# ZhicengShi/mclSTExp

Measured on AMD Instinct MI355X. Metric: training spots/sec (= steps/sec x global batch) at batch 128/GPU, 224px patches, 1000 genes, higher is better.
Workload: dtype bf16; 1 GPU; BASELINE configs[1]: train step, batch 128/GPU, 224x224 patches, 1000 genes, densenet121 image encoder; global_batch=128, parallelism=dp1, backbone_dtype=bf16, infonce=fused, infonce_effective=exact (fused from 1024 pairs), hip_graphs=True, optimizer=Adam(lr=1e-4, wd=1e-3) incl. 2x(65536,G) tables

## Files before the change

### include/mclstexp_hip.h

```cpp
#ifndef MCLSTEXP_HIP_H
#define MCLSTEXP_HIP_H

#include <stddef.h>
#include <stdint.h>

#ifdef __cplusplus
extern "C" {
#endif

#define MCL_ABI_VERSION 13

#define MCL_OK 0
#define MCL_EINVAL (-1)
#define MCL_EUNSUPPORTED (-2)
#define MCL_EWORKSPACE (-3)

typedef void* mcl_stream_t;

int mcl_abi_version(void);
const char* mcl_error_string(int code);

#define MCL_EPI_GELU 1
#define MCL_EPI_GELU_BWD 2
#define MCL_EPI_ACCUM 4
#define MCL_COMPUTE_F32 0
#define MCL_COMPUTE_BF16 1

typedef struct mcl_gemm_args {
  uint32_t struct_size;
  int32_t M, N, K, batch;
  const float* A; int64_t sAm, sAk, sAb;
  const float* B; int64_t sBk, sBn, sBb;
  float* C; int64_t ldc, sCb;
  float alpha;
  int32_t flags;
  const float* bias;
  const float* resid; int64_t ldr, sRb;
  float* pre_out; int64_t ldp;
  const float* aux; int64_t ldaux;
  int32_t compute;
  int32_t ksplit;
  float* workspace;
  const float* flt_thr; int32_t* flt_cnt; float* flt_val; int32_t* flt_idx; int32_t flt_cap;
  uint32_t* counters;
} mcl_gemm_args;

int mcl_gemm(const mcl_gemm_args* args, mcl_stream_t stream);
uint32_t mcl_gemm_args_size(void);
uint32_t mcl_gemm_args_min_size(void);
int32_t mcl_gemm_auto_ksplit(int32_t M, int32_t N, int32_t K, int32_t batch);
int64_t mcl_gemm_workspace_floats(int32_t M, int32_t N, int32_t batch, int32_t ksplit);
int mcl_gemm_group(const mcl_gemm_args* args, int32_t n, mcl_stream_t stream);

int32_t mcl_proj_head_ksplit(int32_t M, int32_t D);
int64_t mcl_proj_head_ws_floats(int32_t M, int32_t ksplit);
int mcl_proj_head_fwd(const float* x, int64_t ldx, int32_t M, int32_t D, const float* wp, int64_t ldwp, const float* bp,
                      const float* wf, int64_t ldwf, const float* bf, const float* gamma, const float* beta, float eps,
                      float* e, float* p, float* a, float* z, float* mean, float* rstd, float* ws, uint32_t* counters,
                      int32_t ksplit, mcl_stream_t stream);
int mcl_proj_head_bwd_rows(const float* de, int64_t ldde, int32_t M, const float* z, const float* mean, const float* rstd,
                           const float* gamma, const float* p, const float* wf, int64_t ldwf, float* dz, float* dp,
                           float* dgamma, float* dbeta, float* dbf, float* dbp, int32_t accumulate_mask, float* ws,
                           uint32_t* counter, mcl_stream_t stream);

int mcl_pos_embed_add_fwd(const float* expr, int64_t ld_expr, const float* pos ,
                          const float* x_table, const float* y_table, int64_t ld_table, int32_t n_rows,
                          float* out, int64_t ld_out, int32_t* ix, int32_t* iy, int32_t* err_flag,
                          int32_t B, int32_t G, mcl_stream_t stream);

int mcl_embed_rowgrad(const float* d_out, int64_t ld_dout, const int32_t* idx, int32_t* owner_idx,
                      float* row_grad, int64_t ld_rg, int32_t B, int32_t G, mcl_stream_t stream);

int mcl_embed_scatter_rows(const int32_t* owner_idx, const float* row_grad, int64_t ld_rg, float* table_grad,
                           int64_t ld_table, int32_t B, int32_t G, int32_t accumulate, mcl_stream_t stream);

int mcl_layernorm_fwd(const float* x, int64_t ldx, const float* gamma, const float* beta, float* y, int64_t ldy,
                      float* mean, float* rstd, int32_t rows, int32_t cols, float eps, mcl_stream_t stream);
int mcl_layernorm_bwd(const float* dy, int64_t lddy, const float* x, int64_t ldx, const float* gamma,
                      const float* mean, const float* rstd, const float* dx_add, int64_t ldadd, float* dx,
                      int64_t lddx, float* dgamma, float* dbeta, int32_t accumulate_params, int32_t rows, int32_t cols,
                      mcl_stream_t stream);

int mcl_attention_fwd(const float* qkv, int64_t ld, int32_t B, int32_t heads, int32_t dim_head, float scale, float* out,
                      int64_t ldo, float* lse, mcl_stream_t stream);
int mcl_attention_bwd(const float* qkv, int64_t ld, int32_t B, int32_t heads, int32_t dim_head, float scale, const float* out,
                      const float* dout, int64_t ldo, const float* lse, float* dvec, float* dqkv, int64_t ldq,
                      mcl_stream_t stream);
int mcl_attention_batched_fwd(const float* qkv, int64_t ld, int32_t B, int32_t nseq, int32_t heads, int32_t dim_head, float scale,
                              float* out, int64_t ldo, float* lse, mcl_stream_t stream);
int mcl_attention_batched_bwd(const float* qkv, int64_t ld, int32_t B, int32_t nseq, int32_t heads, int32_t dim_head, float scale,
                              const float* out, const float* dout, int64_t ldo, const float* lse, float* dvec, float* dqkv,
                              int64_t ldq, mcl_stream_t stream);
int mcl_softmax_rows_fwd(float* s, int64_t ld, int32_t n_rows, int32_t cols, float scale, mcl_stream_t stream);
int mcl_softmax_rows_bwd(const float* p, float* dp, int64_t ld, int32_t n_rows, int32_t cols, float scale,
                         mcl_stream_t stream);

int mcl_colsum(const float* x, int64_t ldx, float* out, int32_t rows, int32_t cols, int32_t accumulate, mcl_stream_t stream);
int mcl_colred_group(int32_t n, const float* const* a, const int64_t* lda, const float* const* x, const int64_t* ldx,
                     const float* const* mean, const float* const* rstd, float* const* out0, float* const* out1,
                     const int32_t* cols, const int32_t* accumulate, int32_t rows, mcl_stream_t stream);
int64_t mcl_rowred_workspace_floats(int32_t rows, int32_t cols);
int mcl_colsum_ws(const float* x, int64_t ldx, float* out, int32_t rows, int32_t cols, int32_t accumulate, float* workspace,
                  mcl_stream_t stream);
int mcl_layernorm_bwd_ws(const float* dy, int64_t lddy, const float* x, int64_t ldx, const float* gamma, const float* mean,
                         const float* rstd, const float* dx_add, int64_t ldadd, float* dx, int64_t lddx, float* dgamma,
                         float* dbeta, int32_t accumulate_params, int32_t rows, int32_t cols, float* workspace, mcl_stream_t stream);

int mcl_soft_clip_mid(const float* S, const float* Tg, const float* lse_row, const float* lse_col, const float* tcol, int32_t B,
                      float c, float* dS, float* dA, float* loss_rows, mcl_stream_t stream);
int mcl_symmetrize(const float* a, int32_t B, float* out, mcl_stream_t stream);

int mcl_infonce_lse(const float* S, int64_t ldS, int32_t R, int32_t C, float* row_lse, float* col_lse,
                    mcl_stream_t stream);
int mcl_infonce_loss(const float* S, int64_t ldS, const float* row_lse, const float* col_lse,
                     int32_t di0, int32_t dj0, int32_t n_diag, int32_t use_rows, int32_t use_cols,
                     float* loss_sum, mcl_stream_t stream);
int mcl_infonce_loss_mean(const float* S, int64_t ldS, const float* row_lse, const float* col_lse, int32_t n, float denom,
                          float* loss_out, mcl_stream_t stream);
int mcl_infonce_dlogits(const float* S, int64_t ldS, const float* row_lse, const float* col_lse, int32_t R,
                        int32_t C, int32_t row0, int32_t col0, float coef, float* dS, int64_t lddS,
                        mcl_stream_t stream);

int64_t mcl_infonce_fused_workspace_bytes(int32_t R, int32_t C, int32_t dim);
int mcl_infonce_fused_lse(const void* a, int64_t lda, const void* b, int64_t ldb, int32_t R, int32_t C, int32_t dim,
                          int32_t diag_off, float inv_temp, float* lse, float* diag, void* workspace, int64_t ws_bytes,
                          mcl_stream_t stream);
int mcl_infonce_fused_grad(const void* a, int64_t lda, const void* b, int64_t ldb, int32_t R, int32_t C, int32_t dim,
                           int32_t diag_off, float inv_temp, const float* lse_a, const float* lse_b, float coef, float* dA,
                           void* workspace, int64_t ws_bytes, mcl_stream_t stream);
int mcl_cast_f32_to_bf16(const float* x, int64_t ldx, void* y, int64_t ldy, int64_t rows, int32_t cols,
                         mcl_stream_t stream);

int64_t mcl_gemm_bf16_workspace_floats(int32_t M, int64_t ldc, int32_t ksplit);
int mcl_gemm_bf16(const void* A, int64_t lda, int64_t sAb, const void* B, int64_t ldb, int64_t sBb, void* C, int64_t ldc,
                  int64_t sCb, int32_t M, int32_t N, int32_t K, int32_t batch, int32_t batch2, int64_t sAb2, int64_t sBb2,
                  int64_t sCb2, float alpha, int32_t flags,
                  const float* bias, const void* resid, int64_t ldr, int64_t sRb, const void* aux, int64_t ldaux,
                  void* pre_out, int64_t ldp, int32_t ksplit, float* workspace, int32_t accumulate, mcl_stream_t stream);
int mcl_ln_bf16_fwd(const void* x, int64_t ldx, const float* gamma, const float* beta, void* y, int64_t ldy, float* mean,
                    float* rstd, int64_t rows, int32_t D, float eps, mcl_stream_t stream);
int64_t mcl_colred_workspace_floats(int64_t rows, int32_t D);
int mcl_ln_bf16_bwd(const void* dy, int64_t lddy, const void* x, int64_t ldx, const float* gamma, const float* mean,
                    const float* rstd, const void* dx_add, int64_t ldadd, void* dx, int64_t lddx, float* workspace,
                    float* dgamma, float* dbeta, int32_t accumulate, int64_t rows, int32_t D, mcl_stream_t stream);
int mcl_colsum_bf16(const void* x, int64_t ldx, int64_t rows, int32_t D, float* workspace, float* out, int32_t accumulate,
                    mcl_stream_t stream);
int mcl_softmax_bf16_fwd(void* s, int64_t ld, int64_t rows, int32_t n, mcl_stream_t stream);
int mcl_softmax_bf16_bwd(const void* P, void* dP, int64_t ld, int64_t rows, int32_t n, float scale, mcl_stream_t stream);
int mcl_vit_attn_fwd(const void* qkv, void* o, float* lse, int32_t B, int32_t T, int32_t heads, float scale, mcl_stream_t stream);
int mcl_vit_attn_bwd(const void* qkv, const void* o, const void* dout, const float* lse, float* dsum, void* dqkv, int32_t B,
                     int32_t T, int32_t heads, float scale, mcl_stream_t stream);
int mcl_vit_patchify_tokens(const float* img, int64_t sb, int64_t sc, int64_t sy, int64_t sx, int32_t B, int32_t H, int32_t W,
                            int32_t p, void* out, int32_t lead_zero_row, int32_t out_f32, mcl_stream_t stream);
int mcl_vit_cls_row(const float* cls, const float* pos, void* x, int32_t B, int32_t T, int32_t D, int32_t dtype,
                    mcl_stream_t stream);
int mcl_vit_assemble_f32(const float* tok, const float* cls, const float* pos, float* x, int32_t B, int32_t T, int32_t D,
                         mcl_stream_t stream);
int mcl_vit_tokens_extract(const void* dx, void* dtok, int32_t B, int32_t T, int32_t D, int32_t dtype, mcl_stream_t stream);
int mcl_vit_token_mean_fwd(const void* x, float* feat, int32_t B, int32_t T, int32_t D, int32_t dtype, mcl_stream_t stream);
int mcl_vit_token_mean_bwd(const float* dfeat, void* dx, int32_t B, int32_t T, int32_t D, int32_t dtype, mcl_stream_t stream);
int mcl_vit_pos_grad(const void* dx, float* dpos, float* dcls, int32_t B, int32_t T, int32_t D, int32_t dtype,
                     int32_t accumulate, mcl_stream_t stream);
int mcl_vit_zero_cls_rows(void* dx, int32_t B, int32_t T, int32_t D, int32_t dtype, mcl_stream_t stream);
int mcl_strided4_f32(const float* src, int32_t n0, int32_t n1, int32_t n2, int32_t n3, int64_t a0, int64_t a1, int64_t a2,
                     int64_t a3, void* dst, int64_t d0, int64_t d1, int64_t d2, int64_t d3, int32_t dst_dtype, int32_t accumulate,
                     mcl_stream_t stream);
int mcl_copy_rows(const void* src, int64_t ld_src_bytes, void* dst, int64_t ld_dst_bytes, int64_t rows, int64_t row_bytes,
                  mcl_stream_t stream);
int mcl_weight_rot180(const void* w, void* wf, int32_t Co, int32_t k, int32_t Ci, int32_t dtype, mcl_stream_t stream);
int mcl_vit_patchify(const float* img, int64_t sb, int64_t sc, int64_t sy, int64_t sx, int32_t B, int32_t H, int32_t W,
                     int32_t p, void* out_bf16, mcl_stream_t stream);

int mcl_quant_e4m3_rows(const float* x, int64_t ldx, int32_t rows, int32_t cols, void* q, int64_t ldq, void* scale,
                        int64_t ld_scale, void* deq_bf16, int64_t ldd, mcl_stream_t stream);
int mcl_dequant_e4m3_rows(const void* q, int64_t ldq, const void* scale, int64_t ld_scale, int32_t rows, int32_t cols,
                          void* deq_bf16, int64_t ldd, mcl_stream_t stream);
int64_t mcl_infonce_fp8_workspace_bytes(int32_t R, int32_t C);
int mcl_infonce_fp8_lse(const void* a8, int64_t lda, const void* scale_a, int64_t ld_sa, const void* b8, int64_t ldb,
                        const void* scale_b, int64_t ld_sb, int32_t R, int32_t C, int32_t dim, float inv_temp, float* lse,
                        void* workspace, int64_t ws_bytes, mcl_stream_t stream);
int mcl_infonce_rowdot_bf16(const void* a, int64_t lda, const void* b, int64_t ldb, int32_t R, int32_t C, int32_t dim,
                            int32_t diag_off, float inv_temp, float* diag, mcl_stream_t stream);

int64_t mcl_bn_workspace_floats(int64_t S, int32_t C, int32_t dtype);
int mcl_bn_stats(const void* x, int64_t ld, int64_t S, int32_t C, int32_t dtype, void* copy_out, int64_t ld_out,
                 float* workspace, float eps, float* mean, float* var, float* rstd, mcl_stream_t stream);
int mcl_bn_act_fwd(const void* x, int64_t ldx, int64_t S, int32_t C, int32_t dtype, const float* gamma,
                   const float* beta, const float* mean, const float* rstd, int32_t relu, void* y, int64_t ldy,
                   mcl_stream_t stream);
int mcl_bn_act_bwd(const void* dy, int64_t lddy, const void* x, int64_t ldx, int64_t S, int32_t C, int32_t dtype,
                   const float* gamma, const float* beta, const float* mean, const float* rstd, int32_t relu,
                   float* workspace, float* dgamma, float* dbeta, int32_t accumulate_params, void* dx, int64_t lddx,
                   int32_t accumulate, mcl_stream_t stream);

int64_t mcl_dense_conv1x1_workspace_floats(int64_t S);
int mcl_dense_conv1x1_fwd(const void* x, int64_t ldx, int64_t S, int32_t K, const float* gamma, const float* beta,
                          const float* mean, const float* rstd, const void* W, void* z, int64_t ldz, float* workspace,
                          float eps, float* zmean, float* zvar, float* zrstd, mcl_stream_t stream);

int64_t mcl_dense_conv3x3_workspace_floats(int64_t S);
int mcl_dense_conv3x3_fwd(const void* z, int64_t S, int32_t H, int32_t W, const float* gamma, const float* beta,
                          const float* mean, const float* rstd, const void* W2, void* out, int64_t ldo,
                          float* workspace, float eps, float* ymean, float* yvar, float* yrstd, mcl_stream_t stream);

int64_t mcl_dense_conv3x3_wrw_workspace_floats(int64_t S);
int mcl_dense_conv3x3_wrw_det(const void* dy, int64_t lddy, const void* z, int64_t S, int32_t H, int32_t W,
                              const float* gamma, const float* beta, const float* mean, const float* rstd,
                              float* workspace, float* dW, int32_t accumulate_w, mcl_stream_t stream);

int64_t mcl_dense_bn1_bwd_workspace_floats(int64_t S, int32_t C);
int mcl_dense_bn1_bwd(const void* dz, const void* W1, int32_t C, const void* x, int64_t ldx, int64_t S,
                      const float* gamma, const float* beta, const float* mean, const float* rstd, float* workspace,
                      float* dgamma, float* dbeta, int32_t accumulate_params, void* gbuf, int64_t ldg,
                      mcl_stream_t stream);

int mcl_dense_bn1_dx_window(const void* dz, const void* W1, int32_t C, int32_t c0, int32_t nc, const void* x, int64_t ldx,
                            int64_t S, const float* gamma, const float* beta, const float* mean, const float* rstd,
                            const float* coef, void* gbuf, int64_t ldg, mcl_stream_t stream);
int mcl_dense_bn1_dx_pair(const void* dzA, const void* W1A, int32_t ldwA, const float* gammaA, const float* betaA,
                          const float* coefA, const void* dzB, const void* W1B, const float* gammaB, const float* betaB,
                          const float* coefB, int32_t C, const void* x, int64_t ldx, int64_t S, const float* mean,
                          const float* rstd, void* gbuf, int64_t ldg, mcl_stream_t stream);

int64_t mcl_wrw_workspace_floats(int64_t S, int32_t M, int32_t N);
int mcl_dense_bn1_wrw(const void* dz, const void* W1, int32_t C, const void* x, int64_t ldx, int64_t S,
                      const float* gamma, const float* beta, const float* mean, const float* rstd, float* workspace,
                      float* dW, int32_t accumulate_w, float* dgamma, float* dbeta, int32_t accumulate_params,
                      float* coef_out, mcl_stream_t stream);
int mcl_dense_bn1_dx(const void* dz, const void* W1, int32_t C, const void* x, int64_t ldx, int64_t S,
                     const float* gamma, const float* beta, const float* mean, const float* rstd, const float* coef,
                     void* gbuf, int64_t ldg, mcl_stream_t stream);
int mcl_dense_bn1_dx_sums(const void* dz, const void* W1, int32_t C, const void* x, int64_t ldx, int64_t S,
                          const float* gamma, const float* beta, const float* mean, const float* rstd, float* workspace,
                          float* dgamma, float* dbeta, int32_t accumulate_params, float* kprev, int32_t have_prev, void* gbuf,
                          int64_t ldg, mcl_stream_t stream);
int mcl_dense_bn1_fix(const void* x, int64_t ldx, void* gbuf, int64_t ldg, int64_t S, int32_t c0, int32_t nc,
                      const float* mean, const float* rstd, const float* kacc, mcl_stream_t stream);
int mcl_conv1x1_wrw_det(const void* dz, int64_t ldz, const void* a, int64_t lda, const float* gamma, const float* beta,
                        const float* mean, const float* rstd, float* workspace, float* dW, int32_t accumulate_w,
                        int64_t S, int32_t M, int32_t N, mcl_stream_t stream);

int64_t mcl_dense_conv3x3_bwd_workspace_floats(int64_t S);
int mcl_dense_conv3x3_bwd(const void* dy, int64_t lddy, int64_t S, int32_t H, int32_t W, const void* W2, const void* z,
                          const float* gamma, const float* beta, const float* mean, const float* rstd, float* workspace,
                          float* dgamma, float* dbeta, int32_t accumulate_params, void* g2, void* dz, mcl_stream_t stream);
int mcl_dense_conv3x3_bwd_fix(const void* dy, int64_t lddy, int64_t S, int32_t H, int32_t W, const void* W2, const void* z,
                              const float* gamma, const float* beta, const float* mean, const float* rstd, float* workspace,
                              float* dgamma, float* dbeta, int32_t accumulate_params, void* g2, void* dz, const void* xfix,
                              int64_t ldxf, const float* fmean, const float* frstd, const float* fk, void* dyc,
                              mcl_stream_t stream);

int mcl_avgpool2_nhwc_bf16(const void* x, void* y, int32_t N, int32_t H, int32_t W, int32_t C, int32_t backward,
                           mcl_stream_t stream);
int mcl_maxpool3s2_nhwc_bf16_fwd(const void* x, void* y, void* idx, int32_t N, int32_t H, int32_t W, int32_t C,
                                 mcl_stream_t stream);
int mcl_maxpool3s2_nhwc_bf16_bwd(const void* idx, const void* dy, void* dx, int32_t N, int32_t H, int32_t W, int32_t C,
                                 mcl_stream_t stream);
int mcl_maxpool3s2_nhwc_bf16_bwd_ld(const void* idx, const void* dy, int64_t lddy, void* dx, int32_t N, int32_t H, int32_t W,
                                    int32_t C, mcl_stream_t stream);

int mcl_bn_act_avgpool_fwd(const void* x, int64_t ldx, int32_t N, int32_t H, int32_t W, int32_t C, const float* gamma,
                           const float* beta, const float* mean, const float* rstd, void* y, int64_t ldy,
                           mcl_stream_t stream);
int mcl_bn_act_avgpool_bwd(const void* dp, int64_t lddp, const void* x, int64_t ldx, int32_t N, int32_t H, int32_t W,
                           int32_t C, const float* gamma, const float* beta, const float* mean, const float* rstd,
                           float* workspace, float* dgamma, float* dbeta, int32_t accumulate_params, void* dx,
                           int64_t lddx, mcl_stream_t stream);
int64_t mcl_conv0_workspace_floats(int32_t N, int32_t H, int32_t W);
int mcl_conv0_fwd(const void* x, int32_t N, int32_t H, int32_t W, const void* Wt, void* y, float* workspace, float eps,
                  float* mean, float* var, float* rstd, mcl_stream_t stream);
int64_t mcl_conv0_wrw_workspace_floats(int32_t N, int32_t H, int32_t W);
int mcl_conv0_wrw(const void* x, int32_t N, int32_t H, int32_t W, const void* dy, float* workspace, float* dW,
                  int32_t accumulate_w, mcl_stream_t stream);

int mcl_bn_act_maxpool_fwd(const void* x, int32_t N, int32_t H, int32_t W, int32_t C, const float* gamma,
                           const float* beta, const float* mean, const float* rstd, void* y, void* idx,
                           mcl_stream_t stream);
int mcl_accum_into_f32(float* dst, const void* src, int64_t n, int32_t src_dtype, mcl_stream_t stream);

int mcl_bn_gap_fwd(const void* x, int64_t ldx, int32_t B, int32_t HW, int32_t C, const float* gamma, const float* beta,
                   const float* mean, const float* rstd, float* out, float* xmean, mcl_stream_t stream);
int mcl_bn_gap_bwd(const float* g, const float* xmean, const void* x, int64_t ldx, int32_t B, int32_t HW, int32_t C,
                   const float* gamma, const float* mean, const float* rstd, float* coef, float* dgamma, float* dbeta,
                   int32_t accumulate_params, void* dx, int64_t lddx, mcl_stream_t stream);
int mcl_bn_eval_rstd(int32_t n, const float* const* running_var, float* const* rstd_out, const int32_t* C, const float* eps,
                     mcl_stream_t stream);
int mcl_bn_running_update(int32_t n, float* const* running_mean, float* const* running_var, const float* const* mean,
                          const float* const* var, int64_t* const* num_batches_tracked, const int32_t* C,
                          const float* factor, const float* momentum, mcl_stream_t stream);
int mcl_image_to_bf16_nhwc(const float* x, int64_t sb, int64_t sc, int64_t sy, int64_t sx, int32_t B, int32_t C, int32_t H,
                           int32_t W, void* y, mcl_stream_t stream);
int mcl_fill_zero(void* p, int64_t bytes, mcl_stream_t stream);
int mcl_dropout_fwd(const float* x, float* y, void* mask, int64_t n, float p, uint64_t seed, mcl_stream_t stream);
int mcl_dropout_bwd(const float* dy, const void* mask, float* dx, int64_t n, float p, mcl_stream_t stream);
int mcl_gelu_f32(const float* x, const float* dy, float* out, int64_t n, mcl_stream_t stream);
int mcl_add_f32(const float* a, const float* b, float* y, int64_t n, mcl_stream_t stream);
int mcl_stamp(void* buf, int32_t idx, mcl_stream_t stream);
int mcl_scale2_f32(const float* a, int64_t na, const float* b, int64_t nb, const float* s, float* ya, float* yb,
                   mcl_stream_t stream);

int mcl_im2col_nhwc(const void* x, int64_t ldx, int32_t N, int32_t H, int32_t W, int32_t C, int32_t KH, int32_t KW,
                    int32_t stride, int32_t pad, int32_t dtype, void* cols, mcl_stream_t stream);
int mcl_col2im_nhwc(const void* dcols, int32_t N, int32_t H, int32_t W, int32_t C, int32_t KH, int32_t KW, int32_t stride,
                    int32_t pad, int32_t dtype, void* dx, int64_t lddx, int32_t accumulate, mcl_stream_t stream);
int mcl_maxpool3s2_nhwc_fwd_any(const void* x, void* y, void* idx, int32_t N, int32_t H, int32_t W, int32_t C, int32_t dtype,
                                mcl_stream_t stream);
int mcl_maxpool3s2_nhwc_bwd_any(const void* idx, const void* dy, void* dx, int32_t N, int32_t H, int32_t W, int32_t C,
                                int32_t dtype, mcl_stream_t stream);
int mcl_avgpool2_nhwc_any(const void* x, void* y, int32_t N, int32_t H, int32_t W, int32_t C, int32_t backward, int32_t dtype,
                          mcl_stream_t stream);
int mcl_gap_nhwc_fwd(const void* x, int64_t ldx, int32_t B, int32_t HW, int32_t C, int32_t dtype, float* out,
                     mcl_stream_t stream);
int mcl_gap_nhwc_bwd(const float* g, int32_t B, int32_t HW, int32_t C, int32_t dtype, void* dx, mcl_stream_t stream);
int mcl_add_relu(const void* a, const void* b, void* y, int64_t n, int32_t backward, int32_t dtype, mcl_stream_t stream);

int mcl_dense_block_pack_w1(const void* const* w1_ptrs, void* const* out_ptrs, int32_t L, int32_t C0, mcl_stream_t stream);
int64_t mcl_dense_block_fwd_workspace_bytes(int32_t B, int32_t L);
int mcl_dense_block_fwd(void* buf, int32_t B, int32_t H, int32_t W, int32_t Ct, int32_t C0, int32_t L,
                        const void* const* layer_ptrs, float eps1, float eps2, float* mean, float* var, float* rstd,
                        void* workspace, int32_t* err_flag, uint32_t max_spins, void* stamps, mcl_stream_t stream);

int mcl_dense_block_pack_bwd(const void* const* w1_ptrs, const void* const* w2_ptrs, void* const* w1t_ptrs,
                             void* const* w2t_ptrs, int32_t L, int32_t C0, mcl_stream_t stream);
int64_t mcl_dense_block_bwd_workspace_bytes(int32_t B, int32_t L);
int mcl_dense_block_bwd(const void* buf, void* gbuf, int32_t B, int32_t H, int32_t W, int32_t Ct, int32_t C0, int32_t L,
                        const void* const* layer_ptrs, const float* mean, const float* rstd, void* workspace,
                        int32_t* err_flag, uint32_t max_spins, void* stamps, mcl_stream_t stream);

int mcl_adam_step(float* p, const float* g, float* m, float* v, int64_t n, double lr, double beta1, double beta2,
                  double eps, double weight_decay, double bc1, double bc2, mcl_stream_t stream);
int mcl_adam_table_step(float* p, float* m, float* v, int32_t n_rows, int32_t cols, const int32_t* row_slot,
                        const float* row_grad, int64_t ld_rg, double lr, double beta1, double beta2, double eps,
                        double weight_decay, double bc1, double bc2, mcl_stream_t stream);

int mcl_adam_consts_update(int64_t* step, float* consts, const double* hyper, mcl_stream_t stream);
int mcl_adam_step_dev(float* p, const float* g, float* m, float* v, int64_t n, const float* consts, mcl_stream_t stream);
int mcl_adam_table_step_dev(float* p, float* m, float* v, int32_t n_rows, int32_t cols, const int32_t* row_slot,
                            const float* row_grad, int64_t ld_rg, const float* consts, mcl_stream_t stream);
int mcl_adam_step_dev_shadow(float* p, const float* g, float* m, float* v, int64_t n, const float* consts,
                             void* shadow_bf16, mcl_stream_t stream);
int mcl_adam_consts_update_hist(int64_t* step, float* consts, const double* hyper, float* hist, int32_t hist_len,
                                mcl_stream_t stream);
int mcl_adam_table_lazy(float* p0, float* m0, float* v0, int32_t* row_step0, float* p1, float* m1, float* v1,
                        int32_t* row_step1, int32_t n_rows, int32_t cols, const float* pos, const int32_t* owner0,
                        const int32_t* owner1, int32_t n_owner, const float* row_grad0, const float* row_grad1, int64_t ld_rg,
                        const int64_t* step, const float* hist, int32_t hist_len, mcl_stream_t stream);
int mcl_row_slot_update(int32_t* row_slot, const int32_t* owner_idx, int32_t B, int32_t fill, mcl_stream_t stream);

int mcl_l2_normalize_rows(const float* x, int64_t ldx, float* y, int64_t ldy, int32_t rows, int32_t dim,
                          mcl_stream_t stream);
int mcl_topk_rows_max_k(void);
int mcl_topk_rows(const float* sim, int64_t ld, int32_t rows, int32_t n, int32_t k, float* values, int64_t* indices,
                  mcl_stream_t stream);
int mcl_topk_rows_indexed(const float* cand_val, int64_t ld, const int32_t* cand_idx, int64_t ld_idx, int rows, int n, int k,
                          float* values, int64_t* indices, int32_t* tie_flag, mcl_stream_t stream);
int mcl_knn_weighted_average(const float* spot_key, int64_t ldk, const float* expression_key, int64_t lde,
                             const float* query, int64_t ldq, const int64_t* indices, int32_t n_query, int32_t k,
                             int32_t dim, int32_t genes, int32_t ord, float* emb_pred, float* expr_pred,
                             mcl_stream_t stream);

int mcl_expr_metrics(const void* pred, int64_t ld_pred, int32_t pred_dtype, const void* truth, int64_t ld_true,
                     int32_t true_dtype, const int64_t* offsets, int32_t S, int32_t G, int32_t n_heg, double* r,
                     double* true_mean, int64_t* heg, double* summary, double* work, mcl_stream_t stream);

int mcl_pearson_pvalue(const double* r, const int64_t* offsets, int32_t S, int32_t G, double* p, double* neglog10p,
                       mcl_stream_t stream);
int mcl_gene_rank(const double* neglog10p, const double* r, int32_t S, int32_t G, int32_t top_n, double* mean,
                  int32_t* n_defined, int64_t* order, int32_t* best_slide, double* best_value, double* best_r,
                  mcl_stream_t stream);

int mcl_knn_combine(const float* spot_key, int64_t ldk, const float* expression_key, int64_t lde, const float* query,
                    int64_t ldq, const int64_t* indices, int32_t n_query, int32_t k, int32_t dim, int32_t genes,
                    int32_t mode, float* emb_pred, float* expr_pred, mcl_stream_t stream);
int mcl_cell_pearson(const void* pred, int64_t ld_pred, int32_t pred_dtype, const void* truth, int64_t ld_true,
                     int32_t true_dtype, int64_t rows, int32_t G, double* r_cell, mcl_stream_t stream);
int mcl_bleep_summary(const void* truth, int64_t ld_true, int32_t true_dtype, const int64_t* offsets, int32_t S, int32_t G,
                      int32_t n_top, const double* r_gene, const double* r_cell, const int32_t* markers, int32_t n_markers,
                      double* gene_sum, double* gene_var, int64_t* top_sum, int64_t* top_var, double* summary,
                      mcl_stream_t stream);
int mcl_corr_from_gram(const double* gram, int32_t m, double* corr, mcl_stream_t stream);

int mcl_pca_gram(const void* x, int64_t ld, int32_t dtype, const int64_t* offsets, int32_t S, int32_t G, int32_t max_rows,
                 const int64_t* gram_offsets, double* mean, double* gram, mcl_stream_t stream);
int mcl_pca_project(const void* x, int64_t ld, int32_t dtype, const int64_t* offsets, int32_t S, int32_t G,
                    int32_t max_rows, int32_t n_comps, const double* mean, const double* evec, const int64_t* evec_offsets,
                    const double* eval, double* loadings, double* sign, double* z, mcl_stream_t stream);
int mcl_kmeans(const double* z, int64_t ld, const int64_t* offsets, int32_t S, int64_t rows, int32_t D, const int32_t* k,
               int32_t k_max, int32_t R, const int64_t* seeds, uint64_t seed, int32_t segment_base, double tol,
               int32_t max_iter, int64_t* seeds_out, int32_t* labels_all, double* centers_all, double* inertia_all,
               int32_t* n_iter_all, double* work, int32_t* labels, double* centers, double* inertia, int32_t* n_iter,
               int32_t* restart, mcl_stream_t stream);
int mcl_cluster_scores(const int32_t* labels_a, const int32_t* labels_b, const int64_t* offsets, int32_t S,
                       int32_t max_rows, double* scores, mcl_stream_t stream);

int mcl_hvg_stats(const void* const* slides, const int64_t* ld, const int32_t* rows, const int32_t* ncols,
                  const int64_t* row_offsets, int32_t dtype, const int32_t* colmaps, int32_t S, int32_t G,
                  int32_t max_rows, int32_t n_top_genes, double* work, double* means, double* dispersions,
                  double* dispersions_norm, int32_t* mean_bin, uint8_t* highly_variable, double* cutoff,
                  double* target_sum, int32_t* status, mcl_stream_t stream);
int mcl_hvg_pool(const uint8_t* highly_variable, int32_t S, int32_t G, const int32_t* extra, int32_t n_extra,
                 uint8_t* union_out, uint8_t* intersection_out, mcl_stream_t stream);
int mcl_expression_matrices(const void* const* slides, const int64_t* ld, const int32_t* rows, const int32_t* ncols,
                            const int64_t* row_offsets, int32_t dtype, const int32_t* sel, int32_t S, int32_t K,
                            int32_t max_rows, float rescale, float* out, mcl_stream_t stream);

int mcl_patch_gather(const void* image_u8, int32_t Hs, int32_t Ws, const int32_t* centers_rc, int32_t N, int32_t r,
                     const void* ops, float divisor, float* out_nchw_f32, void* out_nhwc_bf16, mcl_stream_t stream);
int mcl_log_library_size_normalize(const float* counts, int64_t ldx, float* out, int64_t ldy, int32_t rows,
                                   int32_t cols, float rescale, mcl_stream_t stream);

int mcl_her2st_train_patches(const void* image_u8, int32_t Hs, int32_t Ws, const int32_t* centers_rc, int32_t N, int32_t r,
                             const void* params, float divisor, float* out_nchw_f32, void* out_nhwc_bf16,
                             mcl_stream_t stream);

#ifdef __cplusplus
}
#endif
#endif
```

### mclstexp_amd/_lib.py

```python
from __future__ import annotations

import ctypes as C
import os
from typing import Optional

import torch

_HERE = os.path.dirname(os.path.abspath(__file__))
LIB_PATH = os.environ.get("MCL_LIB_PATH") or os.path.join(_HERE, "libmclstexp_hip.so")
ABI_VERSION = 13

_lib: Optional[C.CDLL] = None

c_f = C.c_float
c_d = C.c_double
c_i = C.c_int32
c_l = C.c_int64
c_p = C.c_void_p


class GemmArgs(C.Structure):
    _fields_ = [
        ("struct_size", C.c_uint32),
        ("M", c_i), ("N", c_i), ("K", c_i), ("batch", c_i),
        ("A", c_p), ("sAm", c_l), ("sAk", c_l), ("sAb", c_l),
        ("B", c_p), ("sBk", c_l), ("sBn", c_l), ("sBb", c_l),
        ("C", c_p), ("ldc", c_l), ("sCb", c_l),
        ("alpha", c_f), ("flags", c_i),
        ("bias", c_p),
        ("resid", c_p), ("ldr", c_l), ("sRb", c_l),
        ("pre_out", c_p), ("ldp", c_l),
        ("aux", c_p), ("ldaux", c_l),
        ("compute", c_i), ("ksplit", c_i),
        ("workspace", c_p),
        ("flt_thr", c_p), ("flt_cnt", c_p), ("flt_val", c_p), ("flt_idx", c_p), ("flt_cap", c_i),
        ("counters", c_p),
    ]




def gemm_args(**kw) -> GemmArgs:
    a = GemmArgs(**kw)
    a.struct_size = C.sizeof(GemmArgs)
    return a


EPI_GELU, EPI_GELU_BWD, EPI_ACCUM = 1, 2, 4
COMPUTE_F32, COMPUTE_BF16 = 0, 1

PROTOTYPES = {
    "mcl_abi_version": [],
    "mcl_error_string": [c_i],
    "mcl_gemm": [C.POINTER(GemmArgs), c_p],
    "mcl_gemm_args_size": [],
    "mcl_gemm_args_min_size": [],
    "mcl_gemm_auto_ksplit": [c_i, c_i, c_i, c_i],
    "mcl_gemm_workspace_floats": [c_i, c_i, c_i, c_i],
    "mcl_gemm_group": [C.POINTER(GemmArgs), c_i, c_p],
    "mcl_proj_head_ksplit": [c_i, c_i],
    "mcl_proj_head_ws_floats": [c_i, c_i],
    "mcl_proj_head_fwd": [c_p, c_l, c_i, c_i, c_p, c_l, c_p, c_p, c_l, c_p, c_p, c_p, c_f, c_p, c_p, c_p, c_p, c_p, c_p, c_p, c_p,
                          c_i, c_p],
    "mcl_proj_head_bwd_rows": [c_p, c_l, c_i, c_p, c_p, c_p, c_p, c_p, c_p, c_l, c_p, c_p, c_p, c_p, c_p, c_p, c_i, c_p, c_p, c_p],
    "mcl_pos_embed_add_fwd": [c_p, c_l, c_p, c_p, c_p, c_l, c_i, c_p, c_l, c_p, c_p, c_p, c_i, c_i, c_p],
    "mcl_embed_rowgrad": [c_p, c_l, c_p, c_p, c_p, c_l, c_i, c_i, c_p],
    "mcl_embed_scatter_rows": [c_p, c_p, c_l, c_p, c_l, c_i, c_i, c_i, c_p],
    "mcl_layernorm_fwd": [c_p, c_l, c_p, c_p, c_p, c_l, c_p, c_p, c_i, c_i, c_f, c_p],
    "mcl_layernorm_bwd": [c_p, c_l, c_p, c_l, c_p, c_p, c_p, c_p, c_l, c_p, c_l, c_p, c_p, c_i, c_i, c_i, c_p],
    "mcl_attention_fwd": [c_p, c_l, c_i, c_i, c_i, c_f, c_p, c_l, c_p, c_p],
    "mcl_attention_bwd": [c_p, c_l, c_i, c_i, c_i, c_f, c_p, c_p, c_l, c_p, c_p, c_p, c_l, c_p],
    "mcl_attention_batched_fwd": [c_p, c_l, c_i, c_i, c_i, c_i, c_f, c_p, c_l, c_p, c_p],
    "mcl_attention_batched_bwd": [c_p, c_l, c_i, c_i, c_i, c_i, c_f, c_p, c_p, c_l, c_p, c_p, c_p, c_l, c_p],
    "mcl_softmax_rows_fwd": [c_p, c_l, c_i, c_i, c_f, c_p],
    "mcl_softmax_rows_bwd": [c_p, c_p, c_l, c_i, c_i, c_f, c_p],
    "mcl_colsum": [c_p, c_l, c_p, c_i, c_i, c_i, c_p],
    "mcl_colred_group": [c_i, C.POINTER(c_p), C.POINTER(c_l), C.POINTER(c_p), C.POINTER(c_l), C.POINTER(c_p), C.POINTER(c_p),
                         C.POINTER(c_p), C.POINTER(c_p), C.POINTER(c_i), C.POINTER(c_i), c_i, c_p],
    "mcl_soft_clip_mid": [c_p, c_p, c_p, c_p, c_p, c_i, c_f, c_p, c_p, c_p, c_p],
    "mcl_symmetrize": [c_p, c_i, c_p, c_p],
    "mcl_colsum_ws": [c_p, c_l, c_p, c_i, c_i, c_i, c_p, c_p],
    "mcl_rowred_workspace_floats": [c_i, c_i],
    "mcl_layernorm_bwd_ws": [c_p, c_l, c_p, c_l, c_p, c_p, c_p, c_p, c_l, c_p, c_l, c_p, c_p, c_i, c_i, c_i, c_p, c_p],
    "mcl_infonce_lse": [c_p, c_l, c_i, c_i, c_p, c_p, c_p],
    "mcl_infonce_loss": [c_p, c_l, c_p, c_p, c_i, c_i, c_i, c_i, c_i, c_p, c_p],
    "mcl_infonce_dlogits": [c_p, c_l, c_p, c_p, c_i, c_i, c_i, c_i, c_f, c_p, c_l, c_p],
    "mcl_infonce_fused_workspace_bytes": [c_i, c_i, c_i],
    "mcl_infonce_fused_lse": [c_p, c_l, c_p, c_l, c_i, c_i, c_i, c_i, c_f, c_p, c_p, c_p, c_l, c_p],
    "mcl_infonce_fused_grad": [c_p, c_l, c_p, c_l, c_i, c_i, c_i, c_i, c_f, c_p, c_p, c_f, c_p, c_p, c_l, c_p],
    "mcl_cast_f32_to_bf16": [c_p, c_l, c_p, c_l, c_l, c_i, c_p],
    "mcl_infonce_loss_mean": [c_p, c_l, c_p, c_p, c_i, c_f, c_p, c_p],
    "mcl_adam_step_dev_shadow": [c_p, c_p, c_p, c_p, c_l, c_p, c_p, c_p],
    "mcl_bn_gap_fwd": [c_p, c_l, c_i, c_i, c_i, c_p, c_p, c_p, c_p, c_p, c_p, c_p],
    "mcl_bn_gap_bwd": [c_p, c_p, c_p, c_l, c_i, c_i, c_i, c_p, c_p, c_p, c_p, c_p, c_p, c_i, c_p, c_l, c_p],
    "mcl_bn_running_update": [c_i, c_p, c_p, c_p, c_p, c_p, c_p, c_p, c_p, c_p],
    "mcl_bn_eval_rstd": [c_i, c_p, c_p, c_p, c_p, c_p],
    "mcl_image_to_bf16_nhwc": [c_p, c_l, c_l, c_l, c_l, c_i, c_i, c_i, c_i, c_p, c_p],
    "mcl_fill_zero": [c_p, c_l, c_p],
    "mcl_stamp": [c_p, c_i, c_p],
    "mcl_dropout_fwd": [c_p, c_p, c_p, c_l, c_f, C.c_uint64, c_p],
    "mcl_dropout_bwd": [c_p, c_p, c_p, c_l, c_f, c_p],
    "mcl_gelu_f32": [c_p, c_p, c_p, c_l, c_p],
    "mcl_add_f32": [c_p, c_p, c_p, c_l, c_p],
    "mcl_im2col_nhwc": [c_p, c_l, c_i, c_i, c_i, c_i, c_i, c_i, c_i, c_i, c_i, c_p, c_p],
    "mcl_col2im_nhwc": [c_p, c_i, c_i, c_i, c_i, c_i, c_i, c_i, c_i, c_i, c_p, c_l, c_i, c_p],
    "mcl_maxpool3s2_nhwc_fwd_any": [c_p, c_p, c_p, c_i, c_i, c_i, c_i, c_i, c_p],
    "mcl_maxpool3s2_nhwc_bwd_any": [c_p, c_p, c_p, c_i, c_i, c_i, c_i, c_i, c_p],
    "mcl_avgpool2_nhwc_any": [c_p, c_p, c_i, c_i, c_i, c_i, c_i, c_i, c_p],
    "mcl_gap_nhwc_fwd": [c_p, c_l, c_i, c_i, c_i, c_i, c_p, c_p],
    "mcl_gap_nhwc_bwd": [c_p, c_i, c_i, c_i, c_i, c_p, c_p],
    "mcl_add_relu": [c_p, c_p, c_p, c_l, c_i, c_i, c_p],
    "mcl_scale2_f32": [c_p, c_l, c_p, c_l, c_p, c_p, c_p, c_p],
    "mcl_maxpool3s2_nhwc_bf16_bwd_ld": [c_p, c_p, c_l, c_p, c_i, c_i, c_i, c_i, c_p],
    "mcl_gemm_bf16_workspace_floats": [c_i, c_l, c_i],
    "mcl_gemm_bf16": [c_p, c_l, c_l, c_p, c_l, c_l, c_p, c_l, c_l, c_i, c_i, c_i, c_i, c_i, c_l, c_l, c_l, c_f, c_i, c_p,
                      c_p, c_l, c_l, c_p, c_l, c_p, c_l, c_i, c_p, c_i, c_p],
    "mcl_ln_bf16_fwd": [c_p, c_l, c_p, c_p, c_p, c_l, c_p, c_p, c_l, c_i, c_f, c_p],
    "mcl_colred_workspace_floats": [c_l, c_i],
    "mcl_ln_bf16_bwd": [c_p, c_l, c_p, c_l, c_p, c_p, c_p, c_p, c_l, c_p, c_l, c_p, c_p, c_p, c_i, c_l, c_i, c_p],
    "mcl_colsum_bf16": [c_p, c_l, c_l, c_i, c_p, c_p, c_i, c_p],
    "mcl_softmax_bf16_fwd": [c_p, c_l, c_l, c_i, c_p],
    "mcl_softmax_bf16_bwd": [c_p, c_p, c_l, c_l, c_i, c_f, c_p],
    "mcl_vit_patchify": [c_p, c_l, c_l, c_l, c_l, c_i, c_i, c_i, c_i, c_p, c_p],
    "mcl_vit_patchify_tokens": [c_p, c_l, c_l, c_l, c_l, c_i, c_i, c_i, c_i, c_p, c_i, c_i, c_p],
    "mcl_vit_cls_row": [c_p, c_p, c_p, c_i, c_i, c_i, c_i, c_p],
    "mcl_vit_assemble_f32": [c_p, c_p, c_p, c_p, c_i, c_i, c_i, c_p],
    "mcl_vit_tokens_extract": [c_p, c_p, c_i, c_i, c_i, c_i, c_p],
    "mcl_vit_token_mean_fwd": [c_p, c_p, c_i, c_i, c_i, c_i, c_p],
    "mcl_vit_token_mean_bwd": [c_p, c_p, c_i, c_i, c_i, c_i, c_p],
    "mcl_vit_pos_grad": [c_p, c_p, c_p, c_i, c_i, c_i, c_i, c_i, c_p],
    "mcl_vit_zero_cls_rows": [c_p, c_i, c_i, c_i, c_i, c_p],
    "mcl_strided4_f32": [c_p, c_i, c_i, c_i, c_i, c_l, c_l, c_l, c_l, c_p, c_l, c_l, c_l, c_l, c_i, c_i, c_p],
    "mcl_copy_rows": [c_p, c_l, c_p, c_l, c_l, c_l, c_p],
    "mcl_weight_rot180": [c_p, c_p, c_i, c_i, c_i, c_i, c_p],
    "mcl_vit_attn_fwd": [c_p, c_p, c_p, c_i, c_i, c_i, c_f, c_p],
    "mcl_vit_attn_bwd": [c_p, c_p, c_p, c_p, c_p, c_p, c_i, c_i, c_i, c_f, c_p],
    "mcl_quant_e4m3_rows": [c_p, c_l, c_i, c_i, c_p, c_l, c_p, c_l, c_p, c_l, c_p],
    "mcl_dequant_e4m3_rows": [c_p, c_l, c_p, c_l, c_i, c_i, c_p, c_l, c_p],
    "mcl_infonce_fp8_workspace_bytes": [c_i, c_i],
    "mcl_infonce_fp8_lse": [c_p, c_l, c_p, c_l, c_p, c_l, c_p, c_l, c_i, c_i, c_i, c_f, c_p, c_p, c_l, c_p],
    "mcl_infonce_rowdot_bf16": [c_p, c_l, c_p, c_l, c_i, c_i, c_i, c_i, c_f, c_p, c_p],
    "mcl_bn_workspace_floats": [c_l, c_i, c_i],
    "mcl_bn_stats": [c_p, c_l, c_l, c_i, c_i, c_p, c_l, c_p, c_f, c_p, c_p, c_p, c_p],
    "mcl_bn_act_fwd": [c_p, c_l, c_l, c_i, c_i, c_p, c_p, c_p, c_p, c_i, c_p, c_l, c_p],
    "mcl_bn_act_bwd": [c_p, c_l, c_p, c_l, c_l, c_i, c_i, c_p, c_p, c_p, c_p, c_i, c_p, c_p, c_p, c_i, c_p, c_l, c_i, c_p],
    "mcl_dense_conv1x1_workspace_floats": [c_l],
    "mcl_dense_conv1x1_fwd": [c_p, c_l, c_l, c_i, c_p, c_p, c_p, c_p, c_p, c_p, c_l, c_p, c_f, c_p, c_p, c_p, c_p],
    "mcl_dense_conv3x3_workspace_floats": [c_l],
    "mcl_dense_bn1_bwd_workspace_floats": [c_l, c_i],
    "mcl_dense_conv3x3_bwd_workspace_floats": [c_l],
    "mcl_avgpool2_nhwc_bf16": [c_p, c_p, c_i, c_i, c_i, c_i, c_i, c_p],
    "mcl_maxpool3s2_nhwc_bf16_fwd": [c_p, c_p, c_p, c_i, c_i, c_i, c_i, c_p],
    "mcl_maxpool3s2_nhwc_bf16_bwd": [c_p, c_p, c_p, c_i, c_i, c_i, c_i, c_p],
    "mcl_dense_conv3x3_bwd": [c_p, c_l, c_l, c_i, c_i, c_p, c_p, c_p, c_p, c_p, c_p, c_p, c_p, c_p, c_i, c_p, c_p, c_p],
    "mcl_dense_conv3x3_bwd_fix": [c_p, c_l, c_l, c_i, c_i, c_p, c_p, c_p, c_p, c_p, c_p, c_p, c_p, c_p, c_i, c_p, c_p, c_p,
                                  c_l, c_p, c_p, c_p, c_p, c_p],
    "mcl_dense_bn1_bwd": [c_p, c_p, c_i, c_p, c_l, c_l, c_p, c_p, c_p, c_p, c_p, c_p, c_p, c_i, c_p, c_l, c_p],
    "mcl_dense_conv3x3_wrw_workspace_floats": [c_l],
    "mcl_dense_conv3x3_wrw_det": [c_p, c_l, c_p, c_l, c_i, c_i, c_p, c_p, c_p, c_p, c_p, c_p, c_i, c_p],
    "mcl_wrw_workspace_floats": [c_l, c_i, c_i],
    "mcl_dense_bn1_wrw": [c_p, c_p, c_i, c_p, c_l, c_l, c_p, c_p, c_p, c_p, c_p, c_p, c_i, c_p, c_p, c_i, c_p, c_p],
    "mcl_dense_bn1_dx_window": [c_p, c_p, c_i, c_i, c_i, c_p, c_l, c_l, c_p, c_p, c_p, c_p, c_p, c_p, c_l, c_p],
    "mcl_dense_bn1_dx_pair": [c_p, c_p, c_i, c_p, c_p, c_p, c_p, c_p, c_p, c_p, c_p, c_i, c_p, c_l, c_l, c_p, c_p, c_p, c_l, c_p],
    "mcl_dense_bn1_dx": [c_p, c_p, c_i, c_p, c_l, c_l, c_p, c_p, c_p, c_p, c_p, c_p, c_l, c_p],
    "mcl_dense_bn1_dx_sums": [c_p, c_p, c_i, c_p, c_l, c_l, c_p, c_p, c_p, c_p, c_p, c_p, c_p, c_i, c_p, c_i, c_p, c_l, c_p],
    "mcl_dense_bn1_fix": [c_p, c_l, c_p, c_l, c_l, c_i, c_i, c_p, c_p, c_p, c_p],
    "mcl_conv1x1_wrw_det": [c_p, c_l, c_p, c_l, c_p, c_p, c_p, c_p, c_p, c_p, c_i, c_l, c_i, c_i, c_p],
    "mcl_dense_conv3x3_fwd": [c_p, c_l, c_i, c_i, c_p, c_p, c_p, c_p, c_p, c_p, c_l, c_p, c_f, c_p, c_p, c_p, c_p],
    "mcl_accum_into_f32": [c_p, c_p, c_l, c_i, c_p],
    "mcl_adam_step": [c_p, c_p, c_p, c_p, c_l, c_d, c_d, c_d, c_d, c_d, c_d, c_d, c_p],
    "mcl_adam_table_step": [c_p, c_p, c_p, c_i, c_i, c_p, c_p, c_l, c_d, c_d, c_d, c_d, c_d, c_d, c_d, c_p],
    "mcl_adam_consts_update": [c_p, c_p, c_p, c_p],
    "mcl_adam_step_dev": [c_p, c_p, c_p, c_p, c_l, c_p, c_p],
    "mcl_adam_table_step_dev": [c_p, c_p, c_p, c_i, c_i, c_p, c_p, c_l, c_p, c_p],
    "mcl_row_slot_update": [c_p, c_p, c_i, c_i, c_p],
    "mcl_dense_block_fwd_workspace_bytes": [c_i, c_i],
    "mcl_dense_block_pack_w1": [c_p, c_p, c_i, c_i, c_p],
    "mcl_dense_block_pack_bwd": [c_p, c_p, c_p, c_p, c_i, c_i, c_p],
    "mcl_dense_block_bwd_workspace_bytes": [c_i, c_i],
    "mcl_dense_block_bwd": [c_p, c_p, c_i, c_i, c_i, c_i, c_i, c_i, c_p, c_p, c_p, c_p, c_p, C.c_uint32, c_p, c_p],
    "mcl_dense_block_fwd": [c_p, c_i, c_i, c_i, c_i, c_i, c_i, c_p, c_f, c_f, c_p, c_p, c_p, c_p, c_p, C.c_uint32, c_p, c_p],
    "mcl_adam_consts_update_hist": [c_p, c_p, c_p, c_p, c_i, c_p],
    "mcl_adam_table_lazy": [c_p, c_p, c_p, c_p, c_p, c_p, c_p, c_p, c_i, c_i, c_p, c_p, c_p, c_i, c_p, c_p, c_l, c_p, c_p, c_i,
                            c_p],
    "mcl_bn_act_avgpool_fwd": [c_p, c_l, c_i, c_i, c_i, c_i, c_p, c_p, c_p, c_p, c_p, c_l, c_p],
    "mcl_bn_act_avgpool_bwd": [c_p, c_l, c_p, c_l, c_i, c_i, c_i, c_i, c_p, c_p, c_p, c_p, c_p, c_p, c_p, c_i, c_p, c_l,
                               c_p],
    "mcl_conv0_workspace_floats": [c_i, c_i, c_i],
    "mcl_conv0_fwd": [c_p, c_i, c_i, c_i, c_p, c_p, c_p, c_f, c_p, c_p, c_p, c_p],
    "mcl_conv0_wrw_workspace_floats": [c_i, c_i, c_i],
    "mcl_conv0_wrw": [c_p, c_i, c_i, c_i, c_p, c_p, c_p, c_i, c_p],
    "mcl_bn_act_maxpool_fwd": [c_p, c_i, c_i, c_i, c_i, c_p, c_p, c_p, c_p, c_p, c_p, c_p],
    "mcl_patch_gather": [c_p, c_i, c_i, c_p, c_i, c_i, c_p, c_f, c_p, c_p, c_p],
    "mcl_her2st_train_patches": [c_p, c_i, c_i, c_p, c_i, c_i, c_p, c_f, c_p, c_p, c_p],
    "mcl_log_library_size_normalize": [c_p, c_l, c_p, c_l, c_i, c_i, c_f, c_p],
    "mcl_l2_normalize_rows": [c_p, c_l, c_p, c_l, c_i, c_i, c_p],
    "mcl_topk_rows_max_k": [],
    "mcl_topk_rows": [c_p, c_l, c_i, c_i, c_i, c_p, c_p, c_p],
    "mcl_topk_rows_indexed": [c_p, c_l, c_p, c_l, c_i, c_i, c_i, c_p, c_p, c_p, c_p],
    "mcl_knn_weighted_average": [c_p, c_l, c_p, c_l, c_p, c_l, c_p, c_i, c_i, c_i, c_i, c_i, c_p, c_p, c_p],
    "mcl_expr_metrics": [c_p, c_l, c_i, c_p, c_l, c_i, c_p, c_i, c_i, c_i, c_p, c_p, c_p, c_p, c_p, c_p],
    "mcl_pearson_pvalue": [c_p, c_p, c_i, c_i, c_p, c_p, c_p],
    "mcl_gene_rank": [c_p, c_p, c_i, c_i, c_i, c_p, c_p, c_p, c_p, c_p, c_p, c_p],
    "mcl_knn_combine": [c_p, c_l, c_p, c_l, c_p, c_l, c_p, c_i, c_i, c_i, c_i, c_i, c_p, c_p, c_p],
    "mcl_cell_pearson": [c_p, c_l, c_i, c_p, c_l, c_i, c_l, c_i, c_p, c_p],
    "mcl_bleep_summary": [c_p, c_l, c_i, c_p, c_i, c_i, c_i, c_p, c_p, c_p, c_i, c_p, c_p, c_p, c_p, c_p, c_p],
    "mcl_corr_from_gram": [c_p, c_i, c_p, c_p],
    "mcl_pca_gram": [c_p, c_l, c_i, c_p, c_i, c_i, c_i, c_p, c_p, c_p, c_p],
    "mcl_pca_project": [c_p, c_l, c_i, c_p, c_i, c_i, c_i, c_i, c_p, c_p, c_p, c_p, c_p, c_p, c_p, c_p],
    "mcl_kmeans": [c_p, c_l, c_p, c_i, c_l, c_i, c_p, c_i, c_i, c_p, C.c_uint64, c_i, c_d, c_i, c_p, c_p, c_p, c_p, c_p, c_p,
                   c_p, c_p, c_p, c_p, c_p, c_p],
    "mcl_cluster_scores": [c_p, c_p, c_p, c_i, c_i, c_p, c_p],
    "mcl_hvg_stats": [c_p, c_p, c_p, c_p, c_p, c_i, c_p, c_i, c_i, c_i, c_i, c_p, c_p, c_p, c_p, c_p, c_p, c_p, c_p, c_p, c_p],
    "mcl_hvg_pool": [c_p, c_i, c_i, c_p, c_i, c_p, c_p, c_p],
    "mcl_expression_matrices": [c_p, c_p, c_p, c_p, c_p, c_i, c_p, c_i, c_i, c_i, c_f, c_p, c_p],
}
_RESTYPES = {"mcl_error_string": C.c_char_p, "mcl_gemm_args_size": C.c_uint32, "mcl_gemm_args_min_size": C.c_uint32, "mcl_dense_block_fwd_workspace_bytes": C.c_int64, "mcl_dense_block_bwd_workspace_bytes": C.c_int64, "mcl_bn_workspace_floats": C.c_int64,
             "mcl_infonce_fused_workspace_bytes": C.c_int64, "mcl_dense_conv1x1_workspace_floats": C.c_int64,
             "mcl_dense_conv3x3_workspace_floats": C.c_int64, "mcl_dense_bn1_bwd_workspace_floats": C.c_int64,
             "mcl_dense_conv3x3_bwd_workspace_floats": C.c_int64, "mcl_conv0_workspace_floats": C.c_int64,
             "mcl_wrw_workspace_floats": C.c_int64, "mcl_dense_conv3x3_wrw_workspace_floats": C.c_int64,
             "mcl_conv0_wrw_workspace_floats": C.c_int64, "mcl_infonce_fp8_workspace_bytes": C.c_int64,
             "mcl_gemm_bf16_workspace_floats": C.c_int64, "mcl_colred_workspace_floats": C.c_int64,
             "mcl_gemm_workspace_floats": C.c_int64, "mcl_rowred_workspace_floats": C.c_int64,
             "mcl_proj_head_ws_floats": C.c_int64}


def load(path: str = LIB_PATH) -> C.CDLL:
    if not os.path.exists(path):
        raise RuntimeError(
            f"{path} not found: the HIP extension is not built.  Run `python -m mclstexp_amd.build` "
            "(hipcc --offload-arch=gfx950).  mclstexp_amd has no CPU fallback.")
    lib = C.CDLL(path)
    for name, argtypes in PROTOTYPES.items():
        try:
            fn = getattr(lib, name)
        except AttributeError as e:
            raise RuntimeError(f"{path} does not export {name}; rebuild the library") from e
        fn.argtypes = argtypes
        fn.restype = _RESTYPES.get(name, C.c_int)
    v = lib.mcl_abi_version()
    if v != ABI_VERSION:
        raise RuntimeError(f"{path} has ABI version {v}, host expects {ABI_VERSION}; rebuild")
    if lib.mcl_gemm_args_size() != C.sizeof(GemmArgs):
        raise RuntimeError(f"{path}: sizeof(mcl_gemm_args) = {lib.mcl_gemm_args_size()}, the ctypes declaration in "
                           f"mclstexp_amd/_lib.py has {C.sizeof(GemmArgs)}; the binding and include/mclstexp_hip.h drifted")
    return lib


def lib() -> C.CDLL:
    global _lib
    if _lib is None:
        _lib = load()
    return _lib


def check(code: int, what: str = "") -> None:
    if code != 0:
        msg = lib().mcl_error_string(code)
        raise RuntimeError(f"mclstexp_hip {what} failed: [{code}] {msg.decode() if msg else '?'}")


class AbiTimer:

    def __init__(self, names):
        self.names = list(names)
        self.records = {n: [] for n in self.names}
        self._orig = {}

    def __enter__(self):
        L = lib()
        for n in self.names:
            orig = getattr(L, n)
            self._orig[n] = orig

            def wrapped(*args, _orig=orig, _n=n):
                st = torch.cuda.current_stream()
                e0 = torch.cuda.Event(enable_timing=True)
                e1 = torch.cuda.Event(enable_timing=True)
                e0.record(st)
                rc = _orig(*args)
                e1.record(st)
                self.records[_n].append((e0, e1, args))
                return rc
            setattr(L, n, wrapped)
        return self

    def __exit__(self, *exc):
        L = lib()
        for n, orig in self._orig.items():
            setattr(L, n, orig)
        self._orig = {}
        return False

    def summary(self):
        torch.cuda.synchronize()
        out = {}
        for n, recs in self.records.items():
            if not recs:
                continue
            ms = [a.elapsed_time(b) for a, b, _ in recs]
            out[n] = {"calls": len(ms), "avg_ms": sum(ms) / len(ms), "total_ms": sum(ms), "ms": ms,
                      "args": [r[2] for r in recs]}
        return out
```

### mclstexp_amd/csrc/bnrelu.hip

```cpp
#include "common.h"

namespace {

constexpr int NTH = 256;

template <typename T> struct Vec;
template <> struct Vec<float> {
  static constexpr int V = 4;
  __device__ static void load(const float* p, float (&f)[4]) {
    const float4 v = *reinterpret_cast<const float4*>(p);
    f[0] = v.x; f[1] = v.y; f[2] = v.z; f[3] = v.w;
  }
  __device__ static void store(float* p, const float (&f)[4]) {
    *reinterpret_cast<float4*>(p) = make_float4(f[0], f[1], f[2], f[3]);
  }
};
template <> struct Vec<bf16_t> {
  static constexpr int V = 8;
  __device__ static void load(const bf16_t* p, float (&f)[8]) {
    const uint4 v = *reinterpret_cast<const uint4*>(p);
    const unsigned w[4] = {v.x, v.y, v.z, v.w};
#pragma unroll
    for (int i = 0; i < 4; ++i) {
      f[2 * i] = __uint_as_float(w[i] << 16);
// ... 30 lines not shown
    const long long r1 = min(S, r0 + rows_per_block);
    for (long long r = r0 + rloc; r < r1; r += rpi) {
      float f[V];
      Vec<T>::load(x + r * ld + (long long)cv * V, f);
      if (copy_out) Vec<T>::store(copy_out + r * ld_out + (long long)cv * V, f);
#pragma unroll
      for (int i = 0; i < V; ++i) {
        const float d = f[i] - k[i];
        s1[i] += d;
        s2[i] = fmaf(d, d, s2[i]);
      }
    }
  }
#pragma unroll
  for (int i = 0; i < V; ++i) {
    smem[i * NTH + t] = s1[i];
    smem[(V + i) * NTH + t] = s2[i];
  }
  __syncthreads();
  if (active && rloc == 0) {
    const long long nblk = gridDim.x;
#pragma unroll
    for (int i = 0; i < V; ++i) {
      float a = 0.0f, b = 0.0f;
      for (int q = 0; q < rpi; ++q) {
        a += smem[i * NTH + t + q * cvn];
        b += smem[(V + i) * NTH + t + q * cvn];
      }
      *reinterpret_cast<float2*>(partial + (((long long)cv * V + i) * nblk + blockIdx.x) * 2) = make_float2(a, b);
    }
  }
}

__device__ __forceinline__ void reduce_partials(const float* __restrict__ partial, int nblk, int c, double& a,
                                                double& b) {
  const int lane = threadIdx.x & 63;
  const float2* p = reinterpret_cast<const float2*>(partial) + (long long)c * nblk;
  float fa = 0.0f, fb = 0.0f;
  double da = 0.0, db = 0.0;
  int cnt = 0;
  for (int i0 = lane; i0 < nblk; i0 += 8 * 64) {
    float2 v[8];
#pragma unroll
    for (int u = 0; u < 8; ++u) v[u] = p[min(i0 + 64 * u, nblk - 1)];
#pragma unroll
    for (int u = 0; u < 8; ++u) {
      if (i0 + 64 * u >= nblk) break;
      fa += v[u].x;
      fb += v[u].y;
      if (++cnt == 4) {
        da += (double)fa; db += (double)fb; fa = fb = 0.0f; cnt = 0;
      }
    }
  }
  da += (double)fa;
  db += (double)fb;
#pragma unroll
  for (int o = 32; o > 0; o >>= 1) {
    da += __shfl_xor(da, o, 64);
    db += __shfl_xor(db, o, 64);
  }
  a = da;
  b = db;
}

template <typename T>
__global__ __launch_bounds__(256) void stats_finalize_kernel(const T* __restrict__ x,
                                                             const float* __restrict__ partial, int nblk, int C,
                                                             long long S, float eps, float* __restrict__ mean,
                                                             float* __restrict__ var, float* __restrict__ rstd) {
  const int c = blockIdx.x * 4 + (threadIdx.x >> 6);
  if (c >= C) return;
  double a, b;
  reduce_partials(partial, nblk, c, a, b);
  if ((threadIdx.x & 63) != 0) return;
  float k;
  if (sizeof(T) == 2) k = bf2f(((const bf16_t*)x)[c]); else k = ((const float*)x)[c];
  const double n = (double)S;
  const double m = a / n;
  double v = b / n - m * m;
  if (v < 0.0) v = 0.0;
  mean[c] = (float)((double)k + m);
  var[c] = (float)v;
  rstd[c] = (float)(1.0 / sqrt(v + (double)eps));
}

template <typename T>
__global__ __launch_bounds__(NTH) void act_fwd_kernel(const T* __restrict__ x, long long ldx, long long S, int C,
                                                      const float* __restrict__ gamma, const float* __restrict__ beta,
                                                      const float* __restrict__ mean, const float* __restrict__ rstd,
                                                      int relu, T* __restrict__ y, long long ldy, int rows_per_block) {
  constexpr int V = Vec<T>::V;
  const int cvn_all = C / V;
  const int tile0 = blockIdx.y * NTH;
  const int cvn = min(cvn_all - tile0, NTH);
  const int rpi = NTH / cvn;
  const int t = threadIdx.x;
  if (t >= rpi * cvn) return;
  const int cv = tile0 + t % cvn, rloc = t / cvn;
  float sc[V], sh[V];
#pragma unroll
  for (int i = 0; i < V; ++i) {
    const int c = cv * V + i;
    sc[i] = gamma[c] * rstd[c];
    sh[i] = fmaf(-mean[c], sc[i], beta[c]);
  }
  const long long r0 = (long long)blockIdx.x * rows_per_block;
  const long long r1 = min(S, r0 + rows_per_block);
  for (long long r = r0 + rloc; r < r1; r += rpi) {
    float f[V];
    Vec<T>::load(x + r * ldx + (long long)cv * V, f);
#pragma unroll
    for (int i = 0; i < V; ++i) {
      float v = fmaf(f[i], sc[i], sh[i]);
      f[i] = relu ? fmaxf(v, 0.0f) : v;
    }
    Vec<T>::store(y + r * ldy + (long long)cv * V, f);
  }
}

template <typename T>
__global__ __launch_bounds__(NTH) void act_avgpool_fwd_kernel(const T* __restrict__ x, long long ldx, long long SP,
                                                              int H, int W, int C, const float* __restrict__ gamma,
                                                              const float* __restrict__ beta,
                                                              const float* __restrict__ mean,
                                                              const float* __restrict__ rstd, T* __restrict__ y,
                                                              long long ldy, int rows_per_block) {
  constexpr int V = Vec<T>::V;
  const int cvn_all = C / V;
  const int tile0 = blockIdx.y * NTH;
  const int cvn = min(cvn_all - tile0, NTH);
  const int rpi = NTH / cvn;
  const int t = threadIdx.x;
  if (t >= rpi * cvn) return;
  const int cv = tile0 + t % cvn, rloc = t / cvn;
  float sc[V], sh[V];
#pragma unroll
  for (int i = 0; i < V; ++i) {
    const int c = cv * V + i;
    sc[i] = gamma[c] * rstd[c];
    sh[i] = fmaf(-mean[c], sc[i], beta[c]);
  }
  const int OW = W >> 1, OH = H >> 1;
  const long long r0 = (long long)blockIdx.x * rows_per_block;
  const long long r1 = min(SP, r0 + rows_per_block);
  for (long long r = r0 + rloc; r < r1; r += rpi) {
    const int ox = (int)(r % OW);
    const long long tt = r / OW;
    const int oy = (int)(tt % OH);
    const long long n = tt / OH;
    const long long base = ((n * H + 2 * oy) * W + 2 * ox);
    float a[V], b[V], c[V], d[V];
    Vec<T>::load(x + base * ldx + (long long)cv * V, a);
    Vec<T>::load(x + (base + 1) * ldx + (long long)cv * V, b);
    Vec<T>::load(x + (base + W) * ldx + (long long)cv * V, c);
    Vec<T>::load(x + (base + W + 1) * ldx + (long long)cv * V, d);
#pragma unroll
    for (int i = 0; i < V; ++i) {
      const float va = fmaxf(fmaf(a[i], sc[i], sh[i]), 0.0f), vb = fmaxf(fmaf(b[i], sc[i], sh[i]), 0.0f);
      const float vc = fmaxf(fmaf(c[i], sc[i], sh[i]), 0.0f), vd = fmaxf(fmaf(d[i], sc[i], sh[i]), 0.0f);
      a[i] = 0.25f * ((va + vb) + (vc + vd));
    }
    Vec<T>::store(y + r * ldy + (long long)cv * V, a);
  }
}

__device__ __forceinline__ long long pooled_row(long long r, int H, int W) {
  const int xw = (int)(r % W);
  const long long t = r / W;
  const int yh = (int)(t % H);
  const long long n = t / H;
  if ((xw >> 1) >= (W >> 1) || (yh >> 1) >= (H >> 1)) return -1;
  return (n * (H >> 1) + (yh >> 1)) * (W >> 1) + (xw >> 1);
}

template <typename T, int MODE = 0>
__global__ __launch_bounds__(NTH) void act_bwd_reduce_kernel(const T* __restrict__ dy, long long lddy,
                                                             const T* __restrict__ x, long long ldx, long long S,
                                                             int C, const float* __restrict__ gamma,
                                                             const float* __restrict__ beta,
                                                             const float* __restrict__ mean,
                                                             const float* __restrict__ rstd, int relu,
                                                             float* __restrict__ partial, int rows_per_block,
                                                             int H = 0, int W = 0) {
  constexpr bool POOL = MODE == 1;
  constexpr int V = Vec<T>::V;
  __shared__ float smem[NTH * 2 * V];
  const int cvn_all = C / V;
  const int tile0 = blockIdx.y * NTH;
  const int cvn = min(cvn_all - tile0, NTH);
  const int rpi = NTH / cvn;
  const int t = threadIdx.x;
  const bool active = t < rpi * cvn;
  const int cv = tile0 + t % cvn, rloc = t / cvn;
  float s1[V], s2[V];
#pragma unroll
  for (int i = 0; i < V; ++i) s1[i] = s2[i] = 0.0f;
  if (active) {
    float sc[V], sh[V], mu[V], rs[V];
#pragma unroll
    for (int i = 0; i < V; ++i) {
      const int c = cv * V + i;
      mu[i] = mean[c];
      rs[i] = rstd[c];
      sc[i] = gamma[c] * rs[i];
      sh[i] = fmaf(-mu[i], sc[i], beta[c]);
    }
    const long long r0 = (long long)blockIdx.x * rows_per_block;
    const long long r1 = min(S, r0 + rows_per_block);
    for (long long r = r0 + rloc; r < r1; r += rpi) {
      float f[V], g[V];
      Vec<T>::load(x + r * ldx + (long long)cv * V, f);
      const long long pr = POOL ? pooled_row(r, H, W) : r;
      if (pr >= 0) Vec<T>::load(dy + pr * lddy + (long long)cv * V, g);
#pragma unroll
      for (int i = 0; i < V; ++i) {
        if (POOL) g[i] = pr >= 0 ? g[i] * 0.25f : 0.0f;
        const float gi = (relu && fmaf(f[i], sc[i], sh[i]) <= 0.0f) ? 0.0f : g[i];
        s1[i] += gi;
        s2[i] = fmaf(gi, (f[i] - mu[i]) * rs[i], s2[i]);
      }
    }
  }
#pragma unroll
  for (int i = 0; i < V; ++i) {
    smem[i * NTH + t] = s1[i];
    smem[(V + i) * NTH + t] = s2[i];
  }
  __syncthreads();
  if (active && rloc == 0) {
    const long long nblk = gridDim.x;
#pragma unroll
    for (int i = 0; i < V; ++i) {
      float a = 0.0f, b = 0.0f;
      for (int q = 0; q < rpi; ++q) {
        a += smem[i * NTH + t + q * cvn];
        b += smem[(V + i) * NTH + t + q * cvn];
      }
      *reinterpret_cast<float2*>(partial + (((long long)cv * V + i) * nblk + blockIdx.x) * 2) = make_float2(a, b);
    }
  }
}

__global__ __launch_bounds__(256) void act_bwd_finalize_kernel(const float* __restrict__ partial, int nblk, int C,
                                                               long long S, float* __restrict__ dgamma,
                                                               float* __restrict__ dbeta, float* __restrict__ coef,
                                                               int accumulate_params) {
  const int c = blockIdx.x * 4 + (threadIdx.x >> 6);
  if (c >= C) return;
  double a, b;
  reduce_partials(partial, nblk, c, a, b);
  if ((threadIdx.x & 63) != 0) return;
  if (accumulate_params) {
    dbeta[c] += (float)a;
    dgamma[c] += (float)b;
  } else {
    dbeta[c] = (float)a;
    dgamma[c] = (float)b;
  }
  coef[2 * c] = (float)(a / (double)S);
  coef[2 * c + 1] = (float)(b / (double)S);
}

template <typename T, int MODE = 0>
__global__ __launch_bounds__(NTH) void act_bwd_dx_kernel(const T* __restrict__ dy, long long lddy,
                                                         const T* __restrict__ x, long long ldx, long long S, int C,
                                                         const float* __restrict__ gamma,
                                                         const float* __restrict__ beta,
                                                         const float* __restrict__ mean,
                                                         const float* __restrict__ rstd, int relu,
                                                         const float* __restrict__ coef, T* dx, long long lddx,
                                                         int accumulate, int rows_per_block, int H = 0, int W = 0) {
  constexpr bool POOL = MODE == 1;
  constexpr int V = Vec<T>::V;
  const int cvn_all = C / V;
  const int tile0 = blockIdx.y * NTH;
  const int cvn = min(cvn_all - tile0, NTH);
  const int rpi = NTH / cvn;
  const int t = threadIdx.x;
  if (t >= rpi * cvn) return;
  const int cv = tile0 + t % cvn, rloc = t / cvn;
  float sc[V], sh[V], mu[V], rs[V], c1[V], c2[V];
#pragma unroll
  for (int i = 0; i < V; ++i) {
    const int c = cv * V + i;
    mu[i] = mean[c];
    rs[i] = rstd[c];
    sc[i] = gamma[c] * rs[i];
    sh[i] = fmaf(-mu[i], sc[i], beta[c]);
    c1[i] = coef[2 * c];
    c2[i] = coef[2 * c + 1];
  }
  const long long r0 = (long long)blockIdx.x * rows_per_block;
  const long long r1 = min(S, r0 + rows_per_block);
  for (long long r = r0 + rloc; r < r1; r += rpi) {
    float f[V], g[V], o[V];
    Vec<T>::load(x + r * ldx + (long long)cv * V, f);
    const long long pr = POOL ? pooled_row(r, H, W) : r;
    if (pr >= 0) Vec<T>::load(dy + pr * lddy + (long long)cv * V, g);
    if (accumulate) Vec<T>::load(dx + r * lddx + (long long)cv * V, o);
#pragma unroll
    for (int i = 0; i < V; ++i) {
      if (POOL) g[i] = pr >= 0 ? g[i] * 0.25f : 0.0f;
      const float gi = (relu && fmaf(f[i], sc[i], sh[i]) <= 0.0f) ? 0.0f : g[i];
      const float xh = (f[i] - mu[i]) * rs[i];
      const float d = sc[i] * (gi - c1[i] - xh * c2[i]);
      o[i] = accumulate ? o[i] + d : d;
    }
    Vec<T>::store(dx + r * lddx + (long long)cv * V, o);
  }
}

template <typename T>
__global__ __launch_bounds__(256) void accum_kernel(float* __restrict__ dst, const T* __restrict__ src, long long n) {
  const long long stride = (long long)gridDim.x * blockDim.x;
  for (long long i = (long long)blockIdx.x * blockDim.x + threadIdx.x; i < n; i += stride) {
    float v;
    if (sizeof(T) == 2) v = bf2f(((const bf16_t*)src)[i]); else v = ((const float*)src)[i];
    dst[i] += v;
  }
}

inline int vec_of(int dtype) { return dtype == 1 ? 8 : 4; }
inline bool ok_layout(const void* p, long long ld, int C, int dtype) {
  const int V = vec_of(dtype);
  return p && (C % V == 0) && (ld % V == 0) && ((reinterpret_cast<uintptr_t>(p) & 15u) == 0);
}
inline void plan(long long S, int C, int dtype, int* nblk, int* rows_per_block, int* tiles) {
  const int V = vec_of(dtype);
  const int cvn_all = C / V;
  const int cvn = cvn_all < NTH ? cvn_all : NTH;
  const int rpi = NTH / cvn;
  long long rpb = (long long)rpi * 8;
  long long nb = (S + rpb - 1) / rpb;
  if (nb > 1024) {
    nb = 1024;
    rpb = (S + nb - 1) / nb;
    rpb = (rpb + rpi - 1) / rpi * rpi;
    nb = (S + rpb - 1) / rpb;
  }
  *nblk = (int)nb;
  *rows_per_block = (int)rpb;
  *tiles = (cvn_all + NTH - 1) / NTH;
}

}

extern "C" int64_t mcl_bn_workspace_floats(int64_t S, int32_t C, int32_t dtype) {
  if (S <= 0 || C <= 0 || (dtype != 0 && dtype != 1) || C % vec_of(dtype) != 0) return -1;
  int nblk, rpb, tiles;
  plan(S, C, dtype, &nblk, &rpb, &tiles);
  return (int64_t)nblk * 2 * C + 2 * C;
}

extern "C" int mcl_bn_stats(const void* x, int64_t ld, int64_t S, int32_t C, int32_t dtype, void* copy_out,
                            int64_t ld_out, float* workspace, float eps, float* mean, float* var, float* rstd,
                            mcl_stream_t stream) {
  MCL_CLEAR_ERROR();
  if (!workspace || !mean || !var || !rstd || S <= 0 || C <= 0 || (dtype != 0 && dtype != 1)) return MCL_EINVAL;
  if (!ok_layout(x, ld, C, dtype) || (copy_out && !ok_layout(copy_out, ld_out, C, dtype))) return MCL_EUNSUPPORTED;
  int nblk, rpb, tiles;
  plan(S, C, dtype, &nblk, &rpb, &tiles);
  hipStream_t st = mcl_stream(stream);
  dim3 grid(nblk, tiles);
  if (dtype == 1) {
    hipLaunchKernelGGL(stats_partial_kernel<bf16_t>, grid, dim3(NTH), 0, st, (const bf16_t*)x, (long long)ld,
                       (long long)S, C, (bf16_t*)copy_out, (long long)ld_out, workspace, rpb);
    hipLaunchKernelGGL(stats_finalize_kernel<bf16_t>, dim3((C + 3) / 4), dim3(256), 0, st, (const bf16_t*)x,
                       workspace, nblk, C, (long long)S, eps, mean, var, rstd);
  } else {
    hipLaunchKernelGGL(stats_partial_kernel<float>, grid, dim3(NTH), 0, st, (const float*)x, (long long)ld,
                       (long long)S, C, (float*)copy_out, (long long)ld_out, workspace, rpb);
    hipLaunchKernelGGL(stats_finalize_kernel<float>, dim3((C + 3) / 4), dim3(256), 0, st, (const float*)x,
                       workspace, nblk, C, (long long)S, eps, mean, var, rstd);
  }
  MCL_CHECK_LAUNCH();
  return MCL_OK;
}

extern "C" int mcl_bn_act_fwd(const void* x, int64_t ldx, int64_t S, int32_t C, int32_t dtype, const float* gamma,
                              const float* beta, const float* mean, const float* rstd, int32_t relu, void* y,
                              int64_t ldy, mcl_stream_t stream) {
  MCL_CLEAR_ERROR();
  if (!gamma || !beta || !mean || !rstd || S <= 0 || C <= 0 || (dtype != 0 && dtype != 1)) return MCL_EINVAL;
  if (!ok_layout(x, ldx, C, dtype) || !ok_layout(y, ldy, C, dtype)) return MCL_EUNSUPPORTED;
  int nblk, rpb, tiles;
  plan(S, C, dtype, &nblk, &rpb, &tiles);
  dim3 grid(nblk, tiles);
  if (dtype == 1)
    hipLaunchKernelGGL(act_fwd_kernel<bf16_t>, grid, dim3(NTH), 0, mcl_stream(stream), (const bf16_t*)x,
                       (long long)ldx, (long long)S, C, gamma, beta, mean, rstd, relu, (bf16_t*)y, (long long)ldy, rpb);
  else
    hipLaunchKernelGGL(act_fwd_kernel<float>, grid, dim3(NTH), 0, mcl_stream(stream), (const float*)x,
                       (long long)ldx, (long long)S, C, gamma, beta, mean, rstd, relu, (float*)y, (long long)ldy, rpb);
  MCL_CHECK_LAUNCH();
  return MCL_OK;
}

extern "C" int mcl_bn_act_bwd(const void* dy, int64_t lddy, const void* x, int64_t ldx, int64_t S, int32_t C,
                              int32_t dtype, const float* gamma, const float* beta, const float* mean,
                              const float* rstd, int32_t relu, float* workspace, float* dgamma, float* dbeta,
                              int32_t accumulate_params, void* dx, int64_t lddx, int32_t accumulate,
                              mcl_stream_t stream) {
  MCL_CLEAR_ERROR();
  if (!gamma || !beta || !mean || !rstd || !workspace || !dgamma || !dbeta || S <= 0 || C <= 0 ||
      (dtype != 0 && dtype != 1))
    return MCL_EINVAL;
  if (!ok_layout(dy, lddy, C, dtype) || !ok_layout(x, ldx, C, dtype) || !ok_layout(dx, lddx, C, dtype))
    return MCL_EUNSUPPORTED;
  int nblk, rpb, tiles;
  plan(S, C, dtype, &nblk, &rpb, &tiles);
  dim3 grid(nblk, tiles);
  hipStream_t st = mcl_stream(stream);
  float* coef = workspace + (long long)nblk * 2 * C;
  if (dtype == 1) {
    hipLaunchKernelGGL(act_bwd_reduce_kernel<bf16_t>, grid, dim3(NTH), 0, st, (const bf16_t*)dy, (long long)lddy,
                       (const bf16_t*)x, (long long)ldx, (long long)S, C, gamma, beta, mean, rstd, relu, workspace, rpb);
    hipLaunchKernelGGL(act_bwd_finalize_kernel, dim3((C + 3) / 4), dim3(256), 0, st, workspace, nblk, C,
                       (long long)S, dgamma, dbeta, coef, accumulate_params);
    hipLaunchKernelGGL(act_bwd_dx_kernel<bf16_t>, grid, dim3(NTH), 0, st, (const bf16_t*)dy, (long long)lddy,
                       (const bf16_t*)x, (long long)ldx, (long long)S, C, gamma, beta, mean, rstd, relu, coef,
                       (bf16_t*)dx, (long long)lddx, accumulate, rpb);
  } else {
    hipLaunchKernelGGL(act_bwd_reduce_kernel<float>, grid, dim3(NTH), 0, st, (const float*)dy, (long long)lddy,
                       (const float*)x, (long long)ldx, (long long)S, C, gamma, beta, mean, rstd, relu, workspace, rpb);
    hipLaunchKernelGGL(act_bwd_finalize_kernel, dim3((C + 3) / 4), dim3(256), 0, st, workspace, nblk, C,
                       (long long)S, dgamma, dbeta, coef, accumulate_params);
    hipLaunchKernelGGL(act_bwd_dx_kernel<float>, grid, dim3(NTH), 0, st, (const float*)dy, (long long)lddy,
                       (const float*)x, (long long)ldx, (long long)S, C, gamma, beta, mean, rstd, relu, coef,
                       (float*)dx, (long long)lddx, accumulate, rpb);
  }
  MCL_CHECK_LAUNCH();
  return MCL_OK;
}

extern "C" int mcl_bn_act_avgpool_fwd(const void* x, int64_t ldx, int32_t N, int32_t H, int32_t W, int32_t C,
                                      const float* gamma, const float* beta, const float* mean, const float* rstd,
                                      void* y, int64_t ldy, mcl_stream_t stream) {
  MCL_CLEAR_ERROR();
  if (!gamma || !beta || !mean || !rstd || N <= 0 || H <= 0 || W <= 0 || C <= 0) return MCL_EINVAL;
  if (H < 2 || W < 2 || !ok_layout(x, ldx, C, 1) || !ok_layout(y, ldy, C, 1)) return MCL_EUNSUPPORTED;
  const long long SP = (long long)N * (H / 2) * (W / 2);
  int nblk, rpb, tiles;
  plan(SP, C, 1, &nblk, &rpb, &tiles);
  hipLaunchKernelGGL(act_avgpool_fwd_kernel<bf16_t>, dim3(nblk, tiles), dim3(NTH), 0, mcl_stream(stream),
                     (const bf16_t*)x, (long long)ldx, SP, H, W, C, gamma, beta, mean, rstd, (bf16_t*)y,
                     (long long)ldy, rpb);
  MCL_CHECK_LAUNCH();
  return MCL_OK;
}

extern "C" int mcl_bn_act_avgpool_bwd(const void* dp, int64_t lddp, const void* x, int64_t ldx, int32_t N, int32_t H,
                                      int32_t W, int32_t C, const float* gamma, const float* beta, const float* mean,
                                      const float* rstd, float* workspace, float* dgamma, float* dbeta,
                                      int32_t accumulate_params, void* dx, int64_t lddx, mcl_stream_t stream) {
  MCL_CLEAR_ERROR();
  if (!gamma || !beta || !mean || !rstd || !workspace || !dgamma || !dbeta || N <= 0 || H <= 0 || W <= 0 || C <= 0)
    return MCL_EINVAL;
  if (H < 2 || W < 2 || !ok_layout(dp, lddp, C, 1) || !ok_layout(x, ldx, C, 1) || !ok_layout(dx, lddx, C, 1))
    return MCL_EUNSUPPORTED;
  const long long S = (long long)N * H * W;
  int nblk, rpb, tiles;
  plan(S, C, 1, &nblk, &rpb, &tiles);
  dim3 grid(nblk, tiles);
  hipStream_t st = mcl_stream(stream);
  float* coef = workspace + (long long)nblk * 2 * C;
  hipLaunchKernelGGL((act_bwd_reduce_kernel<bf16_t, 1>), grid, dim3(NTH), 0, st, (const bf16_t*)dp,
                     (long long)lddp, (const bf16_t*)x, (long long)ldx, S, C, gamma, beta, mean, rstd, 1, workspace, rpb,
                     H, W);
  hipLaunchKernelGGL(act_bwd_finalize_kernel, dim3((C + 3) / 4), dim3(256), 0, st, workspace, nblk, C, S, dgamma,
                     dbeta, coef, accumulate_params);
  hipLaunchKernelGGL((act_bwd_dx_kernel<bf16_t, 1>), grid, dim3(NTH), 0, st, (const bf16_t*)dp, (long long)lddp,
                     (const bf16_t*)x, (long long)ldx, S, C, gamma, beta, mean, rstd, 1, coef, (bf16_t*)dx,
                     (long long)lddx, 0, rpb, H, W);
  MCL_CHECK_LAUNCH();
  return MCL_OK;
}

extern "C" int mcl_accum_into_f32(float* dst, const void* src, int64_t n, int32_t src_dtype, mcl_stream_t stream) {
  MCL_CLEAR_ERROR();
  if (!dst || !src || n <= 0 || (src_dtype != 0 && src_dtype != 1)) return MCL_EINVAL;
  long long blocks = (n + 255) / 256;
  if (blocks > 1024) blocks = 1024;
  if (src_dtype == 1)
    hipLaunchKernelGGL(accum_kernel<bf16_t>, dim3((unsigned)blocks), dim3(256), 0, mcl_stream(stream), dst,
                       (const bf16_t*)src, (long long)n);
  else
    hipLaunchKernelGGL(accum_kernel<float>, dim3((unsigned)blocks), dim3(256), 0, mcl_stream(stream), dst,
                       (const float*)src, (long long)n);
  MCL_CHECK_LAUNCH();
  return MCL_OK;
}
```

### mclstexp_amd/csrc/dense_conv.hip

```cpp
#include "common.h"

namespace {

constexpr int BN = 128;
constexpr int BK = 64;

template <int WM, int RW = 64, int DEPTH = 1>
__global__ __launch_bounds__(128 * WM) void conv1x1_fwd_kernel(const bf16_t* __restrict__ x, long long ldx, long long S,
                                                               int K, const float* __restrict__ gamma,
                                                               const float* __restrict__ beta,
                                                               const float* __restrict__ mean,
                                                               const float* __restrict__ rstd,
                                                               const bf16_t* __restrict__ W, bf16_t* __restrict__ z,
                                                               long long ldz, float2* __restrict__ partial, int nblk) {
  constexpr int BM = RW * WM, NT = 128 * WM;
  constexpr int RI = RW / 32;
  constexpr int NA = (BM * 8) / NT;
  constexpr int A_B = BM * 128, B_B = BN * 128, STAGE_B = A_B + B_B;
  constexpr int NB = (BN * 8) / NT;
  constexpr int NBUF = DEPTH == 0 ? 1 : 2, NSET = DEPTH == 0 ? 1 : DEPTH;
  __shared__ __attribute__((aligned(16))) unsigned char lds[NBUF * STAGE_B + 2 * 1024 * 4];
  float* tab = reinterpret_cast<float*>(lds + NBUF * STAGE_B);

  const int tid = threadIdx.x, lane = tid & 63, wave = tid >> 6;
// ... 547 lines not shown
    sh[i] = fmaf(-mean[c], sc[i], beta[c]);
  }
  f32x16 acc[3];
#pragma unroll
  for (int b = 0; b < 3; ++b)
#pragma unroll
    for (int r = 0; r < 16; ++r) acc[b][r] = 0.0f;

  const int i15 = lane & 15, q = i15 >> 2, jj = i15 & 3;
  const int half16 = 16 * ((lane >> 4) & 1);
  const int byte = (jj & 1) * 8;
  int bz_lo[3], bz_hi[3];
#pragma unroll
  for (int kx = 0; kx < 3; ++kx) {
    const int chunk = wave * 4 + ((half16 + jj * 4) >> 3);
    const int r0 = 8 * h + q + kx, r1 = r0 + 4;
    bz_lo[kx] = r0 * 256 + ((chunk ^ w3k_swz(r0)) << 4) + byte;
    bz_hi[kx] = r1 * 256 + ((chunk ^ w3k_swz(r1)) << 4) + byte;
  }
  const int dchunk = (half16 + jj * 4) >> 3;

  auto fetch = [&](uint4 (&zv)[9], uint4 (&dv)[2], int tile) {
    const int p0 = tile * T3;
    const int qs = p0 + (ky - 1) * W - 1;
#pragma unroll
    for (int i = 0; i < 9; ++i) {
      const int j = rz + 16 * i;
      const int p = qs + j;
      zv[i] = (tile < ntile && j < W3K_ROWS && p >= 0 && p < Si)
                  ? *reinterpret_cast<const uint4*>(z + (long long)p * C3_IN + cc * 8)
                  : make_uint4(0u, 0u, 0u, 0u);
    }
    const int p = p0 + rd;
#pragma unroll
    for (int u = 0; u < 2; ++u)
      dv[u] = (tile < ntile && p < Si) ? *reinterpret_cast<const uint4*>(dy + (long long)p * lddy + (cd + u) * 8)
                                       : make_uint4(0u, 0u, 0u, 0u);
  };
  auto stage = [&](const uint4 (&zv)[9], const uint4 (&dv)[2], int tile) {
    const int p0 = tile * T3;
    const int qs = p0 + (ky - 1) * W - 1;
#pragma unroll
    for (int i = 0; i < 9; ++i) {
      const int j = rz + 16 * i;
      if (j < W3K_ROWS) {
        const int p = qs + j;
        const bool ok = p >= 0 && p < Si;
        *reinterpret_cast<uint4*>(zt + j * 256 + ((cc ^ w3k_swz(j)) << 4)) =
            ok ? bn_relu_chunk(zv[i], sc, sh) : make_uint4(0u, 0u, 0u, 0u);
      }
    }
    const int p = p0 + rd;
    const int x = p % W, y = (p / W) % H;
    const bool vy = (unsigned)(y + ky - 1) < (unsigned)H && p < Si;
#pragma unroll
    for (int kx = 0; kx < 3; ++kx) {
      const bool v = vy && (unsigned)(x + kx - 1) < (unsigned)W;
#pragma unroll
      for (int u = 0; u < 2; ++u)
        *reinterpret_cast<uint4*>(dyt + kx * (T3 * 64) + rd * 64 + (((cd + u) ^ ((rd >> 1) & 3)) << 4)) =
            v ? dv[u] : make_uint4(0u, 0u, 0u, 0u);
    }
  };
  auto multiply = [&]() {
#pragma unroll 2
    for (int ks = 0; ks < 8; ++ks) {
      const int r_lo = ks * 16 + 8 * h + q, r_hi = r_lo + 4;
      const int da_lo = r_lo * 64 + ((dchunk ^ ((r_lo >> 1) & 3)) << 4) + byte;
      const int da_hi = r_hi * 64 + ((dchunk ^ ((r_hi >> 1) & 3)) << 4) + byte;
#pragma unroll
      for (int kx = 0; kx < 3; ++kx) {
        const v4s alo = __builtin_amdgcn_ds_read_tr16_b64_v4i16(
            (v4s __attribute__((address_space(3)))*)(dyt + kx * (T3 * 64) + da_lo));
        const v4s ahi = __builtin_amdgcn_ds_read_tr16_b64_v4i16(
            (v4s __attribute__((address_space(3)))*)(dyt + kx * (T3 * 64) + da_hi));
        const v4s blo = __builtin_amdgcn_ds_read_tr16_b64_v4i16(
            (v4s __attribute__((address_space(3)))*)(zt + bz_lo[kx] + ks * 4096));
        const v4s bhi = __builtin_amdgcn_ds_read_tr16_b64_v4i16(
            (v4s __attribute__((address_space(3)))*)(zt + bz_hi[kx] + ks * 4096));
        bf16x8 fa, fb;
        fa[0] = alo[0]; fa[1] = alo[1]; fa[2] = alo[2]; fa[3] = alo[3];
        fa[4] = ahi[0]; fa[5] = ahi[1]; fa[6] = ahi[2]; fa[7] = ahi[3];
        fb[0] = blo[0]; fb[1] = blo[1]; fb[2] = blo[2]; fb[3] = blo[3];
        fb[4] = bhi[0]; fb[5] = bhi[1]; fb[6] = bhi[2]; fb[7] = bhi[3];
        acc[kx] = __builtin_amdgcn_mfma_f32_32x32x16_bf16(fa, fb, acc[kx], 0, 0, 0);
      }
    }
  };

  const int per = (ntile + G - 1) / G;
  const int t_end = min(ntile, (g + 1) * per);
  uint4 zvA[9], dvA[2], zvB[9], dvB[2];
  int tile = g * per;
  fetch(zvA, dvA, tile < t_end ? tile : ntile);
  fetch(zvB, dvB, tile + 1 < t_end ? tile + 1 : ntile);
  for (; tile < t_end; tile += 2) {
    __syncthreads();
    stage(zvA, dvA, tile);
    __syncthreads();
    fetch(zvA, dvA, tile + 2 < t_end ? tile + 2 : ntile);
    multiply();
    if (tile + 1 < t_end) {
      __syncthreads();
      stage(zvB, dvB, tile + 1);
      __syncthreads();
      fetch(zvB, dvB, tile + 3 < t_end ? tile + 3 : ntile);
      multiply();
    }
  }
  float* dst = wpart + (long long)g * (C3_OUT * 9 * C3_IN);
#pragma unroll
  for (int kx = 0; kx < 3; ++kx) {
    const int n = (3 * ky + kx) * C3_IN + 32 * wave + l31;
#pragma unroll
    for (int r = 0; r < 16; ++r) {
      const int co = (r & 3) + 8 * (r >> 2) + 4 * h;
      dst[co * (9 * C3_IN) + n] = acc[kx][r];
    }
  }
}

}

static inline int wrw3k_groups(int ntile) {
  const int g = 88;
  return ntile < g ? ntile : g;
}

extern "C" int64_t mcl_dense_conv3x3_wrw_workspace_floats(int64_t S) {
  if (S <= 0) return -1;
  const int ntile = (int)((S + T3 - 1) / T3);
  const int64_t g = wrw3k_groups(ntile);
  return (g > 256 ? g : 256) * (int64_t)(C3_OUT * 9 * C3_IN);
}

extern "C" int mcl_dense_conv3x3_wrw_det(const void* dy, int64_t lddy, const void* z, int64_t S, int32_t H, int32_t W,
                                         const float* gamma, const float* beta, const float* mean, const float* rstd,
                                         float* workspace, float* dW, int32_t accumulate_w, mcl_stream_t stream) {
  MCL_CLEAR_ERROR();
  if (!dy || !z || !gamma || !beta || !mean || !rstd || !dW || !workspace || S <= 0 || H <= 0 || W <= 0) return MCL_EINVAL;
  if ((S % ((int64_t)H * W)) || S > 0x7fff0000LL || W > 150 || (lddy % 8) || lddy < C3_OUT || (reinterpret_cast<uintptr_t>(dy) & 15u) ||
      (reinterpret_cast<uintptr_t>(z) & 15u) || (reinterpret_cast<uintptr_t>(dW) & 15u) ||
      (reinterpret_cast<uintptr_t>(workspace) & 15u))
    return MCL_EUNSUPPORTED;
  const int ntile = (int)((S + T3 - 1) / T3);
  hipStream_t st = mcl_stream(stream);
  if (mcl_conv3x3_wrw_rows_applicable(S, H, W)) {
    return mcl_launch_conv3x3_wrw_rows(dy, lddy, z, S, H, W, gamma, beta, mean, rstd, workspace, dW, accumulate_w, st);
  }
  const int G = wrw3k_groups(ntile);
  const int nblk = ((G + 7) / 8) * 8 * 3;
  hipLaunchKernelGGL(conv3x3_wrw_ky_kernel, dim3(nblk), dim3(256), 0, st, (const bf16_t*)dy, (long long)lddy,
                     (const bf16_t*)z, (long long)S, H, W, gamma, beta, mean, rstd, ntile, G, workspace);
  mcl_launch_wrw_merge(workspace, G, (long long)C3_OUT * 9 * C3_IN, dW, accumulate_w, st);
  MCL_CHECK_LAUNCH();
  return MCL_OK;
}

namespace {

constexpr int C0_OUT = 64, C0_K = 7, C0_KP = 24;

constexpr int C0_P0 = 16;
__host__ __device__ inline int c0_pw(int W) { return ((C0_P0 + 3 * W + 24 + 7) / 8) * 8; }
__device__ __forceinline__ u32x4 c0_rsrc(const void* base, unsigned bytes) {
  const unsigned long long a = (unsigned long long)base;
  return u32x4{(unsigned)a, (unsigned)(a >> 32) & 0xFFFFu, bytes, 0x00020000u};
}
__device__ __forceinline__ void c0_dma_slab(const bf16_t* __restrict__ x, int n, int oy0, int H, int W, unsigned slab_lds, int PW,
                                            int wave, int lane) {
  const int cpr = (W * 6) >> 4;
  for (int r = wave; r < 9; r += 4) {
    const int iy = 2 * oy0 - 3 + r;
    const bool inside = iy >= 0 && iy < H;
    const u32x4 rs = c0_rsrc(x + ((long long)(n * H + (inside ? iy : 0)) * W) * 3, inside ? (unsigned)(W * 6) : 0u);
    const unsigned dst = slab_lds + (unsigned)(r * PW + C0_P0) * 2u;
    for (int c0 = 0; c0 < cpr; c0 += 64)
      if (c0 + lane < cpr) buffer_lds16(rs, (unsigned)(c0 + lane) * 16u, dst + (unsigned)c0 * 16u);
  }
}

__global__ __launch_bounds__(256, 3) void conv0_fwd_kernel(const bf16_t* __restrict__ x, int N, int H, int W,
                                                           const bf16_t* __restrict__ Wt, bf16_t* __restrict__ y,
                                                           float2* __restrict__ partial, int ntile) {
  extern __shared__ __attribute__((aligned(16))) unsigned char lds[];
  const int OH = H >> 1, OW = W >> 1;
  const int PW = c0_pw(W);
  const int npix = 2 * OW;
  bf16_t* slab = reinterpret_cast<bf16_t*>(lds);
  const int slab_bytes = 9 * PW * 2;
  bf16_t* ot = reinterpret_cast<bf16_t*>(lds + slab_bytes);
  float* red = reinterpret_cast<float*>(lds + slab_bytes + 256 * 128);
  const int tid = threadIdx.x, lane = tid & 63, wave = tid >> 6;
  const int h = lane >> 5, l31 = lane & 31;

  {
    constexpr int WDW = (C0_OUT * C0_K * 21) / 2;
    unsigned* wl = reinterpret_cast<unsigned*>(ot);
    const unsigned* w32 = reinterpret_cast<const unsigned*>(Wt);
    unsigned wv[(WDW + 255) / 256];
#pragma unroll
    for (int k = 0; k < (WDW + 255) / 256; ++k) wv[k] = w32[min(tid + 256 * k, WDW - 1)];
#pragma unroll
    for (int k = 0; k < (WDW + 255) / 256; ++k) wl[min(tid + 256 * k, WDW - 1)] = wv[k];
  }
  __syncthreads();
  bf16x8 breg[2][11];
  {
    const bf16_t* wls = reinterpret_cast<const bf16_t*>(ot);
#pragma unroll
    for (int nt = 0; nt < 2; ++nt)
#pragma unroll
      for (int s = 0; s < 11; ++s) {
        const int q = 2 * s + h, ky = q / 3, j0 = (q % 3) * 8;
        const int co = nt * 32 + l31;
#pragma unroll
        for (int i = 0; i < 8; ++i) {
          const int j = j0 + i - 1;
          const bool ok = q < 21 && j >= 0 && j < 21;
          const short w1 = (short)wls[ok ? (co * C0_K + ky) * 21 + j : 0];
          breg[nt][s][i] = ok ? w1 : (short)0;
        }
      }
  }
  const int nmt = (npix + 31) >> 5;
  const unsigned slab_lds = (unsigned)(size_t)((__attribute__((address_space(3))) void*)(lds));
  const int wave_u = __builtin_amdgcn_readfirstlane(wave);
  for (int i = tid; i < slab_bytes / 16; i += 256) reinterpret_cast<uint4*>(lds)[i] = make_uint4(0u, 0u, 0u, 0u);
  __syncthreads();
  if ((int)blockIdx.x < ntile)
    c0_dma_slab(x, (int)blockIdx.x / (OH >> 1), ((int)blockIdx.x % (OH >> 1)) * 2, H, W, slab_lds, PW, wave_u, lane);

  for (int tile = blockIdx.x; tile < ntile; tile += gridDim.x) {
    const int n = tile / (OH >> 1), oy0 = (tile % (OH >> 1)) * 2;
    asm volatile("s_waitcnt vmcnt(0)" ::: "memory");
    __syncthreads();

    float s1[2] = {0.f, 0.f}, s2[2] = {0.f, 0.f};
    for (int mt = wave; mt < nmt; mt += 4) {
      int m = mt * 32 + l31;
      const bool mvalid = m < npix;
      if (!mvalid) m = npix - 1;
      const int rr = m / OW, ox = m - rr * OW;
      const unsigned* arow = reinterpret_cast<const unsigned*>(slab + (2 * rr) * PW + 6 + 6 * ox);
      f32x16 acc[2];
#pragma unroll
      for (int nt = 0; nt < 2; ++nt)
#pragma unroll
        for (int r = 0; r < 16; ++r) acc[nt][r] = 0.0f;
#pragma unroll
      for (int s = 0; s < 11; ++s) {
        const int q = 2 * s + h, ky = q / 3, j0 = (q % 3) * 8;
        const unsigned* ap = arow + ((ky * PW + j0) >> 1);
        u32x4 av;
        av[0] = ap[0]; av[1] = ap[1]; av[2] = ap[2]; av[3] = ap[3];
        if (q >= 21) av = (u32x4){0u, 0u, 0u, 0u};
        const bf16x8 a = __builtin_bit_cast(bf16x8, av);
#pragma unroll
        for (int nt = 0; nt < 2; ++nt) acc[nt] = __builtin_amdgcn_mfma_f32_32x32x16_bf16(a, breg[nt][s], acc[nt], 0, 0, 0);
      }
#pragma unroll
      for (int nt = 0; nt < 2; ++nt)
#pragma unroll
        for (int r = 0; r < 16; ++r) {
          const int px = mt * 32 + (r & 3) + 8 * (r >> 2) + 4 * h;
          const float v = round_bf16(acc[nt][r]);
          if (px < npix) {
            s1[nt] += v;
            s2[nt] = fmaf(v, v, s2[nt]);
            ot[px * C0_OUT + nt * 32 + l31] = (bf16_t)(__float_as_uint(v) >> 16);
          }
        }
    }
#pragma unroll
    for (int nt = 0; nt < 2; ++nt) {
      s1[nt] += __shfl_xor(s1[nt], 32, 64);
      s2[nt] += __shfl_xor(s2[nt], 32, 64);
      if (h == 0) {
        red[(wave * 64 + nt * 32 + l31) * 2] = s1[nt];
        red[(wave * 64 + nt * 32 + l31) * 2 + 1] = s2[nt];
      }
    }
    __syncthreads();
    {
      const int nx = tile + (int)gridDim.x;
      if (nx < ntile) c0_dma_slab(x, nx / (OH >> 1), (nx % (OH >> 1)) * 2, H, W, slab_lds, PW, wave_u, lane);
    }
    if (tid < 64) {
      float a = 0.f, b = 0.f;
#pragma unroll
      for (int w = 0; w < 4; ++w) {
        a += red[(w * 64 + tid) * 2];
        b += red[(w * 64 + tid) * 2 + 1];
      }
      const float nn = (float)npix;
      partial[(long long)tid * ntile + tile] = make_float2(a, b - a * a / nn);
    }
    bf16_t* yo = y + ((long long)(n * OH + oy0) * OW) * C0_OUT;
    for (int c = tid; c < npix * 8; c += 256)
      reinterpret_cast<uint4*>(yo)[c] = reinterpret_cast<const uint4*>(ot)[c];
  }
}

__global__ __launch_bounds__(256, 2) void conv0_wrw_kernel(const bf16_t* __restrict__ x, int N, int H, int W,
                                                           const bf16_t* __restrict__ dy, float* __restrict__ dW,
                                                           int ntile, float* __restrict__ wpart) {
  extern __shared__ __attribute__((aligned(16))) unsigned char lds[];
  const int OH = H >> 1, OW = W >> 1;
  const int PW = (W + 6) * 3 + 8;
  const int OWp = (OW + 15) & ~15;
  const int npix = 2 * OW;
  bf16_t* slab = reinterpret_cast<bf16_t*>(lds);
  const int slab_bytes = (9 * PW * 2 + 15) & ~15;
  unsigned char* dyt = lds + slab_bytes;
  const int tid = threadIdx.x, lane = tid & 63, wave = tid >> 6;
  const int h = lane >> 5, l31 = lane & 31;
  const int mt = wave & 1, kt0 = (wave >> 1) * 3;
  int koff[3];
  bool kval[3];
#pragma unroll
  for (int t = 0; t < 3; ++t) {
    const int k = (kt0 + t) * 32 + l31;
    const int ky = k / C0_KP, j = k % C0_KP;
    kval[t] = k < 7 * C0_KP && j < 21;
    koff[t] = kval[t] ? ky * PW + j : 0;
  }
  f32x16 acc[3];
#pragma unroll
  for (int t = 0; t < 3; ++t)
#pragma unroll
    for (int r = 0; r < 16; ++r) acc[t][r] = 0.0f;

  for (int i = tid; i < (slab_bytes + 2 * OWp * 128) / 16; i += 256) reinterpret_cast<uint4*>(lds)[i] = make_uint4(0u, 0u, 0u, 0u);
  const int i16 = lane & 15, q4 = i16 >> 2;
  const int lch = (mt * 32 + 16 * ((lane >> 4) & 1)) / 8 + ((i16 & 3) >> 1);
  const unsigned a_off = (unsigned)(q4 * 128 + ((lch ^ (((q4 >> 1) & 1) << 2)) << 4) + (i16 & 1) * 8);
  constexpr int NDY = 8, NX = 4;
  const int cpr = (W * 6) >> 4;
  u32x4 rdy[NDY];
  uint4 rx[NX];
  unsigned xvalid = 0;
  for (int tile = blockIdx.x; tile < ntile; tile += gridDim.x) {
    const int n = tile / (OH >> 1), oy0 = (tile % (OH >> 1)) * 2;
    const bf16_t* dyo = dy + ((long long)(n * OH + oy0) * OW) * C0_OUT;
#pragma unroll
    for (int u = 0; u < NDY; ++u) rdy[u] = reinterpret_cast<const u32x4*>(dyo)[min(tid + 256 * u, npix * 8 - 1)];
    xvalid = 0;
#pragma unroll
    for (int u = 0; u < NX; ++u) {
      const int c = min(tid + 256 * u, 9 * cpr - 1);
      const int r = c / cpr, cc = c % cpr;
      const int iy = 2 * oy0 - 3 + r;
      xvalid |= (iy >= 0 && iy < H) ? (1u << u) : 0u;
      rx[u] = *reinterpret_cast<const uint4*>(x + ((long long)(n * H + min(max(iy, 0), H - 1)) * W) * 3 + cc * 8);
    }
    __syncthreads();
#pragma unroll
    for (int u = 0; u < NDY; ++u) {
      const int c = tid + 256 * u;
      if (c < npix * 8) {
        const int px = c >> 3, c8 = c & 7;
        const int pc = px < OW ? px : px - OW + OWp;
        *reinterpret_cast<u32x4*>(dyt + pc * 128 + ((c8 ^ (((pc >> 1) & 1) << 2)) << 4)) = rdy[u];
      }
    }
#pragma unroll
    for (int u = 0; u < NX; ++u) {
      const int c = tid + 256 * u;
      if (c < 9 * cpr) {
        const int r = c / cpr, cc = c % cpr;
        bf16_t* d = slab + r * PW + 9 + cc * 8;
        const bool ok = (xvalid >> u) & 1u;
        const unsigned wv[4] = {ok ? rx[u].x : 0u, ok ? rx[u].y : 0u, ok ? rx[u].z : 0u, ok ? rx[u].w : 0u};
#pragma unroll
        for (int i = 0; i < 4; ++i) {
          d[2 * i] = (bf16_t)(wv[i] & 0xFFFFu);
          d[2 * i + 1] = (bf16_t)(wv[i] >> 16);
        }
      }
    }
    __syncthreads();

    for (int p0 = 0; p0 < 2 * OWp; p0 += 16) {
      const int rr = p0 / OWp, ox0 = p0 - rr * OWp;
      const unsigned char* ap = dyt + (p0 + 8 * h) * 128 + a_off;
      const v4s alo = __builtin_amdgcn_ds_read_tr16_b64_v4i16((v4s __attribute__((address_space(3)))*)(ap));
      const v4s ahi = __builtin_amdgcn_ds_read_tr16_b64_v4i16((v4s __attribute__((address_space(3)))*)(ap + 4 * 128));
      bf16x8 a;
      a[0] = alo[0]; a[1] = alo[1]; a[2] = alo[2]; a[3] = alo[3];
      a[4] = ahi[0]; a[5] = ahi[1]; a[6] = ahi[2]; a[7] = ahi[3];
      const bf16_t* brow = slab + (2 * rr) * PW + 6 * (ox0 + 8 * h);
#pragma unroll
      for (int t = 0; t < 3; ++t) {
        const bf16_t* bp = brow + koff[t];
        bf16x8 b;
#pragma unroll
        for (int i = 0; i < 8; ++i) b[i] = (short)bp[6 * i];
        acc[t] = __builtin_amdgcn_mfma_f32_32x32x16_bf16(a, b, acc[t], 0, 0, 0);
      }
    }
  }
#pragma unroll
  for (int t = 0; t < 3; ++t) {
    if (!kval[t]) continue;
    const int k = (kt0 + t) * 32 + l31;
    const int ky = k / C0_KP, j = k % C0_KP;
    float* dst = wpart + (long long)blockIdx.x * (C0_OUT * C0_K * 21);
#pragma unroll
    for (int r = 0; r < 16; ++r) {
      const int co = mt * 32 + (r & 3) + 8 * (r >> 2) + 4 * h;
      dst[(co * C0_K + ky) * 21 + j] = acc[t][r];
    }
  }
}

}


extern "C" int64_t mcl_conv0_workspace_floats(int32_t N, int32_t H, int32_t W) {
  if (N <= 0 || H <= 0 || W <= 0) return -1;
  return (int64_t)N * (H / 4 + 1) * C0_OUT * 2;
}

extern "C" int mcl_conv0_fwd(const void* x, int32_t N, int32_t H, int32_t W, const void* Wt, void* y, float* workspace,
                             float eps, float* mean, float* var, float* rstd, mcl_stream_t stream) {
  MCL_CLEAR_ERROR();
  if (!x || !Wt || !y || !workspace || N <= 0 || H <= 0 || W <= 0) return MCL_EINVAL;
  const bool want_stats = mean || var || rstd;
  if (want_stats && (!mean || !var || !rstd)) return MCL_EINVAL;
  if ((H % 4) || (W % 8) || W > 256 || (reinterpret_cast<uintptr_t>(x) & 15u) || (reinterpret_cast<uintptr_t>(y) & 15u))
    return MCL_EUNSUPPORTED;
  const int OH = H / 2, OW = W / 2;
  const int ntile = N * (OH / 2);
  const int PW = c0_pw(W);
  const size_t lds_bytes = (size_t)(9 * PW * 2) + 256 * 128 + 4 * 64 * 2 * 4;
  static mcl_device_once attr_once;
  if (auto attr_guard = attr_once.first()) {
    (void)hipFuncSetAttribute(reinterpret_cast<const void*>(conv0_fwd_kernel),
                              hipFuncAttributeMaxDynamicSharedMemorySize, 96 * 1024);
  }
  hipStream_t st = mcl_stream(stream);
  float2* part = reinterpret_cast<float2*>(workspace);
  hipLaunchKernelGGL(conv0_fwd_kernel, dim3(ntile < 768 ? ntile : 768), dim3(256), lds_bytes, st, (const bf16_t*)x, N, H,
                     W, (const bf16_t*)Wt, (bf16_t*)y, part, ntile);
  if (want_stats)
    hipLaunchKernelGGL(tile_stats_finalize_kernel, dim3(C0_OUT), dim3(256), 0, st, (const float2*)part, ntile, C0_OUT,
                       (long long)N * OH * OW, 2 * OW, eps, mean, var, rstd);
  MCL_CHECK_LAUNCH();
  return MCL_OK;
}

inline int conv0_wrw_grid(int ntile) {
  const int cap = 768;
  return ntile < cap ? ntile : cap;
}
extern "C" int64_t mcl_conv0_wrw_workspace_floats(int32_t N, int32_t H, int32_t W) {
  if (N <= 0 || H <= 0 || W <= 0) return -1;
  return (int64_t)conv0_wrw_grid(N * (H / 4)) * (C0_OUT * C0_K * 21);
}

extern "C" int mcl_conv0_wrw(const void* x, int32_t N, int32_t H, int32_t W, const void* dy, float* workspace, float* dW,
                             int32_t accumulate_w, mcl_stream_t stream) {
  MCL_CLEAR_ERROR();
  if (!x || !dy || !dW || !workspace || N <= 0 || H <= 0 || W <= 0) return MCL_EINVAL;
  if ((H % 4) || (W % 8) || W > 256 || (reinterpret_cast<uintptr_t>(x) & 15u) || (reinterpret_cast<uintptr_t>(dy) & 15u) ||
      (reinterpret_cast<uintptr_t>(workspace) & 15u) || (reinterpret_cast<uintptr_t>(dW) & 15u))
    return MCL_EUNSUPPORTED;
  const int OH = H / 2, OW = W / 2, OWp = (OW + 15) & ~15;
  const int ntile = N * (OH / 2);
  const int PW = (W + 6) * 3 + 8;
  const size_t lds_bytes = (size_t)((9 * PW * 2 + 15) & ~15) + (size_t)2 * OWp * 128;
  static mcl_device_once attr_once;
  if (auto attr_guard = attr_once.first()) {
    (void)hipFuncSetAttribute(reinterpret_cast<const void*>(conv0_wrw_kernel),
                              hipFuncAttributeMaxDynamicSharedMemorySize, 96 * 1024);
  }
  hipStream_t st = mcl_stream(stream);
  const int grid = conv0_wrw_grid(ntile);
  hipLaunchKernelGGL(conv0_wrw_kernel, dim3(grid), dim3(256), lds_bytes, st, (const bf16_t*)x, N, H, W,
                     (const bf16_t*)dy, dW, ntile, workspace);
  mcl_launch_wrw_merge(workspace, grid, (long long)C0_OUT * C0_K * 21, dW, accumulate_w, st);
  MCL_CHECK_LAUNCH();
  return MCL_OK;
}
```

### mclstexp_amd/csrc/device.h

```cpp
#pragma once
#include <hip/hip_runtime.h>

typedef unsigned short bf16_t;
typedef __bf16 bf16x2_t __attribute__((ext_vector_type(2)));
typedef short bf16x8 __attribute__((ext_vector_type(8)));
typedef short v4s __attribute__((ext_vector_type(4)));
typedef float f32x2 __attribute__((ext_vector_type(2)));
typedef float f32x4 __attribute__((ext_vector_type(4)));
typedef float f32x16 __attribute__((ext_vector_type(16)));
typedef unsigned u32x2 __attribute__((ext_vector_type(2)));
typedef unsigned u32x4 __attribute__((ext_vector_type(4)));
typedef unsigned long long u64;

#define MCL_LDSP(p) ((__attribute__((address_space(3))) void*)(p))
#define MCL_GLBP(p) ((const __attribute__((address_space(1))) void*)(p))

__device__ __forceinline__ float bf_lo(unsigned w) { return __uint_as_float(w << 16); }
__device__ __forceinline__ float bf_hi(unsigned w) { return __uint_as_float(w & 0xFFFF0000u); }
__device__ __forceinline__ float bf2f(bf16_t v) { return __uint_as_float(((unsigned)v) << 16); }
__device__ __forceinline__ unsigned pack_bf16(float a, float b) {
  const f32x2 v = {a, b};
  return __builtin_bit_cast(unsigned, __builtin_convertvector(v, bf16x2_t));
}
__device__ __forceinline__ bf16_t f2bf(float f) { return (bf16_t)(pack_bf16(f, 0.0f) & 0xFFFFu); }
__device__ __forceinline__ float round_bf16(float v) { return bf_lo(pack_bf16(v, 0.0f)); }
__device__ __forceinline__ unsigned f2bf_rne(float f) {
  unsigned u = __float_as_uint(f);
  if ((u & 0x7F800000u) == 0x7F800000u) return u >> 16;
  u += 0x7FFFu + ((u >> 16) & 1u);
  return u >> 16;
}

__device__ __forceinline__ void unpack8(uint4 v, float (&f)[8]) {
  const unsigned w[4] = {v.x, v.y, v.z, v.w};
#pragma unroll
  for (int i = 0; i < 4; ++i) {
    f[2 * i] = bf_lo(w[i]);
    f[2 * i + 1] = bf_hi(w[i]);
  }
}
__device__ __forceinline__ uint4 pack8(const float (&f)[8]) {
  unsigned w[4];
#pragma unroll
  for (int i = 0; i < 4; ++i) {
    const f32x2 v = {f[2 * i], f[2 * i + 1]};
    w[i] = __builtin_bit_cast(unsigned, __builtin_convertvector(v, bf16x2_t));
  }
  return make_uint4(w[0], w[1], w[2], w[3]);
}

__device__ __forceinline__ uint4 bn_relu_chunk(uint4 v, const float (&sc)[8], const float (&sh)[8]) {
  unsigned w[4] = {v.x, v.y, v.z, v.w};
#pragma unroll
  for (int i = 0; i < 4; ++i) {
    const float lo = fmaxf(fmaf(bf_lo(w[i]), sc[2 * i], sh[2 * i]), 0.0f);
    const float hi = fmaxf(fmaf(bf_hi(w[i]), sc[2 * i + 1], sh[2 * i + 1]), 0.0f);
    w[i] = pack_bf16(lo, hi);
  }
  return make_uint4(w[0], w[1], w[2], w[3]);
}

template <typename T>
__device__ __forceinline__ double ldd(const T* p) { return (double)*p; }

__device__ __forceinline__ unsigned lanes_below(unsigned long long mask) {
  return __builtin_amdgcn_mbcnt_hi((unsigned)(mask >> 32), __builtin_amdgcn_mbcnt_lo((unsigned)mask, 0u));
}

__device__ __forceinline__ float half_wave_sum(float x) {
#define MCL_DPP_ADD(ctrl, rmask)                                                                              \
  x += __int_as_float(__builtin_amdgcn_update_dpp(0, __float_as_int(x), ctrl, rmask, 0xF, false))
  MCL_DPP_ADD(0xB1, 0xF);
  MCL_DPP_ADD(0x4E, 0xF);
  MCL_DPP_ADD(0x141, 0xF);
  MCL_DPP_ADD(0x140, 0xF);
  MCL_DPP_ADD(0x142, 0xA);
#undef MCL_DPP_ADD
  return x;
}

__device__ __forceinline__ int opaque_lane(int lane) {
  asm volatile("" : "+v"(lane));
  return lane;
}

__device__ __forceinline__ void glds16(const void* src, unsigned dst) {
  unsigned keep;
  asm volatile("s_mov_b32 %0, m0\n\ts_mov_b32 m0, %2\n\ts_nop 0\n\tglobal_load_lds_dwordx4 %1, off\n\ts_mov_b32 m0, %0"
               : "=&s"(keep)
               : "v"(src), "s"(dst)
               : "memory");
}
__device__ __forceinline__ void glds16s(const void* sbase, unsigned voff, unsigned dst) {
  asm volatile("s_mov_b32 m0, %2\n\ts_nop 0\n\tglobal_load_lds_dwordx4 %1, %0"
               :
               : "s"(sbase), "v"(voff), "s"(dst)
               : "memory", "m0");
}
__device__ __forceinline__ void glds4(const void* src, unsigned dst) {
  unsigned keep;
  asm volatile("s_mov_b32 %0, m0\n\ts_mov_b32 m0, %2\n\ts_nop 0\n\tglobal_load_lds_dword %1, off\n\ts_mov_b32 m0, %0"
               : "=&s"(keep)
               : "v"(src), "s"(dst)
               : "memory");
}
__device__ __forceinline__ void buffer_lds16(u32x4 rsrc, unsigned voff, unsigned dst) {
  unsigned keep;
  asm volatile("s_mov_b32 %0, m0\n\ts_mov_b32 m0, %3\n\ts_nop 0\n\tbuffer_load_dwordx4 %1, %2, 0 offen lds\n\ts_mov_b32 m0, %0"
               : "=&s"(keep)
               : "v"(voff), "s"(rsrc), "s"(dst)
               : "memory");
}
```

### mclstexp_amd/densenet_fused.py

```python
from __future__ import annotations

import contextlib
import os
from typing import List, NamedTuple, Optional, Tuple

import torch
import torch.nn.functional as F
from torch import nn

from . import _lib
from ._lib import check

Tensor = torch.Tensor
CL = torch.channels_last
_ws_cache = {}

_fallbacks: dict = {}


def fallback_counts() -> dict:
    return dict(_fallbacks)


def reset_fallbacks() -> None:
# ... 767 lines not shown
        conv1 = "single"
    else:
        conv1 = "two_pass"
    if not kacc_live:
        fix = "none"
    elif conv1 != "single":
        fix = "launch_all"
    elif growth == 32 and conv2 == "own" and _c3_flat_kernel(W):
        fix = "fold"
    else:
        fix = "launch_32"
    return _LayerPlan(conv2, conv1, fix, lanes=side_stream and conv1 != "generic" and conv2 == "own",
                      opens_pair=conv1 == "gram" and l >= 1 and growth == 32 and cin - growth >= 8)


class DenseBlockFn(torch.autograd.Function):

    @staticmethod
    def forward(ctx, x0, meta, *params):
        stats, eps1, eps2, growth, bn2_stats = meta[:5]
        prefilled = len(meta) > 5 and meta[5]
        ctx.first_block = (not prefilled) or (len(meta) > 6 and bool(meta[6]))
        L = len(params) // 6
        B, C0, H, W = x0.shape
        Ct = C0 + L * growth
        dev, dt = x0.device, x0.dtype
        pre = getattr(stats, "buf", None) if prefilled else None
        if (pre is not None and tuple(pre.shape) == (B, Ct, H, W) and pre.dtype == dt and x0.data_ptr() == pre.data_ptr()
                and x0.stride() == pre[:, :C0].stride()):
            buf, adopted = pre.detach(), True
        else:
            buf, adopted = torch.empty((B, Ct, H, W), device=dev, dtype=dt, memory_format=CL), False
            x0 = dense_cl(x0)
        if adopted:
            pass
        elif prefilled:
            buf[:, :C0].copy_(x0)
        else:
            bn_stats(x0, stats.mean[:C0], stats.var[:C0], stats.rstd[:C0], eps1[0], copy_out=buf[:, :C0])
        saved = []
        wcast = []
        kept_cols = {}
        ctx.persistent = False
        if _block_persistent_ok(buf, params, growth, L, C0, dt):
            wcast = [_weight(params[6 * l + k], dt) for l in range(L) for k in (2, 5)]
            zs = dense_block_fwd_persistent(buf, params, wcast, stats, bn2_stats, C0, L, eps1[0], eps2[0])
            for l in range(L):
                saved += [buf.new_empty(0), zs[l], buf.new_empty(0)]
            L_done = L
            ctx.persistent = True
        else:
            L_done = 0
        for l in range(L_done, L):
            g1, b1, w1, g2, b2, w2 = params[6 * l: 6 * l + 6]
            cin = C0 + l * growth
            w1c = _weight(w1, dt)
            m2, v2, r2 = bn2_stats[l]
            if _fused_1x1_ok(buf, w1c):
                a = None
                z = dense_conv1x1_fwd(buf[:, :cin], g1, b1, stats.mean[:cin], stats.rstd[:cin], w1c, eps2[l], m2, v2, r2)
            else:
                a = torch.empty((B, cin, H, W), device=dev, dtype=dt, memory_format=CL)
                bn_act_fwd(buf[:, :cin], g1, b1, stats.mean[:cin], stats.rstd[:cin], True, a)
                z = _conv1x1_fwd(a, w1c)
                bn_stats(z, m2, v2, r2, eps2[l])
            w2c = _weight(w2, dt)
            c1 = cin + growth
            if growth == 32 and _fused_3x3_ok(z, w2c):
                a2 = None
                dense_conv3x3_fwd(z, g2, b2, m2, r2, w2c, buf[:, cin:c1], eps1[min(l + 1, L - 1)],
                                  stats.mean[cin:c1], stats.var[cin:c1], stats.rstd[cin:c1])
            else:
                from . import conv_generic as cg
                a2 = torch.empty_like(z, memory_format=CL)
                bn_act_fwd(z, g2, b2, m2, r2, True, a2)
                _, cols2 = cg.conv_fwd(a2, w2c, 1, 1, out=buf[:, cin:c1], want_cols=True)
                kept_cols[l] = cols2
                bn_stats(buf[:, cin:c1], stats.mean[cin:c1], stats.var[cin:c1], stats.rstd[cin:c1], eps1[min(l + 1, L - 1)])
            saved += [a if a is not None else buf.new_empty(0), z, a2 if a2 is not None else buf.new_empty(0)]
            wcast += [w1c, w2c]
        ctx.save_for_backward(buf, *saved, *wcast)
        ctx.kept_cols = kept_cols
        ctx.params = params
        ctx.meta = (stats, growth, bn2_stats, L, C0)
        ctx.cap = None
        if CAPTURE_BLOCKS is not None:
            ctx.cap = {"buf": buf, "C0": C0, "growth": growth, "params": params, "wcast": wcast,
                       "mean": stats.mean, "rstd": stats.rstd, "var": stats.var, "z": saved[1::3], "bn2": bn2_stats}
            CAPTURE_BLOCKS.append(ctx.cap)
        return buf

    @staticmethod
    def backward(ctx, gbuf):
        stats, growth, bn2_stats, L, C0 = ctx.meta
        t = ctx.saved_tensors
        buf = t[0]
        dev = buf.device
        B, _, H, W = buf.shape
        params = ctx.params
        saved = t[1: 1 + 3 * L]
        wcast = t[1 + 3 * L:]
        if not gbuf.is_contiguous(memory_format=CL):
            gbuf = dense_cl(gbuf)
        if ctx.cap is not None:
            ctx.cap["gin"] = gbuf.clone(memory_format=CL)
            ctx.cap["dz"] = [None] * L
            ctx.cap["dyc"] = [None] * L
            ctx.cap["gbuf"] = gbuf
        grads = [None] * (6 * L)
        stamp(f"bwd block {buf.shape[2]}x{buf.shape[3]} start (main)")
        if getattr(ctx, "persistent", False) and _block_bwd_persistent_ok(buf, gbuf, params, L):
            zs = [saved[3 * l + 1] for l in range(L)]
            dzs, dycs = dense_block_bwd_persistent(buf, gbuf, params, wcast, zs, stats, bn2_stats, C0, L)
            if ctx.cap is not None:
                ctx.cap["dz"] = list(dzs)
                ctx.cap["dyc"] = list(dycs)
            gw1s = {}

            def _weight_grads():
                for l in range(L - 1, -1, -1):
                    g1, b1, w1, g2, b2, w2 = params[6 * l: 6 * l + 6]
                    cin = C0 + l * growth
                    m2, v2, r2 = bn2_stats[l]
                    ok = dense_conv3x3_wrw(dycs[l], zs[l], g2, b2, m2, r2, w2)
                    assert ok
                    gw1s[l] = conv1x1_wrw(dzs[l], buf[:, :cin], w1, bn=(g1, b1, stats.mean[:cin], stats.rstd[:cin]))
                if STAMPS:
                    stamp(f"bwd block {buf.shape[2]}x{buf.shape[3]} weight gradients done (side)")

            joins = buf.shape[0] * buf.shape[2] * buf.shape[3] >= JOIN_MIN_PIXELS or ctx.first_block
            lanes = USE_SIDE_STREAM and all(_direct_all(params[6 * l + 2]) and params[6 * l + 2].grad.is_contiguous()
                                            for l in range(L))
            _side_fork(dev, _weight_grads, (gbuf, buf, *dzs, *dycs, *zs), lanes=lanes, defer=True)
            if not lanes:
                for l in range(L):
                    grads[6 * l + 2] = gw1s[l]
            if STAMPS:
                stamp(f"bwd block {buf.shape[2]}x{buf.shape[3]} end (main)")
            if joins:
                _side_join(dev)
                stamp(f"bwd block {buf.shape[2]}x{buf.shape[3]} after join (main)")
            return (gbuf[:, :C0], None, *grads)
        kacc = None
        pair_a = None
        pair_cin = 0

        def flush_pair():
            nonlocal pair_a
            if pair_a is not None:
                dzA, wA, gA, bA, cA = pair_a
                dense_bn1_dx(dzA, wA, buf[:, :pair_cin], gA, bA, stats.mean[:pair_cin], stats.rstd[:pair_cin], cA,
                             gbuf[:, :pair_cin], window=(0, pair_cin - growth))
                pair_a = None

        def gram_dx(opens_pair, dz, w1c, g1, b1, cin, coef):
            nonlocal pair_a, pair_cin
            mine = (dz, w1c, g1, b1, coef)
            if pair_a is not None:
                dense_bn1_dx_pair(pair_a, mine, buf[:, :cin], stats.mean[:cin], stats.rstd[:cin], gbuf[:, :cin])
                pair_a = None
            elif opens_pair:
                dense_bn1_dx(dz, w1c, buf[:, :cin], g1, b1, stats.mean[:cin], stats.rstd[:cin], coef, gbuf[:, :cin],
                             window=(cin - growth, growth))
                pair_a, pair_cin = mine, cin
            else:
                dense_bn1_dx(dz, w1c, buf[:, :cin], g1, b1, stats.mean[:cin], stats.rstd[:cin], coef, gbuf[:, :cin])
        for l in range(L - 1, -1, -1):
            g1, b1, w1, g2, b2, w2 = params[6 * l: 6 * l + 6]
            a, z, a2 = saved[3 * l: 3 * l + 3]
            w1c, w2c = wcast[2 * l: 2 * l + 2]
            cin = C0 + l * growth
            c1 = cin + growth
            m2, v2, r2 = bn2_stats[l]
            x, gx, mean1, rstd1 = buf[:, :cin], gbuf[:, :cin], stats.mean[:cin], stats.rstd[:cin]
            dy_view = gbuf[:, cin:c1]
            d2 = _direct_all(g2, b2)
            d1 = _direct_all(g1, b1)
            fused1 = a.numel() == 0
            fused2 = a2.numel() == 0 and _fused_3x3_ok(z, w2c)
            plan = _plan_layer(l, cin, growth, B, H, W, fused1, fused2, fused1 and _bn1_wrw_ok(w1),
                               fused2 and _wrw3_direct_ok(w2, z, dy_view), kacc is not None, USE_SIDE_STREAM,
                               USE_BN1_SINGLE_PASS, BN1_SINGLE_PASS_MAX_MAP, FUSED_BN1_WRW_MIN_PIXELS)
            fold = None
            if plan.fix == "fold":
                fold = (buf[:, cin:c1], stats.mean[cin:c1], stats.rstd[cin:c1], kacc[cin:c1])
            elif plan.fix == "launch_32":
                dense_bn1_fix(buf, gbuf, cin, growth, stats.mean, stats.rstd, kacc)
            elif plan.fix == "launch_all":
                dense_bn1_fix(buf, gbuf, 0, c1, stats.mean, stats.rstd, kacc)
                kacc = None
            dw2 = None
            if plan.conv2 == "own":
                dz, dg2, db2, dyc = dense_conv3x3_bwd(dy_view, w2c, z, g2, b2, m2, r2, into_param_grads=d2, fix=fold)
            else:
                dyc = None
                if a2.numel() == 0:
                    a2 = torch.empty_like(z, memory_format=CL)
                    bn_act_fwd(z, g2, b2, m2, r2, True, a2)
                da2, dw2 = _conv_bwd(dy_view, a2, w2c, w2, 1, ctx.kept_cols.pop(l, None))
                dz = torch.empty_like(z, memory_format=CL)
                dg2, db2 = bn_act_bwd(dense_cl(da2), z, g2, b2, m2, r2, True, dz, False, into_param_grads=d2)
            dy_w = dyc if dyc is not None else dy_view
            if ctx.cap is not None:
                ctx.cap["dz"][l] = dz
                ctx.cap["dyc"][l] = dyc
            ev = _fork_event(dev) if plan.lanes else None
            if plan.conv1 != "gram":
                flush_pair()
            gw1 = None
            if plan.conv1 == "gram":
                dg1, db1, coef = dense_bn1_wrw(dz, w1c, x, g1, b1, mean1, rstd1, w1, into_param_grads=d1)
                gram_dx(plan.opens_pair, dz, w1c, g1, b1, cin, coef)
            elif plan.conv1 == "single":
                have_prev = kacc is not None
                if not have_prev:
                    kacc = torch.empty((buf.shape[1], 2), device=dev, dtype=torch.float32)
                dg1, db1 = dense_bn1_dx_sums(dz, w1c, x, g1, b1, mean1, rstd1, gx, kacc, have_prev, into_param_grads=d1)
            elif plan.conv1 == "two_pass":
                dg1, db1 = dense_bn1_bwd(dz, w1c, x, g1, b1, mean1, rstd1, gx, into_param_grads=d1)
            else:
                da, dw1 = _conv1x1_bwd(dz, a, w1c, w1)
                dg1, db1 = bn_act_bwd(da, x, g1, b1, mean1, rstd1, True, gx, True, into_param_grads=d1)
                gw1 = None if dw1 is None else _wgrad(w1, dw1)

            def weight_grads():
                if plan.conv2 == "own":
                    done = dense_conv3x3_wrw(dy_w, z, g2, b2, m2, r2, w2)
                    assert done
                if plan.conv1 in ("single", "two_pass"):
                    return conv1x1_wrw(dz, x, w1, bn=(g1, b1, mean1, rstd1))
                return gw1

            gw1 = _side_fork(dev, weight_grads, (dz, gbuf, z, buf, dy_w), lanes=plan.lanes, event=ev)
            grads[6 * l: 6 * l + 6] = [dg1, db1, gw1, dg2, db2, None if dw2 is None else _wgrad(w2, dw2)]
        flush_pair()
        if kacc is not None:
            dense_bn1_fix(buf, gbuf, 0, C0, stats.mean, stats.rstd, kacc)
        if STAMPS:
            stamp(f"bwd block {buf.shape[2]}x{buf.shape[3]} end (main)")
            if USE_SIDE_STREAM:
                with torch.cuda.stream(_side_stream(buf.device)):
                    stamp(f"bwd block {buf.shape[2]}x{buf.shape[3]} weight gradients done (side)")
        if buf.shape[0] * buf.shape[2] * buf.shape[3] >= JOIN_MIN_PIXELS or ctx.first_block:
            _side_join(buf.device)
            stamp(f"bwd block {buf.shape[2]}x{buf.shape[3]} after join (main)")
        return (gbuf[:, :C0], None, *grads)


def _bn_train(x: Tensor, bn: nn.BatchNorm2d, relu: bool, rec: _RunningStats) -> Tensor:
    C = x.shape[1]
    mean = torch.empty(C, device=x.device, dtype=torch.float32)
    var = torch.empty_like(mean)
    rstd = torch.empty_like(mean)
    x = dense_cl(x)
    bn_stats(x, mean, var, rstd, bn.eps)
    rec.add(bn, mean, var, x.numel() // C)
    return BNActFn.apply(x, bn.weight, bn.bias, mean, rstd, relu)


def dense_block(blk: nn.Module, x: Tensor, rec: _RunningStats, stats: Optional[_BlockStats] = None,
                force_join: bool = False) -> Tuple[Tensor, _BlockStats]:
    layers = list(blk.values())
    growth = layers[0].conv2.out_channels
    C0 = x.shape[1]
    Ct = C0 + len(layers) * growth
    prefilled = stats is not None
    if stats is None:
        stats = _BlockStats(Ct, x.device)
    bott = layers[0].conv1.out_channels
    bn2 = [tuple(torch.empty(bott, device=x.device, dtype=torch.float32) for _ in range(3)) for _ in layers]
    params = []
    for ly in layers:
        params += [ly.norm1.weight, ly.norm1.bias, ly.conv1.weight, ly.norm2.weight, ly.norm2.bias, ly.conv2.weight]
    meta = (stats, [ly.norm1.eps for ly in layers], [ly.norm2.eps for ly in layers], growth, bn2, prefilled, force_join)
    buf = DenseBlockFn.apply(x, meta, *params)
    n = x.shape[0] * x.shape[2] * x.shape[3]
    for i, ly in enumerate(layers):
        cin = C0 + i * growth
        rec.add(ly.norm1, stats.mean[:cin], stats.var[:cin], n)
        rec.add(ly.norm2, bn2[i][0], bn2[i][1], n)
    return buf, stats




def _conv0_ok(x: Tensor, conv: nn.Conv2d) -> bool:
    B, C, H, W = x.shape
    return (x.is_cuda and x.dtype == torch.bfloat16 and C == 3 and H % 4 == 0 and W % 8 == 0
            and W <= 256 and x.is_contiguous(memory_format=CL) and tuple(conv.weight.shape) == (64, 3, 7, 7)
            and conv.stride == (2, 2) and conv.padding == (3, 3) and conv.bias is None and not x.requires_grad)


def conv0_fwd(x: Tensor, w16: Tensor, eps: float, stats: Optional[Tuple[Tensor, Tensor, Tensor]]) -> Tensor:
    B, _, H, W = x.shape
    y = torch.empty((B, 64, H // 2, W // 2), device=x.device, dtype=torch.bfloat16, memory_format=CL)
    L = _lib.lib()
    ws = _ws(L.mcl_conv0_workspace_floats(B, H, W), x.device)
    st = (None, None, None) if stats is None else tuple(t.data_ptr() for t in stats)
    check(L.mcl_conv0_fwd(x.data_ptr(), B, H, W, w16.data_ptr(), y.data_ptr(), ws.data_ptr(), eps, *st, _stream()),
          "mcl_conv0_fwd")
    return y


class Conv0Fn(torch.autograd.Function):

    @staticmethod
    def forward(ctx, x, w, meta):
        eps, stats = meta
        w16 = _weight(w, x.dtype)
        y = conv0_fwd(x, w16, eps, stats)
        ctx.save_for_backward(x, w16)
        ctx.w = w
        ctx.cap = None
        if CAPTURE_MISC is not None:
            ctx.cap = {"kind": "conv0", "x": x, "w16": w16, "y": y, "stats": stats, "w": w}
            CAPTURE_MISC.append(ctx.cap)
        return y

    @staticmethod
    def backward(ctx, dy):
        x, w16 = ctx.saved_tensors
        dy = dense_cl(dy)
        w = ctx.w
        if ctx.cap is not None:
            ctx.cap["dy"] = dy
        B, _, H, W = x.shape
        if _direct_all(w) and dy.dtype == torch.bfloat16:
            L = _lib.lib()
            ws = _ws(L.mcl_conv0_wrw_workspace_floats(B, H, W), x.device)
            tgt, in_place = _grad_target_khwc(w)
            check(L.mcl_conv0_wrw(x.data_ptr(), B, H, W, dy.data_ptr(), ws.data_ptr(), tgt.data_ptr(), int(in_place),
                                  _stream()), "mcl_conv0_wrw")
            _grad_finish_khwc(w, tgt, in_place)
            return None, None, None
        from . import conv_generic as cg
        dw = cg.conv_bwd_weight(dy, x, ctx.w, 2, 3)
        return None, (None if dw is None else dw.to(ctx.w.dtype)), None




def _pool_ok(x: Tensor, even: bool) -> bool:
    return (x.is_cuda and x.dtype == torch.bfloat16 and x.dim() == 4 and x.shape[1] % 8 == 0
            and x.is_contiguous(memory_format=CL) and (not even or (x.shape[2] % 2 == 0 and x.shape[3] % 2 == 0)))


class AvgPool2Fn(torch.autograd.Function):

    @staticmethod
    def forward(ctx, x):
        B, C, H, W = x.shape
        y = torch.empty((B, C, H // 2, W // 2), device=x.device, dtype=x.dtype, memory_format=CL)
        check(_lib.lib().mcl_avgpool2_nhwc_bf16(x.data_ptr(), y.data_ptr(), B, H, W, C, 0, _stream()), "mcl_avgpool2")
        ctx.shape = (B, C, H, W)
        return y

    @staticmethod
    def backward(ctx, dy):
        B, C, H, W = ctx.shape
        dy = dense_cl(dy)
        dx = torch.empty((B, C, H, W), device=dy.device, dtype=dy.dtype, memory_format=CL)
        check(_lib.lib().mcl_avgpool2_nhwc_bf16(dy.data_ptr(), dx.data_ptr(), B, H, W, C, 1, _stream()), "mcl_avgpool2")
        return dx


class MaxPool3s2Fn(torch.autograd.Function):

    @staticmethod
    def forward(ctx, x):
        B, C, H, W = x.shape
        y = torch.empty((B, C, (H - 1) // 2 + 1, (W - 1) // 2 + 1), device=x.device, dtype=x.dtype, memory_format=CL)
        idx = torch.empty((B, y.shape[2], y.shape[3], C), device=x.device, dtype=torch.uint8)
        check(_lib.lib().mcl_maxpool3s2_nhwc_bf16_fwd(x.data_ptr(), y.data_ptr(), idx.data_ptr(), B, H, W, C, _stream()),
              "mcl_maxpool")
        ctx.save_for_backward(idx)
        ctx.shape = (B, C, H, W)
        return y

    @staticmethod
    def backward(ctx, dy):
        (idx,) = ctx.saved_tensors
        B, C, H, W = ctx.shape
        dy = dense_cl(dy)
        dx = torch.empty((B, C, H, W), device=dy.device, dtype=dy.dtype, memory_format=CL)
        check(_lib.lib().mcl_maxpool3s2_nhwc_bf16_bwd(idx.data_ptr(), dy.data_ptr(), dx.data_ptr(), B, H, W, C, _stream()),
              "mcl_maxpool bwd")
        return dx


class StemTailFn(torch.autograd.Function):

    @staticmethod
    def forward(ctx, x, gamma, beta, mean, rstd):
        B, C, H, W = x.shape
        y = torch.empty((B, C, (H - 1) // 2 + 1, (W - 1) // 2 + 1), device=x.device, dtype=x.dtype, memory_format=CL)
        idx = torch.empty((B, y.shape[2], y.shape[3], C), device=x.device, dtype=torch.uint8)
        check(_lib.lib().mcl_bn_act_maxpool_fwd(x.data_ptr(), B, H, W, C, gamma.data_ptr(), beta.data_ptr(),
                                                mean.data_ptr(), rstd.data_ptr(), y.data_ptr(), idx.data_ptr(),
                                                _stream()), "mcl_bn_act_maxpool_fwd")
        ctx.save_for_backward(x, idx, mean, rstd)
        ctx.params = (gamma, beta)
        ctx.cap = None
        if CAPTURE_MISC is not None:
            ctx.cap = {"kind": "stem_tail", "x": x, "y": y, "mean": mean, "rstd": rstd, "params": (gamma, beta)}
            CAPTURE_MISC.append(ctx.cap)
        return y

    @staticmethod
    def backward(ctx, dy):
        x, idx, mean, rstd = ctx.saved_tensors
        gamma, beta = ctx.params
        B, C, H, W = x.shape
        pdy, _, Cd, lddy = _rows(dy)
        assert Cd == C and dy.dtype == x.dtype
        if ctx.cap is not None:
            ctx.cap["dy"] = dy.clone(memory_format=CL)
        g = torch.empty_like(x, memory_format=CL)
        check(_lib.lib().mcl_maxpool3s2_nhwc_bf16_bwd_ld(idx.data_ptr(), pdy, lddy, g.data_ptr(), B, H, W, C, _stream()),
              "mcl_maxpool bwd")
        direct = _direct_all(gamma, beta)
        dg, db = bn_act_bwd(g, x, gamma, beta, mean, rstd, True, g, False, into_param_grads=direct)
        if ctx.cap is not None:
            ctx.cap["dx"] = g
        return g, dg, db, None, None




def _stem_tail_ok(x: Tensor) -> bool:
    return _pool_ok(x, False) and x.shape[1] <= 2048


def max_pool_3s2(x: Tensor) -> Tensor:
    if _pool_ok(x, False):
        return MaxPool3s2Fn.apply(x)
    from . import conv_generic as cg
    return cg.max_pool_3s2(x)


def avg_pool_2(x: Tensor) -> Tensor:
    if _pool_ok(x, True):
        return AvgPool2Fn.apply(x)
    from . import conv_generic as cg
    return cg.avg_pool_2(x)


_ident_cache = {}


def _identity_bn(device) -> Tuple[Tensor, Tensor]:
    v = _ident_cache.get(device.index)
    if v is None:
        v = (torch.ones(1024, device=device, dtype=torch.float32), torch.zeros(1024, device=device, dtype=torch.float32))
        _ident_cache[device.index] = v
    return v


def bn_act_avgpool_fwd(x: Tensor, gamma: Tensor, beta: Tensor, mean: Tensor, rstd: Tensor) -> Tensor:
    B, C, H, W = x.shape
    px, S, _, ld = _rows(x)
    p = torch.empty((B, C, H // 2, W // 2), device=x.device, dtype=x.dtype, memory_format=CL)
    check(_lib.lib().mcl_bn_act_avgpool_fwd(px, ld, B, H, W, C, gamma.data_ptr(), beta.data_ptr(), mean.data_ptr(),
                                            rstd.data_ptr(), p.data_ptr(), C, _stream()), "mcl_bn_act_avgpool_fwd")
    return p


def pooled_conv1x1_fwd(p: Tensor, w16: Tensor, eps: float, stats: Optional[_BlockStats], out: Optional[Tensor] = None
                       ) -> Tensor:
    B, C, H, W = p.shape
    Co = w16.shape[0]
    y = out if out is not None else torch.empty((B, Co, H, W), device=p.device, dtype=p.dtype, memory_format=CL)
    py, Sy, Cy, ldy = _rows(y)
    one, zero = _identity_bn(p.device)
    pp, S, _, ldp = _rows(p)
    assert (Sy, Cy) == (S, Co) and y.dtype == p.dtype
    L = _lib.lib()
    ws = _ws(L.mcl_dense_conv1x1_workspace_floats(S), p.device)
    for n0 in range(0, Co, 128):
        st = (None, None, None) if stats is None else tuple(t.data_ptr() + 4 * n0 for t in (stats.mean, stats.var, stats.rstd))
        check(L.mcl_dense_conv1x1_fwd(pp, ldp, S, C, one.data_ptr(), zero.data_ptr(), zero.data_ptr(), one.data_ptr(),
                                      w16.data_ptr() + 2 * n0 * C, py + 2 * n0, ldy, ws.data_ptr(), eps,
                                      *st, _stream()), "mcl_dense_conv1x1_fwd (transition)")
    return y


def _transition_ok(buf: Tensor, w: Tensor) -> bool:
    B, C, H, W = buf.shape
    return (buf.is_cuda and buf.dtype == torch.bfloat16 and H >= 2
            and W >= 2 and C % 8 == 0 and C <= 1024 and w.shape[0] % 128 == 0 and w.shape[1] == C
            and buf.is_contiguous(memory_format=CL))


class TransitionFn(torch.autograd.Function):

    @staticmethod
    def forward(ctx, buf, gamma, beta, w, meta):
        stats, next_stats, eps_next = meta
        p = bn_act_avgpool_fwd(buf, gamma, beta, stats.mean, stats.rstd)
        w16 = _weight(w, buf.dtype)
        nbuf = getattr(next_stats, "buf", None)
        out = nbuf[:, :w16.shape[0]] if nbuf is not None else None
        y = pooled_conv1x1_fwd(p, w16, eps_next, next_stats, out=out)
        ctx.save_for_backward(buf, p, w16)
        ctx.params = (gamma, beta, w)
        ctx.stats = stats
        ctx.cap = None
        if CAPTURE_MISC is not None:
            ctx.cap = {"kind": "transition", "buf": buf, "p": p, "w16": w16, "y": y, "stats": stats, "next_stats": next_stats,
                       "params": (gamma, beta, w), "eps_next": eps_next}
            CAPTURE_MISC.append(ctx.cap)
        return y

    @staticmethod
    def backward(ctx, dy):
        buf, p, w16 = ctx.saved_tensors
        gamma, beta, w = ctx.params
        stats = ctx.stats
        B, C, H, W = buf.shape
        Co = w16.shape[0]
        _rows(dy)
        lanes = USE_SIDE_STREAM and _direct_all(w) and w.grad.is_contiguous()
        ev = _fork_event(buf.device) if lanes else None
        pdy, Sq, Co_, lddy = _rows(dy)
        assert Co_ == Co and dy.dtype == torch.bfloat16
        dp = torch.empty((B, C, dy.shape[2], dy.shape[3]), device=buf.device, dtype=torch.bfloat16, memory_format=CL)
        check(_lib.lib().mcl_gemm_bf16(pdy, lddy, 0, w16.data_ptr(), C, 0, dp.data_ptr(), C, 0, Sq, C, Co, 1, 1, 0, 0, 0,
                                       1.0, 2, None, None, 0, 0, None, 0, None, 0, 1, None, 0, _stream()),
              "mcl_gemm_bf16 (transition backward-data)")
        dx = torch.empty_like(buf, memory_format=CL)
        direct = _direct_all(gamma, beta)
        if direct:
            dg, db = gamma.grad, beta.grad
        else:
            dg = torch.empty(C, device=buf.device, dtype=torch.float32)
            db = torch.empty(C, device=buf.device, dtype=torch.float32)
        L = _lib.lib()
        ws = _ws(L.mcl_bn_workspace_floats(B * H * W, C, 1), buf.device)
        check(L.mcl_bn_act_avgpool_bwd(dp.data_ptr(), C, buf.data_ptr(), C, B, H, W, C, gamma.data_ptr(),
                                       beta.data_ptr(), stats.mean.data_ptr(), stats.rstd.data_ptr(), ws.data_ptr(),
                                       dg.data_ptr(), db.data_ptr(), int(direct), dx.data_ptr(), C, _stream()),
              "mcl_bn_act_avgpool_bwd")
        dw = _side_fork(buf.device, lambda: conv1x1_wrw(dy, p, w), (dy, p), lanes=lanes, event=ev)
        gw = None if dw is None else dw.view_as(w).to(w.dtype)
        if ctx.cap is not None:
            ctx.cap.update({"dy": dy, "dp": dp, "dx": dx.clone(memory_format=CL)})
        return dx, (None if direct else dg), (None if direct else db), gw, None


class BNGlobalPoolFn(torch.autograd.Function):

    @staticmethod
    def forward(ctx, x, gamma, beta, mean, rstd):
        B, C, H, W = x.shape
        px, S, _, ld = _rows(x)
        out = torch.empty((B, C), device=x.device, dtype=torch.float32)
        xm = torch.empty((B, C), device=x.device, dtype=torch.float32)
        check(_lib.lib().mcl_bn_gap_fwd(px, ld, B, H * W, C, gamma.data_ptr(), beta.data_ptr(), mean.data_ptr(),
                                        rstd.data_ptr(), out.data_ptr(), xm.data_ptr(), _stream()), "mcl_bn_gap_fwd")
        ctx.save_for_backward(x, xm, mean, rstd)
        ctx.params = (gamma, beta)
        ctx.cap = None
        if CAPTURE_MISC is not None:
            ctx.cap = {"kind": "norm5_pool", "x": x, "out": out, "mean": mean, "rstd": rstd, "params": (gamma, beta)}
            CAPTURE_MISC.append(ctx.cap)
        return out

    @staticmethod
    def backward(ctx, g):
        x, xm, mean, rstd = ctx.saved_tensors
        gamma, beta = ctx.params
        B, C, H, W = x.shape
        g = g.contiguous()
        if g.dtype != torch.float32:
            g = g.float()
        px, S, _, ld = _rows(x)
        dx = torch.empty_like(x, memory_format=CL)
        direct = _direct_all(gamma, beta)
        if direct:
            dg, db = gamma.grad, beta.grad
        else:
            dg = torch.empty(C, device=x.device, dtype=torch.float32)
            db = torch.empty(C, device=x.device, dtype=torch.float32)
        coef = torch.empty(2 * C, device=x.device, dtype=torch.float32)
        check(_lib.lib().mcl_bn_gap_bwd(g.data_ptr(), xm.data_ptr(), px, ld, B, H * W, C, gamma.data_ptr(), mean.data_ptr(),
                                        rstd.data_ptr(), coef.data_ptr(), dg.data_ptr(), db.data_ptr(), int(direct),
                                        dx.data_ptr(), C, _stream()), "mcl_bn_gap_bwd")
        if ctx.cap is not None:
            ctx.cap.update({"g": g, "dx": dx.clone(memory_format=CL)})
        return dx, (None if direct else dg), (None if direct else db), None, None


def _gap_ok(buf: Tensor) -> bool:
    return (buf.is_cuda and buf.dtype == torch.bfloat16 and buf.dim() == 4 and buf.shape[1] % 8 == 0
            and buf.is_contiguous(memory_format=CL))


def image_to_act(x: Tensor, act_dtype: torch.dtype, out: Optional[Tensor] = None) -> Tensor:
    if (act_dtype == torch.bfloat16 and x.is_cuda and x.dtype == torch.float32 and x.dim() == 4 and not x.requires_grad
            and x.numel() > 0):
        B, C, H, W = x.shape
        if out is not None:
            assert out.shape == x.shape and out.dtype == torch.bfloat16 and out.is_contiguous(memory_format=CL)
            y = out
        else:
            y = torch.empty((B, C, H, W), device=x.device, dtype=torch.bfloat16, memory_format=CL)
        sb, sc, sy, sx = x.stride()
        check(_lib.lib().mcl_image_to_bf16_nhwc(x.data_ptr(), sb, sc, sy, sx, B, C, H, W, y.data_ptr(), _stream()),
              "mcl_image_to_bf16_nhwc")
        return y
    y = x.to(dtype=act_dtype).contiguous(memory_format=CL)
    if out is not None:
        out.copy_(y)
        return out
    return y


_cut_anchors = {}


def _cut_anchor(device) -> Tensor:
    a = _cut_anchors.get(device.index)
    if a is None:
        a = torch.zeros(1, device=device, requires_grad=True)
        _cut_anchors[device.index] = a
    return a


class _CutFn(torch.autograd.Function):
    @staticmethod
    def forward(ctx, x, anchor, slot):
        ctx.slot = slot
        return x.view_as(x)

    @staticmethod
    def backward(ctx, g):
        ctx.slot["grad"] = g
        return None, None, None


FORWARD_BLOCK_HOOKS: dict = {}


def densenet_features_fused(features: nn.Sequential, x: Tensor, act_dtype: torch.dtype = torch.bfloat16,
                            pooled: bool = False, cuts: Optional[list] = None, cut_blocks=()) -> Tensor:
    if not x.is_cuda:
        raise RuntimeError("densenet_features_fused: input is on the CPU; the fused backbone path is GPU-only")
    rec = _RunningStats()
    x = image_to_act(x, act_dtype)
    own_conv0 = _conv0_ok(x, features.conv0)
    if own_conv0:
        mean0, var0, rstd0 = (torch.empty(64, device=x.device, dtype=torch.float32) for _ in range(3))
        x = Conv0Fn.apply(x, features.conv0.weight, (features.norm0.eps, (mean0, var0, rstd0)))
    else:
        from . import conv_generic as cg
        x = cg.conv2d(x, features.conv0.weight, features.conv0.stride[0], features.conv0.padding[0])
    x = dense_cl(x)
    if _stem_tail_ok(x):
        C0 = x.shape[1]
        if not own_conv0:
            mean0, var0, rstd0 = (torch.empty(C0, device=x.device, dtype=torch.float32) for _ in range(3))
            bn_stats(x, mean0, var0, rstd0, features.norm0.eps)
        rec.add(features.norm0, mean0, var0, x.numel() // C0)
        x = StemTailFn.apply(x, features.norm0.weight, features.norm0.bias, mean0, rstd0)
    else:
        x = _bn_train(x, features.norm0, True, rec)
        x = max_pool_3s2(dense_cl(x))
    i = 1
    out = None
    next_stats = None
    cut_here = False
    while hasattr(features, f"denseblock{i}"):
        buf, stats = dense_block(getattr(features, f"denseblock{i}"), x, rec, next_stats, force_join=cut_here)
        stamp(f"fwd block {i} done (main)")
        hook = FORWARD_BLOCK_HOOKS.get(i)
        if hook is not None:
            hook()
        next_stats = None
        n = buf.shape[0] * buf.shape[2] * buf.shape[3]
        if hasattr(features, f"transition{i}"):
            tr = getattr(features, f"transition{i}")
            rec.add(tr.norm, stats.mean, stats.var, n)
            nxt = list(getattr(features, f"denseblock{i + 1}").values()) if hasattr(features, f"denseblock{i + 1}") else None
            if nxt is not None and _transition_ok(buf, tr.conv.weight):
                co = tr.conv.weight.shape[0]
                next_stats = _BlockStats(co + len(nxt) * nxt[0].conv2.out_channels, buf.device)
                next_stats.buf = torch.empty((buf.shape[0], next_stats.mean.numel(), buf.shape[2] // 2, buf.shape[3] // 2),
                                             device=buf.device, dtype=buf.dtype, memory_format=CL)
                x = TransitionFn.apply(buf, tr.norm.weight, tr.norm.bias, tr.conv.weight,
                                       (stats, next_stats, nxt[0].norm1.eps))
                cut_here = cuts is not None and (i + 1) in cut_blocks and x.requires_grad
                if cut_here:
                    slot = {}
                    cuts.append((x, slot))
                    x = _CutFn.apply(x.detach(), _cut_anchor(x.device), slot)
            else:
                from . import conv_generic as cg
                a = BNActFn.apply(buf, tr.norm.weight, tr.norm.bias, stats.mean, stats.rstd, True)
                x = avg_pool_2(cg.conv2d(a, tr.conv.weight, 1, 0))
        else:
            if pooled and _gap_ok(buf):
                out = BNGlobalPoolFn.apply(buf, features.norm5.weight, features.norm5.bias, stats.mean, stats.rstd)
            else:
                out = BNActFn.apply(buf, features.norm5.weight, features.norm5.bias, stats.mean, stats.rstd, False)
                if pooled:
                    from . import conv_generic as _cg
                    out = _cg.global_avg_pool(out)
            rec.add(features.norm5, stats.mean, stats.var, n)
        i += 1
    rec.flush()
    return out


@torch.no_grad()
def eval_rstd(bns) -> List[Tensor]:
    import ctypes as C
    if not bns:
        return []
    dev = bns[0].running_var.device
    sizes = [bn.running_var.numel() for bn in bns]
    flat = torch.empty(sum(sizes), device=dev, dtype=torch.float32)
    outs, o = [], 0
    for n in sizes:
        outs.append(flat[o:o + n])
        o += n
    for bn in bns:
        if bn.running_var.dtype != torch.float32 or not bn.running_var.is_contiguous():
            raise RuntimeError("eval_rstd: running statistics must be contiguous fp32")
    n = len(bns)
    vp = C.c_void_p * n
    check(_lib.lib().mcl_bn_eval_rstd(n, vp(*[bn.running_var.data_ptr() for bn in bns]), vp(*[t.data_ptr() for t in outs]),
                                      (C.c_int32 * n)(*sizes), (C.c_float * n)(*[float(bn.eps) for bn in bns]), _stream()),
          "mcl_bn_eval_rstd")
    return outs


def densenet_features_eval(features: nn.Sequential, x: Tensor, act_dtype: torch.dtype = torch.bfloat16,
                           pooled: bool = False) -> Tensor:
    if not x.is_cuda:
        raise RuntimeError("densenet_features_eval: input is on the CPU; the fused backbone path is GPU-only")
    if act_dtype not in (torch.bfloat16, torch.float32):
        raise RuntimeError("densenet_features_eval: activations are bf16 (fused kernels) or fp32 (generic own-kernel path)")
    bns = [m for m in features.modules() if isinstance(m, nn.BatchNorm2d)]
    rs = {id(bn): r for bn, r in zip(bns, eval_rstd(bns))}

    def affine(t: Tensor, bn: nn.BatchNorm2d, relu: bool) -> Tensor:
        t = dense_cl(t)
        out = torch.empty_like(t, memory_format=CL)
        bn_act_fwd(t, bn.weight, bn.bias, bn.running_mean, rs[id(bn)], relu, out)
        return out

    def copy_into(dst: Tensor, src: Tensor) -> None:
        one, zero = _identity_bn(src.device)
        C = src.shape[1]
        bn_act_fwd(src, one[:C], zero[:C], zero[:C], one[:C], False, dst)

    x = image_to_act(x, act_dtype)
    if _conv0_ok(x, features.conv0):
        x = conv0_fwd(x, _weight(features.conv0.weight, act_dtype), features.norm0.eps, None)
    else:
        from . import conv_generic as cg
        x = cg.conv_fwd(x, _weight(features.conv0.weight, act_dtype), features.conv0.stride[0], features.conv0.padding[0])
    if not x.is_contiguous(memory_format=CL):
        raise RuntimeError("densenet_features_eval: the stem convolution must produce a channels-last tensor")
    if _stem_tail_ok(x):
        x = StemTailFn.apply(x, features.norm0.weight, features.norm0.bias, features.norm0.running_mean,
                             rs[id(features.norm0)])
    else:
        x = max_pool_3s2(affine(x, features.norm0, True))
    i = 1
    out = None
    pre = None
    while hasattr(features, f"denseblock{i}"):
        layers = list(getattr(features, f"denseblock{i}").values())
        growth = layers[0].conv2.out_channels
        B, C0, H, W = x.shape
        if pre is not None:
            buf = pre
        else:
            buf = torch.empty((B, C0 + len(layers) * growth, H, W), device=x.device, dtype=act_dtype, memory_format=CL)
            copy_into(buf[:, :C0], x)
        pre = None
        for l, ly in enumerate(layers):
            cin = C0 + l * growth
            w1c, w2c = _weight(ly.conv1.weight, act_dtype), _weight(ly.conv2.weight, act_dtype)
            if growth == 32 and _fused_1x1_ok(buf, w1c) and w1c.shape[0] == 128:
                z = dense_conv1x1_fwd(buf[:, :cin], ly.norm1.weight, ly.norm1.bias, ly.norm1.running_mean,
                                      rs[id(ly.norm1)], w1c, ly.norm2.eps, None, None, None)
                dense_conv3x3_fwd(z, ly.norm2.weight, ly.norm2.bias, ly.norm2.running_mean, rs[id(ly.norm2)], w2c,
                                  buf[:, cin:cin + growth], ly.norm1.eps, None, None, None)
            else:
                from . import conv_generic as cg
                a = torch.empty((B, cin, H, W), device=x.device, dtype=act_dtype, memory_format=CL)
                bn_act_fwd(buf[:, :cin], ly.norm1.weight, ly.norm1.bias, ly.norm1.running_mean, rs[id(ly.norm1)], True, a)
                z = affine(_conv1x1_fwd(a, w1c), ly.norm2, True)
                cg.conv_fwd(z, w2c, 1, 1, out=buf[:, cin:cin + growth])
        if hasattr(features, f"transition{i}"):
            tr = getattr(features, f"transition{i}")
            nxt = getattr(features, f"denseblock{i + 1}", None)
            Co = tr.conv.weight.shape[0]
            Hn, Wn = buf.shape[2] // 2, buf.shape[3] // 2
            if nxt is not None:
                nl = list(nxt.values())
                pre = torch.empty((buf.shape[0], Co + len(nl) * nl[0].conv2.out_channels, Hn, Wn), device=buf.device,
                                  dtype=act_dtype, memory_format=CL)
            if _transition_ok(buf, tr.conv.weight):
                p = bn_act_avgpool_fwd(buf, tr.norm.weight, tr.norm.bias, tr.norm.running_mean, rs[id(tr.norm)])
                x = pooled_conv1x1_fwd(p, _weight(tr.conv.weight, act_dtype), tr.norm.eps, None,
                                       out=None if pre is None else pre[:, :Co])
            else:
                from . import conv_generic as cg
                a = affine(buf, tr.norm, True)
                x = avg_pool_2(cg.conv_fwd(a, _weight(tr.conv.weight, act_dtype), 1, 0))
                if pre is not None:
                    copy_into(pre[:, :Co], x)
                    x = pre[:, :Co]
        elif pooled and _gap_ok(buf):
            bn = features.norm5
            B, C, H, W = buf.shape
            out = torch.empty((B, C), device=buf.device, dtype=torch.float32)
            check(_lib.lib().mcl_bn_gap_fwd(buf.data_ptr(), C, B, H * W, C, bn.weight.data_ptr(), bn.bias.data_ptr(),
                                            bn.running_mean.data_ptr(), rs[id(bn)].data_ptr(), out.data_ptr(), None,
                                            _stream()), "mcl_bn_gap_fwd")
        else:
            out = affine(buf, features.norm5, False)
            if pooled:
                from . import conv_generic as cg
                out = cg.global_avg_pool(out)
        i += 1
    return out
```

### mclstexp_amd/kernel_costs.py

```python
from __future__ import annotations


def _conv1x1_wrw_det(a):
    S, M, N = a[11], a[12], a[13]
    return 2 * S * (M + N) + 4 * M * N


def _conv1x1_wrw_det_flops(a):
    return 2 * a[11] * a[12] * a[13]


def _conv3x3_wrw_det(a):
    S = a[3]
    return 2 * S * (32 + 128) + 4 * 32 * 1152


def _conv3x3_flops_S3(a):
    return 2 * a[3] * 32 * 1152


def _bn1_bwd(a):
    C, S = a[2], a[5]
    return 2 * S * (128 + C) + 2 * S * (128 + 3 * C)


def _bn1_bwd_strict(a):
    C, S = a[2], a[5]
    return 2 * S * (128 + 3 * C)


def _bn1_flops(a):
    return 2 * a[5] * 128 * a[2]


def _conv3x3_bwd(a):
    S = a[2]
    return 2 * S * (32 + 128 + 128) + 2 * S * (128 + 128 + 128)


def _conv3x3_bwd_strict(a):
    return 2 * a[2] * (32 + 128 + 128)


def _conv3x3_flops_S2(a):
    return 2 * a[2] * 32 * 1152


def _conv3x3_bwd_fix(a):
    return _conv3x3_bwd(a) + 2 * a[2] * (32 + 32)


def _conv3x3_bwd_fix_strict(a):
    return _conv3x3_bwd_strict(a) + 2 * a[2] * (32 + 32)


def _conv1x1_fwd(a):
    S, K = a[2], a[3]
    return 2 * S * (K + 128)


def _conv1x1_fwd_flops(a):
    return 2 * a[2] * a[3] * 128


def _conv3x3_fwd(a):
    S = a[1]
    return 2 * S * (128 + 32)


def _conv3x3_flops_S1(a):
    return 2 * a[1] * 32 * 1152


def _bn1_wrw(a):
    C, S = a[2], a[5]
    return 2 * S * (128 + C) + 4 * 128 * C


def _bn1_wrw_flops(a):
    return 2 * 2 * a[5] * 128 * a[2]


def _bn1_dx(a):
    C, S = a[2], a[5]
    return 2 * S * (128 + 3 * C)


def _bn1_dx_window(a):
    nc, S = a[4], a[7]
    return 2 * S * (128 + 3 * nc)


def _bn1_dx_window_flops(a):
    return 2 * a[7] * 128 * a[4]


def _bn1_dx_pair(a):
    C, S = a[11], a[14]
    return 2 * S * (2 * 128 + 3 * C)


def _bn1_dx_pair_flops(a):
    return 2 * 2 * a[14] * 128 * a[11]


def _bn1_dx_sums(a):
    C, S = a[2], a[5]
    return 2 * S * (128 + 3 * C)


def _bn1_fix(a):
    return 2 * a[4] * 3 * a[6]


def _adam_table(a):
    return 24 * a[3] * a[4]


def _adam_table_lazy(a):
    tables = 2 if a[4] else 1
    return tables * a[13] * a[9] * (24 + (4 if a[14] else 0))


def _block_fwd(a):
    B, HW, Ct, C0, L = a[1], a[2] * a[3], a[4], a[5], a[6]
    w = sum(128 * (C0 + 32 * l) * 2 for l in range(L)) + L * 32 * 1152 * 2
    return 2 * B * HW * C0 + L * 2 * B * HW * 128 + 2 * B * HW * 32 * L + w


def _block_fwd_flops(a):
    B, HW, C0, L = a[1], a[2] * a[3], a[5], a[6]
    return sum(2 * B * HW * (128 * (C0 + 32 * l) + 1152 * 32) for l in range(L))


def _block_bwd(a):
    B, HW, Ct, C0, L = a[2], a[3] * a[4], a[5], a[6], a[7]
    w = sum(128 * (C0 + 32 * l) * 2 for l in range(L)) + L * 32 * 1152 * 2
    return 2 * 2 * B * HW * Ct + 2 * B * HW * C0 + L * 2 * B * HW * (128 + 128 + 32) + w


def _block_bwd_flops(a):
    B, HW, C0, L = a[2], a[3] * a[4], a[6], a[7]
    return sum(2 * B * HW * (128 * (C0 + 32 * l) + 1152 * 32) for l in range(L))


def _adam(a):
    return 28 * a[4]


def _adam_shadow(a):
    return 30 * a[4]


def _zero(a):
    return 0


def _e(kernels, b, strict=None, flops=_zero, bound=None, unit=None):
    return {"kernels": kernels, "bytes": b, "strict": strict or b, "flops": flops, "bound": bound, "unit": unit}


TABLE = {
    "mcl_conv1x1_wrw_det": _e("wrw_partial_kernel + wrw_merge_kernel", _conv1x1_wrw_det, flops=_conv1x1_wrw_det_flops),
    "mcl_dense_conv3x3_wrw_det": _e("conv3x3_wrw_rows_kernel (56x56, 28x28 maps) / conv3x3_wrw_ky_kernel + wrw_merge_kernel",
                                    _conv3x3_wrw_det, flops=_conv3x3_flops_S3,
                                    bound="mfma/lds"),
    "mcl_dense_bn1_wrw": _e("wrw_partial_kernel<Gram> + wrw_merge_kernel", _bn1_wrw, flops=_bn1_wrw_flops),
    "mcl_dense_bn1_dx": _e("bn1_bwd_kernel<1> (one layer) / bn1_dx_pair_kernel (two consecutive layers' passes as one: "
                           "mcl_dense_bn1_dx_pair, preceded by the 32-channel mcl_dense_bn1_dx_window)", _bn1_dx, flops=_bn1_flops),
    "mcl_dense_bn1_dx_window": _e("bn1_bwd_kernel<1> on a 32-channel window", _bn1_dx_window, flops=_bn1_dx_window_flops,
                                  unit="mcl_dense_bn1_dx"),
    "mcl_dense_bn1_dx_pair": _e("bn1_dx_pair_kernel", _bn1_dx_pair, flops=_bn1_dx_pair_flops, unit="mcl_dense_bn1_dx"),
    "mcl_dense_bn1_dx_sums": _e("bn1_bwd_kernel<2> (single pass: dx data term + previous layer's mean terms + sums) + "
                                "bn1_bwd_finalize_kernel", _bn1_dx_sums, flops=_bn1_flops),
    "mcl_dense_bn1_fix": _e("bn1_fix_kernel", _bn1_fix, bound="latency"),
    "mcl_dense_bn1_bwd": _e("bn1_bwd_kernel<0> + bn1_bwd_finalize_kernel + bn1_bwd_kernel<1>", _bn1_bwd, _bn1_bwd_strict,
                            flops=lambda a: 2 * _bn1_flops(a)),
    "mcl_dense_conv3x3_bwd": _e("conv3x3_bwd_rows_kernel (56x56, 28x28 maps) / conv3x3_bwd_kernel (14x14, 7x7; with the "
                                "folded bn1_fix as mcl_dense_conv3x3_bwd_fix) + bn1_bwd_finalize_kernel + bn2_dz_kernel",
                                _conv3x3_bwd, _conv3x3_bwd_strict, flops=_conv3x3_flops_S2, bound="mfma/lds"),
    "mcl_dense_conv3x3_bwd_fix": _e("conv3x3_bwd_kernel (folded bn1_fix) + bn1_bwd_finalize_kernel + bn2_dz_kernel",
                                    _conv3x3_bwd_fix, _conv3x3_bwd_fix_strict, flops=_conv3x3_flops_S2, bound="mfma/lds",
                                    unit="mcl_dense_conv3x3_bwd"),
    "mcl_dense_conv1x1_fwd": _e("conv1x1_fwd_kernel + tile_stats_finalize_kernel", _conv1x1_fwd, flops=_conv1x1_fwd_flops),
    "mcl_dense_conv3x3_fwd": _e("conv3x3_fwd_rows_kernel + sums_finalize_kernel (56x56, 28x28 maps) / conv3x3_fwd_kernel + "
                                "tile_stats_finalize_kernel", _conv3x3_fwd, flops=_conv3x3_flops_S1, bound="mfma/lds"),
    "mcl_adam_table_step_dev": _e("adam_table_kernel", _adam_table, bound="hbm"),
    "mcl_dense_block_fwd": _e("dense_block_fwd_kernel (a whole 7x7 dense block forward: one persistent launch, in-launch batch-statistics "
                              "seams) + zero_words_kernel", _block_fwd, flops=_block_fwd_flops, bound="latency"),
    "mcl_dense_block_bwd": _e("dense_block_bwd_kernel (the block's data-gradient chain: one persistent launch) + zero_words_kernel",
                              _block_bwd, flops=_block_bwd_flops, bound="latency"),
    "mcl_adam_table_lazy": _e("adam_table_lazy_kernel (catch-up of gathered rows / update of the rows with a gradient)",
                              _adam_table_lazy, bound="latency"),
    "mcl_adam_step_dev": _e("adam_kernel", _adam, bound="hbm"),
    "mcl_adam_step_dev_shadow": _e("adam_kernel<shadow> (update + bf16 shadow of the parameters)", _adam_shadow, bound="hbm"),
}
```

Measured before the change: 12320 spots/s.

## Fuse stem BN/ReLU backward dx into conv0 weight-gradient staging

The stem's norm0/relu0 backward is split: a sums-only pass computes dgamma/dbeta and the coefficients, and the per-element dx is formed inside a new conv0 weight-gradient kernel while it stages dy into LDS. This skips the separate act_bwd_dx pass, which wrote the full-resolution stem gradient and had the wrw kernel read it back. StemTailFn and Conv0Fn coordinate through a shared link dict, which adds cross-autograd coupling and a runtime consistency check.

```diff
diff --git a/include/mclstexp_hip.h b/include/mclstexp_hip.h
--- a/include/mclstexp_hip.h
+++ b/include/mclstexp_hip.h
@@ -192,6 +192,10 @@
                    const float* gamma, const float* beta, const float* mean, const float* rstd, int32_t relu,
                    float* workspace, float* dgamma, float* dbeta, int32_t accumulate_params, void* dx, int64_t lddx,
                    int32_t accumulate, mcl_stream_t stream);
+int mcl_bn_act_bwd_sums(const void* dy, int64_t lddy, const void* x, int64_t ldx, int64_t S, int32_t C, int32_t dtype,
+                        const float* gamma, const float* beta, const float* mean, const float* rstd, int32_t relu,
+                        float* workspace, float* dgamma, float* dbeta, int32_t accumulate_params, float* coef,
+                        mcl_stream_t stream);
 
 int64_t mcl_dense_conv1x1_workspace_floats(int64_t S);
 int mcl_dense_conv1x1_fwd(const void* x, int64_t ldx, int64_t S, int32_t K, const float* gamma, const float* beta,
@@ -272,6 +276,9 @@
 int64_t mcl_conv0_wrw_workspace_floats(int32_t N, int32_t H, int32_t W);
 int mcl_conv0_wrw(const void* x, int32_t N, int32_t H, int32_t W, const void* dy, float* workspace, float* dW,
                   int32_t accumulate_w, mcl_stream_t stream);
+int mcl_conv0_wrw_bnrelu(const void* x, int32_t N, int32_t H, int32_t W, const void* g, const void* z, const float* gamma,
+                         const float* beta, const float* mean, const float* rstd, const float* coef, float* workspace,
+                         float* dW, int32_t accumulate_w, mcl_stream_t stream);
 
 int mcl_bn_act_maxpool_fwd(const void* x, int32_t N, int32_t H, int32_t W, int32_t C, const float* gamma,
                            const float* beta, const float* mean, const float* rstd, void* y, void* idx,
diff --git a/mclstexp_amd/_lib.py b/mclstexp_amd/_lib.py
--- a/mclstexp_amd/_lib.py
+++ b/mclstexp_amd/_lib.py
@@ -144,6 +144,7 @@
     "mcl_bn_stats": [c_p, c_l, c_l, c_i, c_i, c_p, c_l, c_p, c_f, c_p, c_p, c_p, c_p],
     "mcl_bn_act_fwd": [c_p, c_l, c_l, c_i, c_i, c_p, c_p, c_p, c_p, c_i, c_p, c_l, c_p],
     "mcl_bn_act_bwd": [c_p, c_l, c_p, c_l, c_l, c_i, c_i, c_p, c_p, c_p, c_p, c_i, c_p, c_p, c_p, c_i, c_p, c_l, c_i, c_p],
+    "mcl_bn_act_bwd_sums": [c_p, c_l, c_p, c_l, c_l, c_i, c_i, c_p, c_p, c_p, c_p, c_i, c_p, c_p, c_p, c_i, c_p, c_p],
     "mcl_dense_conv1x1_workspace_floats": [c_l],
     "mcl_dense_conv1x1_fwd": [c_p, c_l, c_l, c_i, c_p, c_p, c_p, c_p, c_p, c_p, c_l, c_p, c_f, c_p, c_p, c_p, c_p],
     "mcl_dense_conv3x3_workspace_floats": [c_l],
@@ -190,6 +191,7 @@
     "mcl_conv0_fwd": [c_p, c_i, c_i, c_i, c_p, c_p, c_p, c_f, c_p, c_p, c_p, c_p],
     "mcl_conv0_wrw_workspace_floats": [c_i, c_i, c_i],
     "mcl_conv0_wrw": [c_p, c_i, c_i, c_i, c_p, c_p, c_p, c_i, c_p],
+    "mcl_conv0_wrw_bnrelu": [c_p, c_i, c_i, c_i, c_p, c_p, c_p, c_p, c_p, c_p, c_p, c_p, c_p, c_i, c_p],
     "mcl_bn_act_maxpool_fwd": [c_p, c_i, c_i, c_i, c_i, c_p, c_p, c_p, c_p, c_p, c_p, c_p],
     "mcl_patch_gather": [c_p, c_i, c_i, c_p, c_i, c_i, c_p, c_f, c_p, c_p, c_p],
     "mcl_her2st_train_patches": [c_p, c_i, c_i, c_p, c_i, c_i, c_p, c_f, c_p, c_p, c_p],
diff --git a/mclstexp_amd/csrc/bnrelu.hip b/mclstexp_amd/csrc/bnrelu.hip
--- a/mclstexp_amd/csrc/bnrelu.hip
+++ b/mclstexp_amd/csrc/bnrelu.hip
@@ -356,9 +356,7 @@
 #pragma unroll
     for (int i = 0; i < V; ++i) {
       if (POOL) g[i] = pr >= 0 ? g[i] * 0.25f : 0.0f;
-      const float gi = (relu && fmaf(f[i], sc[i], sh[i]) <= 0.0f) ? 0.0f : g[i];
-      const float xh = (f[i] - mu[i]) * rs[i];
-      const float d = sc[i] * (gi - c1[i] - xh * c2[i]);
+      const float d = bn_act_bwd_elem(f[i], g[i], relu, sc[i], sh[i], mu[i], rs[i], c1[i], c2[i]);
       o[i] = accumulate ? o[i] + d : d;
     }
     Vec<T>::store(dx + r * lddx + (long long)cv * V, o);
@@ -451,6 +449,21 @@
   return MCL_OK;
 }
 
+static void launch_act_bwd_sums(const void* dy, int64_t lddy, const void* x, int64_t ldx, int64_t S, int32_t C, int32_t dtype,
+                                const float* gamma, const float* beta, const float* mean, const float* rstd, int32_t relu,
+                                float* workspace, int nblk, int rpb, int tiles, float* dgamma, float* dbeta,
+                                int32_t accumulate_params, float* coef, hipStream_t st) {
+  dim3 grid(nblk, tiles);
+  if (dtype == 1)
+    hipLaunchKernelGGL(act_bwd_reduce_kernel<bf16_t>, grid, dim3(NTH), 0, st, (const bf16_t*)dy, (long long)lddy,
+                       (const bf16_t*)x, (long long)ldx, (long long)S, C, gamma, beta, mean, rstd, relu, workspace, rpb);
+  else
+    hipLaunchKernelGGL(act_bwd_reduce_kernel<float>, grid, dim3(NTH), 0, st, (const float*)dy, (long long)lddy,
+                       (const float*)x, (long long)ldx, (long long)S, C, gamma, beta, mean, rstd, relu, workspace, rpb);
+  hipLaunchKernelGGL(act_bwd_finalize_kernel, dim3((C + 3) / 4), dim3(256), 0, st, workspace, nblk, C, (long long)S,
+                     dgamma, dbeta, coef, accumulate_params);
+}
+
 extern "C" int mcl_bn_act_bwd(const void* dy, int64_t lddy, const void* x, int64_t ldx, int64_t S, int32_t C,
                               int32_t dtype, const float* gamma, const float* beta, const float* mean,
                               const float* rstd, int32_t relu, float* workspace, float* dgamma, float* dbeta,
@@ -467,23 +480,33 @@
   dim3 grid(nblk, tiles);
   hipStream_t st = mcl_stream(stream);
   float* coef = workspace + (long long)nblk * 2 * C;
-  if (dtype == 1) {
-    hipLaunchKernelGGL(act_bwd_reduce_kernel<bf16_t>, grid, dim3(NTH), 0, st, (const bf16_t*)dy, (long long)lddy,
-                       (const bf16_t*)x, (long long)ldx, (long long)S, C, gamma, beta, mean, rstd, relu, workspace, rpb);
-    hipLaunchKernelGGL(act_bwd_finalize_kernel, dim3((C + 3) / 4), dim3(256), 0, st, workspace, nblk, C,
-                       (long long)S, dgamma, dbeta, coef, accumulate_params);
+  launch_act_bwd_sums(dy, lddy, x, ldx, S, C, dtype, gamma, beta, mean, rstd, relu, workspace, nblk, rpb, tiles, dgamma,
+                      dbeta, accumulate_params, coef, st);
+  if (dtype == 1)
     hipLaunchKernelGGL(act_bwd_dx_kernel<bf16_t>, grid, dim3(NTH), 0, st, (const bf16_t*)dy, (long long)lddy,
                        (const bf16_t*)x, (long long)ldx, (long long)S, C, gamma, beta, mean, rstd, relu, coef,
                        (bf16_t*)dx, (long long)lddx, accumulate, rpb);
-  } else {
-    hipLaunchKernelGGL(act_bwd_reduce_kernel<float>, grid, dim3(NTH), 0, st, (const float*)dy, (long long)lddy,
-                       (const float*)x, (long long)ldx, (long long)S, C, gamma, beta, mean, rstd, relu, workspace, rpb);
-    hipLaunchKernelGGL(act_bwd_finalize_kernel, dim3((C + 3) / 4), dim3(256), 0, st, workspace, nblk, C,
-                       (long long)S, dgamma, dbeta, coef, accumulate_params);
+  else
     hipLaunchKernelGGL(act_bwd_dx_kernel<float>, grid, dim3(NTH), 0, st, (const float*)dy, (long long)lddy,
                        (const float*)x, (long long)ldx, (long long)S, C, gamma, beta, mean, rstd, relu, coef,
                        (float*)dx, (long long)lddx, accumulate, rpb);
-  }
+  MCL_CHECK_LAUNCH();
+  return MCL_OK;
+}
+
+extern "C" int mcl_bn_act_bwd_sums(const void* dy, int64_t lddy, const void* x, int64_t ldx, int64_t S, int32_t C,
+                                   int32_t dtype, const float* gamma, const float* beta, const float* mean,
+                                   const float* rstd, int32_t relu, float* workspace, float* dgamma, float* dbeta,
+                                   int32_t accumulate_params, float* coef, mcl_stream_t stream) {
+  MCL_CLEAR_ERROR();
+  if (!gamma || !beta || !mean || !rstd || !workspace || !dgamma || !dbeta || !coef || S <= 0 || C <= 0 ||
+      (dtype != 0 && dtype != 1))
+    return MCL_EINVAL;
+  if (!ok_layout(dy, lddy, C, dtype) || !ok_layout(x, ldx, C, dtype)) return MCL_EUNSUPPORTED;
+  int nblk, rpb, tiles;
+  plan(S, C, dtype, &nblk, &rpb, &tiles);
+  launch_act_bwd_sums(dy, lddy, x, ldx, S, C, dtype, gamma, beta, mean, rstd, relu, workspace, nblk, rpb, tiles, dgamma,
+                      dbeta, accumulate_params, coef, mcl_stream(stream));
   MCL_CHECK_LAUNCH();
   return MCL_OK;
 }
diff --git a/mclstexp_amd/csrc/dense_conv.hip b/mclstexp_amd/csrc/dense_conv.hip
--- a/mclstexp_amd/csrc/dense_conv.hip
+++ b/mclstexp_amd/csrc/dense_conv.hip
@@ -873,6 +873,51 @@
   }
 }
 
+__device__ __forceinline__ void c0_wrw_slab_chunk(bf16_t* d, uint4 v, bool ok) {
+  const unsigned wv[4] = {ok ? v.x : 0u, ok ? v.y : 0u, ok ? v.z : 0u, ok ? v.w : 0u};
+#pragma unroll
+  for (int i = 0; i < 4; ++i) {
+    d[2 * i] = (bf16_t)(wv[i] & 0xFFFFu);
+    d[2 * i + 1] = (bf16_t)(wv[i] >> 16);
+  }
+}
+__device__ __forceinline__ void c0_wrw_mma(const unsigned char* dyt, const bf16_t* slab, int PW, int OWp, unsigned a_off, int h,
+                                           const int (&koff)[3], f32x16 (&acc)[3]) {
+  for (int p0 = 0; p0 < 2 * OWp; p0 += 16) {
+    const int rr = p0 / OWp, ox0 = p0 - rr * OWp;
+    const unsigned char* ap = dyt + (p0 + 8 * h) * 128 + a_off;
+    const v4s alo = __builtin_amdgcn_ds_read_tr16_b64_v4i16((v4s __attribute__((address_space(3)))*)(ap));
+    const v4s ahi = __builtin_amdgcn_ds_read_tr16_b64_v4i16((v4s __attribute__((address_space(3)))*)(ap + 4 * 128));
+    bf16x8 a;
+    a[0] = alo[0]; a[1] = alo[1]; a[2] = alo[2]; a[3] = alo[3];
+    a[4] = ahi[0]; a[5] = ahi[1]; a[6] = ahi[2]; a[7] = ahi[3];
+    const bf16_t* brow = slab + (2 * rr) * PW + 6 * (ox0 + 8 * h);
+#pragma unroll
+    for (int t = 0; t < 3; ++t) {
+      const bf16_t* bp = brow + koff[t];
+      bf16x8 b;
+#pragma unroll
+      for (int i = 0; i < 8; ++i) b[i] = (short)bp[6 * i];
+      acc[t] = __builtin_amdgcn_mfma_f32_32x32x16_bf16(a, b, acc[t], 0, 0, 0);
+    }
+  }
+}
+__device__ __forceinline__ void c0_wrw_store_partial(float* __restrict__ wpart, const f32x16 (&acc)[3], const bool (&kval)[3],
+                                                     int mt, int kt0, int h, int l31) {
+#pragma unroll
+  for (int t = 0; t < 3; ++t) {
+    if (!kval[t]) continue;
+    const int k = (kt0 + t) * 32 + l31;
+    const int ky = k / C0_KP, j = k % C0_KP;
+    float* dst = wpart + (long long)blockIdx.x * (C0_OUT * C0_K * 21);
+#pragma unroll
+    for (int r = 0; r < 16; ++r) {
+      const int co = mt * 32 + (r & 3) + 8 * (r >> 2) + 4 * h;
+      dst[(co * C0_K + ky) * 21 + j] = acc[t][r];
+    }
+  }
+}
+
 __global__ __launch_bounds__(256, 2) void conv0_wrw_kernel(const bf16_t* __restrict__ x, int N, int H, int W,
                                                            const bf16_t* __restrict__ dy, float* __restrict__ dW,
                                                            int ntile, float* __restrict__ wpart) {
@@ -941,48 +986,136 @@
       if (c < 9 * cpr) {
         const int r = c / cpr, cc = c % cpr;
         bf16_t* d = slab + r * PW + 9 + cc * 8;
-        const bool ok = (xvalid >> u) & 1u;
-        const unsigned wv[4] = {ok ? rx[u].x : 0u, ok ? rx[u].y : 0u, ok ? rx[u].z : 0u, ok ? rx[u].w : 0u};
-#pragma unroll
-        for (int i = 0; i < 4; ++i) {
-          d[2 * i] = (bf16_t)(wv[i] & 0xFFFFu);
-          d[2 * i + 1] = (bf16_t)(wv[i] >> 16);
-        }
+        c0_wrw_slab_chunk(d, rx[u], (xvalid >> u) & 1u);
       }
     }
     __syncthreads();
 
-    for (int p0 = 0; p0 < 2 * OWp; p0 += 16) {
-      const int rr = p0 / OWp, ox0 = p0 - rr * OWp;
-      const unsigned char* ap = dyt + (p0 + 8 * h) * 128 + a_off;
-      const v4s alo = __builtin_amdgcn_ds_read_tr16_b64_v4i16((v4s __attribute__((address_space(3)))*)(ap));
-      const v4s ahi = __builtin_amdgcn_ds_read_tr16_b64_v4i16((v4s __attribute__((address_space(3)))*)(ap + 4 * 128));
-      bf16x8 a;
-      a[0] = alo[0]; a[1] = alo[1]; a[2] = alo[2]; a[3] = alo[3];
-      a[4] = ahi[0]; a[5] = ahi[1]; a[6] = ahi[2]; a[7] = ahi[3];
-      const bf16_t* brow = slab + (2 * rr) * PW + 6 * (ox0 + 8 * h);
-#pragma unroll
-      for (int t = 0; t < 3; ++t) {
-        const bf16_t* bp = brow + koff[t];
-        bf16x8 b;
-#pragma unroll
-        for (int i = 0; i < 8; ++i) b[i] = (short)bp[6 * i];
-        acc[t] = __builtin_amdgcn_mfma_f32_32x32x16_bf16(a, b, acc[t], 0, 0, 0);
-      }
-    }
-  }
+    c0_wrw_mma(dyt, slab, PW, OWp, a_off, h, koff, acc);
+  }
+  c0_wrw_store_partial(wpart, acc, kval, mt, kt0, h, l31);
+}
+
+template <int NDY, int NX>
+__global__ __launch_bounds__(256, 2) void conv0_wrw_bnrelu_kernel(const bf16_t* __restrict__ x, int N, int H, int W,
+                                                                  const bf16_t* __restrict__ g, const bf16_t* __restrict__ z,
+                                                                  const float* __restrict__ gamma, const float* __restrict__ beta,
+                                                                  const float* __restrict__ mean, const float* __restrict__ rstd,
+                                                                  const float* __restrict__ coef, int ntile,
+                                                                  float* __restrict__ wpart) {
+  extern __shared__ __attribute__((aligned(16))) unsigned char lds[];
+  const int OH = H >> 1, OW = W >> 1;
+  const int PW = (W + 6) * 3 + 8;
+  const int OWp = (OW + 15) & ~15;
+  const int npix = 2 * OW;
+  bf16_t* slab = reinterpret_cast<bf16_t*>(lds);
+  const int slab_bytes = (9 * PW * 2 + 15) & ~15;
+  unsigned char* dyt = lds + slab_bytes;
+  float* tab = reinterpret_cast<float*>(dyt + 2 * OWp * 128);
+  const int tid = threadIdx.x, lane = tid & 63, wave = tid >> 6;
+  const int h = lane >> 5, l31 = lane & 31;
+  const int mt = wave & 1, kt0 = (wave >> 1) * 3;
+  int koff[3];
+  bool kval[3];
 #pragma unroll
   for (int t = 0; t < 3; ++t) {
-    if (!kval[t]) continue;
     const int k = (kt0 + t) * 32 + l31;
     const int ky = k / C0_KP, j = k % C0_KP;
-    float* dst = wpart + (long long)blockIdx.x * (C0_OUT * C0_K * 21);
-#pragma unroll
-    for (int r = 0; r < 16; ++r) {
-      const int co = mt * 32 + (r & 3) + 8 * (r >> 2) + 4 * h;
-      dst[(co * C0_K + ky) * 21 + j] = acc[t][r];
-    }
-  }
+    kval[t] = k < 7 * C0_KP && j < 21;
+    koff[t] = kval[t] ? ky * PW + j : 0;
+  }
+  f32x16 acc[3];
+#pragma unroll
+  for (int t = 0; t < 3; ++t)
+#pragma unroll
+    for (int r = 0; r < 16; ++r) acc[t][r] = 0.0f;
+  for (int i = tid; i < (slab_bytes + 2 * OWp * 128) / 16; i += 256) reinterpret_cast<uint4*>(lds)[i] = make_uint4(0u, 0u, 0u, 0u);
+  if (tid < C0_OUT) {
+    const float mu = mean[tid], rs = rstd[tid];
+    const float sc = gamma[tid] * rs;
+    float* t = tab + (tid >> 3) * 48 + ((tid & 7) >> 1) * 12 + (tid & 1);
+    t[0] = sc;
+    t[2] = fmaf(-mu, sc, beta[tid]);
+    t[4] = mu;
+    t[6] = rs;
+    t[8] = coef[2 * tid];
+    t[10] = coef[2 * tid + 1];
+  }
+  const int i16 = lane & 15, q4 = i16 >> 2;
+  const int lch = (mt * 32 + 16 * ((lane >> 4) & 1)) / 8 + ((i16 & 3) >> 1);
+  const unsigned a_off = (unsigned)(q4 * 128 + ((lch ^ (((q4 >> 1) & 1) << 2)) << 4) + (i16 & 1) * 8);
+  const int c8 = tid & 7;
+  const float4* ktab = reinterpret_cast<const float4*>(tab + c8 * 48);
+
+  const int cpr = (W * 6) >> 4;
+  u32x4 rg[NDY], rz[NDY];
+  uint4 rx[NX];
+  unsigned xvalid = 0;
+  auto request = [&](int tile) {
+    const int n = tile / (OH >> 1), oy0 = (tile % (OH >> 1)) * 2;
+    const long long o = ((long long)(n * OH + oy0) * OW) * C0_OUT;
+    const unsigned char* gb = reinterpret_cast<const unsigned char*>(g + o);
+    const unsigned char* zb = reinterpret_cast<const unsigned char*>(z + o);
+    const int t = opaque_lane(tid);
+#pragma unroll
+    for (int u = 0; u < NDY; ++u) {
+      const unsigned off = (unsigned)min(t + 256 * u, npix * 8 - 1) * 16u;
+      rg[u] = *reinterpret_cast<const u32x4*>(gb + off);
+      rz[u] = *reinterpret_cast<const u32x4*>(zb + off);
+    }
+    const unsigned char* xb = reinterpret_cast<const unsigned char*>(x + (long long)n * H * W * 3);
+    xvalid = 0;
+#pragma unroll
+    for (int u = 0; u < NX; ++u) {
+      const int c = min(t + 256 * u, 9 * cpr - 1);
+      const int r = c / cpr, cc = c % cpr;
+      const int iy = 2 * oy0 - 3 + r;
+      xvalid |= (iy >= 0 && iy < H) ? (1u << u) : 0u;
+      rx[u] = *reinterpret_cast<const uint4*>(xb + (unsigned)((min(max(iy, 0), H - 1) * W * 3 + cc * 8) * 2));
+    }
+  };
+
+  int tile = blockIdx.x;
+  request(tile);
+  for (;;) {
+    __syncthreads();
+#pragma unroll
+    for (int i = 0; i < 4; ++i) {
+      const float4 k0 = ktab[3 * i], k1 = ktab[3 * i + 1], k2 = ktab[3 * i + 2];
+#pragma unroll
+      for (int u = 0; u < NDY; ++u) {
+        const unsigned wg = rg[u][i], wz = rz[u][i];
+        const float d0 = bn_act_bwd_elem(bf_lo(wz), bf_lo(wg), 1, k0.x, k0.z, k1.x, k1.z, k2.x, k2.z);
+        const float d1 = bn_act_bwd_elem(bf_hi(wz), bf_hi(wg), 1, k0.y, k0.w, k1.y, k1.w, k2.y, k2.w);
+        rg[u][i] = f2bf_rne(d0) | (f2bf_rne(d1) << 16);
+      }
+    }
+    const int ts = opaque_lane(tid);
+#pragma unroll
+    for (int u = 0; u < NDY; ++u) {
+      const int c = ts + 256 * u;
+      if (c < npix * 8) {
+        const int px = c >> 3;
+        const int pc = px < OW ? px : px - OW + OWp;
+        *reinterpret_cast<u32x4*>(dyt + pc * 128 + (((c & 7) ^ (((pc >> 1) & 1) << 2)) << 4)) = rg[u];
+      }
+    }
+#pragma unroll
+    for (int u = 0; u < NX; ++u) {
+      const int c = ts + 256 * u;
+      if (c < 9 * cpr) {
+        const int r = c / cpr, cc = c % cpr;
+        c0_wrw_slab_chunk(slab + r * PW + 9 + cc * 8, rx[u], (xvalid >> u) & 1u);
+      }
+    }
+    const int nx = tile + (int)gridDim.x;
+    if (nx < ntile) request(nx);
+    __syncthreads();
+    c0_wrw_mma(dyt, slab, PW, OWp, a_off, h, koff, acc);
+    if (nx >= ntile) break;
+    tile = nx;
+  }
+  c0_wrw_store_partial(wpart, acc, kval, mt, kt0, h, l31);
 }
 
 }
@@ -1054,3 +1187,38 @@
   MCL_CHECK_LAUNCH();
   return MCL_OK;
 }
+
+extern "C" int mcl_conv0_wrw_bnrelu(const void* x, int32_t N, int32_t H, int32_t W, const void* g, const void* z,
+                                    const float* gamma, const float* beta, const float* mean, const float* rstd,
+                                    const float* coef, float* workspace, float* dW, int32_t accumulate_w,
+                                    mcl_stream_t stream) {
+  MCL_CLEAR_ERROR();
+  if (!x || !g || !z || !gamma || !beta || !mean || !rstd || !coef || !dW || !workspace || N <= 0 || H <= 0 || W <= 0)
+    return MCL_EINVAL;
+  if ((H % 4) || (W % 8) || W > 256 || (reinterpret_cast<uintptr_t>(x) & 15u) || (reinterpret_cast<uintptr_t>(g) & 15u) ||
+      (reinterpret_cast<uintptr_t>(z) & 15u) || (reinterpret_cast<uintptr_t>(workspace) & 15u) ||
+      (reinterpret_cast<uintptr_t>(dW) & 15u))
+    return MCL_EUNSUPPORTED;
+  const int OH = H / 2, OW = W / 2, OWp = (OW + 15) & ~15;
+  const int ntile = N * (OH / 2);
+  const int PW = (W + 6) * 3 + 8;
+  const size_t lds_bytes = (size_t)((9 * PW * 2 + 15) & ~15) + (size_t)2 * OWp * 128 + C0_OUT * 6 * sizeof(float);
+  static mcl_device_once attr_once;
+  if (auto attr_guard = attr_once.first()) {
+    (void)hipFuncSetAttribute(reinterpret_cast<const void*>(conv0_wrw_bnrelu_kernel<7, 3>),
+                              hipFuncAttributeMaxDynamicSharedMemorySize, 96 * 1024);
+    (void)hipFuncSetAttribute(reinterpret_cast<const void*>(conv0_wrw_bnrelu_kernel<8, 4>),
+                              hipFuncAttributeMaxDynamicSharedMemorySize, 96 * 1024);
+  }
+  hipStream_t st = mcl_stream(stream);
+  const int grid = conv0_wrw_grid(ntile);
+  if (W <= 224)
+    hipLaunchKernelGGL((conv0_wrw_bnrelu_kernel<7, 3>), dim3(grid), dim3(256), lds_bytes, st, (const bf16_t*)x, N, H, W,
+                       (const bf16_t*)g, (const bf16_t*)z, gamma, beta, mean, rstd, coef, ntile, workspace);
+  else
+    hipLaunchKernelGGL((conv0_wrw_bnrelu_kernel<8, 4>), dim3(grid), dim3(256), lds_bytes, st, (const bf16_t*)x, N, H, W,
+                       (const bf16_t*)g, (const bf16_t*)z, gamma, beta, mean, rstd, coef, ntile, workspace);
+  mcl_launch_wrw_merge(workspace, grid, (long long)C0_OUT * C0_K * 21, dW, accumulate_w, st);
+  MCL_CHECK_LAUNCH();
+  return MCL_OK;
+}
diff --git a/mclstexp_amd/csrc/device.h b/mclstexp_amd/csrc/device.h
--- a/mclstexp_amd/csrc/device.h
+++ b/mclstexp_amd/csrc/device.h
@@ -60,6 +60,13 @@
   return make_uint4(w[0], w[1], w[2], w[3]);
 }
 
+__device__ __forceinline__ float bn_act_bwd_elem(float f, float g, int relu, float sc, float sh, float mu, float rs, float c1,
+                                                 float c2) {
+  const float gi = (relu && fmaf(f, sc, sh) <= 0.0f) ? 0.0f : g;
+  const float xh = (f - mu) * rs;
+  return sc * (gi - c1 - xh * c2);
+}
+
 template <typename T>
 __device__ __forceinline__ double ldd(const T* p) { return (double)*p; }
 
diff --git a/mclstexp_amd/densenet_fused.py b/mclstexp_amd/densenet_fused.py
--- a/mclstexp_amd/densenet_fused.py
+++ b/mclstexp_amd/densenet_fused.py
@@ -1093,11 +1093,17 @@
     return y
 
 
+FUSED_STEM_BWD = True
+
+
 class Conv0Fn(torch.autograd.Function):
 
     @staticmethod
     def forward(ctx, x, w, meta):
-        eps, stats = meta
+        eps, stats = meta[0], meta[1]
+        ctx.link = meta[2] if len(meta) > 2 else None
+        if ctx.link is not None:
+            ctx.link["w"] = w
         w16 = _weight(w, x.dtype)
         y = conv0_fwd(x, w16, eps, stats)
         ctx.save_for_backward(x, w16)
@@ -1116,6 +1122,20 @@
         if ctx.cap is not None:
             ctx.cap["dy"] = dy
         B, _, H, W = x.shape
+        bn = ctx.link.pop("bn", None) if ctx.link is not None else None
+        if bn is not None:
+            g, z0, gamma, beta, mean, rstd, coef = bn
+            if dy.data_ptr() != g.data_ptr() or not _direct_all(w):
+                raise RuntimeError("Conv0Fn.backward: the fused stem backward was announced but its gradient tensor or the "
+                                   "direct .grad target is not what StemTailFn.backward saw")
+            L = _lib.lib()
+            ws = _ws(L.mcl_conv0_wrw_workspace_floats(B, H, W), x.device)
+            tgt, in_place = _grad_target_khwc(w)
+            check(L.mcl_conv0_wrw_bnrelu(x.data_ptr(), B, H, W, g.data_ptr(), z0.data_ptr(), gamma.data_ptr(),
+                                         beta.data_ptr(), mean.data_ptr(), rstd.data_ptr(), coef.data_ptr(), ws.data_ptr(),
+                                         tgt.data_ptr(), int(in_place), _stream()), "mcl_conv0_wrw_bnrelu")
+            _grad_finish_khwc(w, tgt, in_place)
+            return None, None, None
         if _direct_all(w) and dy.dtype == torch.bfloat16:
             L = _lib.lib()
             ws = _ws(L.mcl_conv0_wrw_workspace_floats(B, H, W), x.device)
@@ -1182,7 +1202,8 @@
 class StemTailFn(torch.autograd.Function):
 
     @staticmethod
-    def forward(ctx, x, gamma, beta, mean, rstd):
+    def forward(ctx, x, gamma, beta, mean, rstd, link=None):
+        ctx.link = link
         B, C, H, W = x.shape
         y = torch.empty((B, C, (H - 1) // 2 + 1, (W - 1) // 2 + 1), device=x.device, dtype=x.dtype, memory_format=CL)
         idx = torch.empty((B, y.shape[2], y.shape[3], C), device=x.device, dtype=torch.uint8)
@@ -1210,10 +1231,26 @@
         check(_lib.lib().mcl_maxpool3s2_nhwc_bf16_bwd_ld(idx.data_ptr(), pdy, lddy, g.data_ptr(), B, H, W, C, _stream()),
               "mcl_maxpool bwd")
         direct = _direct_all(gamma, beta)
+        link = ctx.link
+        if (FUSED_STEM_BWD and link is not None and ctx.cap is None and C == 64 and x.dtype == torch.bfloat16
+                and _direct_all(link["w"])):
+            L = _lib.lib()
+            S = B * H * W
+            ws = _ws(L.mcl_bn_workspace_floats(S, C, 1), x.device)
+            coef = torch.empty(2 * C, device=x.device, dtype=torch.float32)
+            if direct:
+                dg, db = gamma.grad, beta.grad
+            else:
+                dg, db = (torch.empty(C, device=x.device, dtype=torch.float32) for _ in range(2))
+            check(L.mcl_bn_act_bwd_sums(g.data_ptr(), C, x.data_ptr(), C, S, C, 1, gamma.data_ptr(), beta.data_ptr(),
+                                        mean.data_ptr(), rstd.data_ptr(), 1, ws.data_ptr(), dg.data_ptr(), db.data_ptr(),
+                                        int(direct), coef.data_ptr(), _stream()), "mcl_bn_act_bwd_sums")
+            link["bn"] = (g, x, gamma, beta, mean, rstd, coef)
+            return (g, None, None, None, None, None) if direct else (g, dg, db, None, None, None)
         dg, db = bn_act_bwd(g, x, gamma, beta, mean, rstd, True, g, False, into_param_grads=direct)
         if ctx.cap is not None:
             ctx.cap["dx"] = g
-        return g, dg, db, None, None
+        return g, dg, db, None, None, None
 
 
 
@@ -1441,8 +1478,10 @@
     own_conv0 = _conv0_ok(x, features.conv0)
     if own_conv0:
         mean0, var0, rstd0 = (torch.empty(64, device=x.device, dtype=torch.float32) for _ in range(3))
-        x = Conv0Fn.apply(x, features.conv0.weight, (features.norm0.eps, (mean0, var0, rstd0)))
+        stem_link = {}
+        x = Conv0Fn.apply(x, features.conv0.weight, (features.norm0.eps, (mean0, var0, rstd0), stem_link))
     else:
+        stem_link = None
         from . import conv_generic as cg
         x = cg.conv2d(x, features.conv0.weight, features.conv0.stride[0], features.conv0.padding[0])
     x = dense_cl(x)
@@ -1452,7 +1491,7 @@
             mean0, var0, rstd0 = (torch.empty(C0, device=x.device, dtype=torch.float32) for _ in range(3))
             bn_stats(x, mean0, var0, rstd0, features.norm0.eps)
         rec.add(features.norm0, mean0, var0, x.numel() // C0)
-        x = StemTailFn.apply(x, features.norm0.weight, features.norm0.bias, mean0, rstd0)
+        x = StemTailFn.apply(x, features.norm0.weight, features.norm0.bias, mean0, rstd0, stem_link)
     else:
         x = _bn_train(x, features.norm0, True, rec)
         x = max_pool_3s2(dense_cl(x))
diff --git a/mclstexp_amd/kernel_costs.py b/mclstexp_amd/kernel_costs.py
--- a/mclstexp_amd/kernel_costs.py
+++ b/mclstexp_amd/kernel_costs.py
@@ -150,6 +150,15 @@
 
 def _adam_shadow(a):
     return 30 * a[4]
+
+
+def _conv0_wrw_bnrelu(a):
+    N, H, W = a[1], a[2], a[3]
+    return 2 * 2 * N * (H // 2) * (W // 2) * 64 + 2 * N * H * W * 3
+
+
+def _conv0_wrw_flops(a):
+    return 2 * a[1] * (a[2] // 2) * (a[3] // 2) * 64 * 147
 
 
 def _zero(a):
@@ -192,6 +201,8 @@
                               _block_bwd, flops=_block_bwd_flops, bound="latency"),
     "mcl_adam_table_lazy": _e("adam_table_lazy_kernel (catch-up of gathered rows / update of the rows with a gradient)",
                               _adam_table_lazy, bound="latency"),
+    "mcl_conv0_wrw_bnrelu": _e("conv0_wrw_bnrelu_kernel (norm0 / relu0 backward formed in the staging) + wrw_merge_kernel",
+                               _conv0_wrw_bnrelu, flops=_conv0_wrw_flops, bound="hbm"),
     "mcl_adam_step_dev": _e("adam_kernel", _adam, bound="hbm"),
     "mcl_adam_step_dev_shadow": _e("adam_kernel<shadow> (update + bf16 shadow of the parameters)", _adam_shadow, bound="hbm"),
 }
```

Result: no change. 12430 spots/s, median of 6 (+0.8%).
